# slothfulxtx/Texture-GS

Measured on AMD Instinct MI355X. Metric: fwd+bwd views/sec @800x800, 300k Gaussians + 1024^2 texture; HBM GB/s vs roofline, higher is better.
Workload: dtype f32; 1 GPU; c3: N=300000 Gaussians, cubemap 6x1024x1024x3 f32, 800x800, fwd+bwd, sh_degree 3; parallelism=views sharded dp1, view_pipeline=3 HIP streams, order=accumulate, forwards begun one view per stream ahead, grad_allreduce=none (1 GPU)

## Files before the change

include/texgs.h:

```cpp
#ifndef TEXGS_H
#define TEXGS_H

#include <stddef.h>
#include <stdint.h>

#ifdef __cplusplus
extern "C" {
#endif

#define TEXGS_ABI_VERSION 19
#define TEXGS_TILE 16
#define TEXGS_REC_TEST_FLOATS 8
#define TEXGS_REC_SHADE_FLOATS 20
#define TEXGS_ACC_FLOATS 32

typedef struct TexGSFrame {
    int32_t image_height;
    int32_t image_width;
    float   tanfovx;
    float   tanfovy;
    float   scale_modifier;
    int32_t sh_degree;
    int32_t sh_coeffs;
    int32_t tex_res;
    int32_t num_gaussians;
    int32_t debug;
    const float* bg;
    const float* viewmatrix;
    const float* projmatrix;
    const float* campos;
} TexGSFrame;

typedef struct TexGSInputs {
    const float* means3D;
    const float* shs;
    const float* opacities;
    const float* scales;
    const float* rotations;
    const float* uvs;
    const float* gradient_uvs;
    const float* texture;
    const float* color_offset;
    const float* cov3D_precomp;
} TexGSInputs;

typedef struct TexGSGeom {
    float*    rec_test;
    float*    rec_shade;
    float*    depth;
    int32_t*  radii;
    uint32_t* rect;
    uint32_t* tiles_touched;
    uint32_t* offsets;
    void*     scan_temp;
    size_t    scan_temp_bytes;
} TexGSGeom;

typedef struct TexGSBinning {
    uint32_t  num_rendered;
    uint64_t* keys_unsorted;
    uint64_t* keys_sorted;
    uint32_t* point_list;
    uint32_t* ranges;
    uint32_t* tile_order;
    void*     sort_temp;
    size_t    sort_temp_bytes;
} TexGSBinning;

typedef struct TexGSImage {
    float*    out_color;
    float*    out_depth;
    float*    out_norm;
    float*    out_alpha;
    float*    final_T;
    uint32_t* n_contrib;
    uint32_t* tex_bin_count;
    uint32_t* survivors;
    uint16_t* surv_qmask;
    uint32_t* surv_count;
    uint32_t* tex_bin_resv;
} TexGSImage;
#define TEXGS_RESV_WORDS 192

#define TEXGS_ACC_MEANS3D 1
#define TEXGS_ACC_MEANS2D 2
#define TEXGS_ACC_SHS 4
#define TEXGS_ACC_OPACITIES 8
#define TEXGS_ACC_SCALES 16
#define TEXGS_ACC_ROTATIONS 32
#define TEXGS_ACC_UVS 64
#define TEXGS_ACC_COLOR_OFFSET 128
#define TEXGS_ACC_COV3D 256
#define TEXGS_ACC_ALL 511

#define TEXGS_WANT_TEXTURE   1
#define TEXGS_WANT_GAUSSIANS 2
#define TEXGS_WANT_ALL       3

typedef struct TexGSGrads {
    const float* dL_dcolor;
    const float* dL_ddepth;
    const float* dL_dnorm;
    const float* dL_dalpha;
    float* acc;
    float* dL_dmeans3D;
    float* dL_dmeans2D;
    float* dL_dshs;
    float* dL_dopacities;
    float* dL_dscales;
    float* dL_drotations;
    float* dL_duvs;
    float* dL_dtexture;
    float* dL_dcolor_offset;
    float* dL_dcov3D;
    uint32_t want;
    float*    tex_bins;
    uint32_t* tex_bin_cursor;
    uint32_t* tex_bin_base;
    uint32_t  tex_rec_cap;
    int32_t accumulate;
} TexGSGrads;

int         texgs_abi_version(void);
const char* texgs_build_id(void);
const char* texgs_last_error(void);

size_t texgs_scan_temp_bytes(int32_t num_gaussians);
size_t texgs_sort_temp_bytes(uint32_t num_rendered, uint32_t num_tiles);
size_t texgs_tex_bin_count(int32_t tex_res);
#define TEXGS_TEXBIN_RECORD_FLOATS 4

int texgs_preprocess_forward(const TexGSFrame* frame, const TexGSInputs* in, TexGSGeom* geom, void* stream);

size_t texgs_num_rendered_words(int32_t num_gaussians);
int texgs_num_rendered_begin(const TexGSGeom* geom, int32_t num_gaussians, uint32_t* host_pinned, size_t host_words, int32_t sort_first,
                             void* stream);
int texgs_num_rendered_reduce(const uint32_t* host_pinned, int32_t num_gaussians, uint32_t* host_out, uint64_t* fingerprint_out);
int texgs_depth_sort_scan(TexGSGeom* geom, int32_t num_gaussians, void* stream);

int texgs_bin_sort_render_forward(const TexGSFrame* frame, const TexGSInputs* in, const TexGSGeom* geom,
                                  TexGSBinning* bin, TexGSImage* img, void* stream);

int texgs_render_forward(const TexGSFrame* frame, const TexGSInputs* in, const TexGSGeom* geom,
                         const TexGSBinning* bin, TexGSImage* img, void* stream);

int texgs_backward(const TexGSFrame* frame, const TexGSInputs* in, const TexGSGeom* geom,
                   const TexGSBinning* bin, const TexGSImage* img, TexGSGrads* grads, void* stream);

int texgs_backward_render(const TexGSFrame* frame, const TexGSInputs* in, const TexGSGeom* geom,
                          const TexGSBinning* bin, const TexGSImage* img, TexGSGrads* grads, void* stream);
int texgs_backward_preprocess(const TexGSFrame* frame, const TexGSInputs* in, const TexGSGeom* geom, TexGSGrads* grads,
                              void* stream);

enum {
    TEXGS_K_PREPROCESS_FWD = 0, TEXGS_K_SCAN = 1, TEXGS_K_DUPLICATE = 2, TEXGS_K_SORT = 3, TEXGS_K_RANGES = 4,
    TEXGS_K_RENDER_FWD = 5, TEXGS_K_RENDER_BWD = 6, TEXGS_K_PREPROCESS_BWD = 7, TEXGS_K_TEXGRAD_REDUCE = 8,
    TEXGS_NUM_KERNELS = 9
};
int texgs_profile_enable(int on);
int texgs_profile_select(uint32_t kernel_mask);
int texgs_profile_read(float* ms_sum_host, uint32_t* launches_host);

int texgs_rgb_alpha_loss(const float* image, const float* gt_image, const float* alpha, const float* gt_alpha,
                         int32_t H, int32_t W, float lambda_dssim, float lambda_alpha, float* scratch, float* sums,
                         float* dL_dimage, float* dL_dalpha, void* stream);

int texgs_geom_losses(const float* norm, const float* gt_norm, const float* gt_image, const float* mask, const float* depth,
                      const float* gt_depth, int32_t H, int32_t W, float lambda_norm, float lambda_smooth, float gamma,
                      float lambda_depth, float* sums, float* dL_dnorm, float* dL_ddepth, void* stream);

int texgs_norm_from_depth(const float* depth, const float* viewmatrix, float tanfovx, float tanfovy, int32_t H, int32_t W,
                          float threshold, float* out_norm, float* out_mask, void* stream);

typedef struct TexGSUVNet {
    const float *W1, *b1;
    const float *W2, *b2;
    const float *emb;
    const float *W3, *b3, *W4, *b4;
    const float *W5, *b5;
    const float *xyz_offset, *xyz_scale;
    int32_t hidden;
} TexGSUVNet;
enum { TEXGS_UV_FP32 = 0, TEXGS_UV_BF16X3 = 1, TEXGS_UV_MIXED = 2 };
size_t texgs_uv_packed_bytes(int32_t precision);
int texgs_uv_pack(const TexGSUVNet* net, int32_t precision, void* packed, void* stream);
int texgs_uv_taylor_packed(const TexGSUVNet* net, int32_t precision, const void* packed, const float* xyz, int32_t N, float* uvs,
                           float* grad_uvs, void* stream);

typedef struct TexGSUVNetGrad {
    float *dW1, *db1;
    float *dW2, *db2;
    float *dW3, *db3, *dW4, *db4;
    float *dW5, *db5;
} TexGSUVNetGrad;
size_t texgs_uv_backward_temp_bytes(int32_t N);
int texgs_uv_backward(const TexGSUVNet* net, int32_t precision, const float* xyz, const float* g_uvs, int32_t N, const TexGSUVNetGrad* out,
                      void* temp, void* stream);

#define TEXGS_HASHGRID_MAX_LEVELS 16
#define TEXGS_HASHGRID_FEATURES 4
typedef struct TexGSHashGrid {
    int32_t n_levels;
    int32_t n_features;
    int32_t log2_hashmap_size;
    float   base_resolution;
    float   per_level_scale;
} TexGSHashGrid;
int texgs_hashgrid_levels(const TexGSHashGrid* grid, float* scale, uint32_t* res, uint32_t* size, uint32_t* offset, uint32_t* n_params);
int texgs_hashgrid_forward(const TexGSHashGrid* grid, const float* params, const float* x, int32_t N, float* enc, void* stream);
size_t texgs_hashgrid_backward_temp_bytes(const TexGSHashGrid* grid, int32_t N);
int texgs_hashgrid_backward(const TexGSHashGrid* grid, const float* params, const float* x, const float* d_enc, int32_t N,
                            float* d_params, float* d_x, void* temp, void* stream);
size_t texgs_chamfer_nn_temp_bytes(int32_t P);
int texgs_chamfer_nn(const float* a, int32_t P, const float* b, int32_t Q, float* d2, int32_t* idx, void* temp, void* stream);

size_t texgs_knn3_temp_bytes(int32_t n);
int texgs_knn3_mean_dist2(const float* xyz, int32_t n, float* mean_d2, void* temp, void* stream);
size_t texgs_fps_temp_bytes(int32_t n, int32_t k);
int texgs_farthest_points(const float* xyz, int32_t n, int32_t k, int32_t start, int32_t* idx, void* temp, void* stream);

#define TEXGS_CUBE_LINEAR 0
#define TEXGS_CUBE_NEAREST 1
int texgs_cube_sample(const float* tex, int32_t R, int32_t C, const float* dirs, int32_t N, int32_t filter, int32_t tap_map,
                      float* out, void* stream);
int texgs_cube_latlong(const float* tex, int32_t R, int32_t C, int32_t H, int32_t W, int32_t tap_map, float* out, void* stream);
int texgs_cube_sample_backward(const float* tex, int32_t R, int32_t C, const float* dirs, int32_t N, const float* g_out,
                               float* d_tex, float* d_dirs, void* stream);
int texgs_cube_sample_nearest_backward(int32_t R, int32_t C, const float* dirs, int32_t N, const float* g_out, float* d_tex,
                                       void* stream);

int texgs_density_stats(const float* grad, const int32_t* radii, int32_t n, float* accum, float* denom, float* max_radii, void* stream);

#define TEXGS_DENSITY_KEEP       1
#define TEXGS_DENSITY_CLONE      2
#define TEXGS_DENSITY_CLONE_KEPT 4
#define TEXGS_DENSITY_SPLIT      8
#define TEXGS_DENSITY_CHILD      16
typedef struct {
    const float* accum;
    const float* denom;
    const float* scaling;
    const float* opacity;
    int32_t n;
    float max_grad, min_opacity, dense_scale, big_scale;
    int32_t densify, use_big;
} TexGSDensityPlan;
size_t texgs_density_plan_temp_bytes(int32_t n);
int texgs_density_plan(const TexGSDensityPlan* plan, uint8_t* action, int32_t* rank, uint32_t* totals, void* temp, void* stream);

#define TEXGS_DENSITY_ROW_COPY    0
#define TEXGS_DENSITY_ROW_MOMENT  1
#define TEXGS_DENSITY_ROW_SCALING 2
#define TEXGS_DENSITY_ROW_XYZ     3
#define TEXGS_DENSITY_MAX_ROWS    24
typedef struct {
    const float* src;
    float* dst;
    int32_t width;
    int32_t kind;
} TexGSDensityRow;
typedef struct {
    TexGSDensityRow row[TEXGS_DENSITY_MAX_ROWS];
    int32_t rows;
    int32_t n;
    const uint8_t* action;
    const int32_t* rank;
    int32_t n_kept, n_clone, n_split, n_child;
    const float* scaling;
    const float* rotation;
    const float* noise;
} TexGSDensityMove;
int texgs_density_move(const TexGSDensityMove* move, void* stream);

#define TEXGS_METRICS_ROW     16
#define TEXGS_METRICS_L1      0
#define TEXGS_METRICS_SE      1
#define TEXGS_METRICS_SSIM    4
#define TEXGS_METRICS_MAE_NUM 7
#define TEXGS_METRICS_MAE_DEN 8
#define TEXGS_METRICS_PIXELS  9
#define TEXGS_METRICS_CROPPED 10
size_t texgs_eval_metrics_temp_bytes(int32_t H, int32_t W);
int texgs_eval_metrics(const float* image, const float* gt_image, const float* norm, const float* gt_norm, const float* alpha,
                       int32_t H, int32_t W, int32_t clamp01, void* temp, double* row, void* stream);

int texgs_selftest_waveops(const float* seed128, float* out576, void* stream);

int texgs_mark_visible(const TexGSFrame* frame, const float* means3D, uint8_t* visible, void* stream);

#ifdef __cplusplus
}
#endif
#endif
```

texture-gs_amd/csrc/abi.hip:

```cpp
#include "common.h"
#include <stdio.h>
#include <string.h>
#include <stdlib.h>

#include <mutex>
#include <vector>

namespace {

thread_local char g_err[512] = "";

struct EvRec { int kid; hipEvent_t a, b; };
std::mutex g_prof_mu;
bool g_prof_on = false;
uint32_t g_prof_mask = 0xFFFFFFFFu;
std::vector<EvRec> g_prof_log;
std::vector<hipEvent_t> g_prof_free;

hipEvent_t prof_event() {
    if (!g_prof_free.empty()) { hipEvent_t e = g_prof_free.back(); g_prof_free.pop_back(); return e; }
    hipEvent_t e; (void)hipEventCreate(&e); return e;
}

struct ProfScope {
    int kid; hipStream_t s; hipEvent_t a; bool on;
    ProfScope(int k, hipStream_t st) : kid(k), s(st), a(nullptr), on(false) {
        std::lock_guard<std::mutex> l(g_prof_mu);
        if (g_prof_on && ((g_prof_mask >> k) & 1u)) { on = true; a = prof_event(); (void)hipEventRecord(a, s); }
    }
    ~ProfScope() {
        if (!on) return;
        std::lock_guard<std::mutex> l(g_prof_mu);
        hipEvent_t b = prof_event(); (void)hipEventRecord(b, s);
        g_prof_log.push_back({kid, a, b});
    }
};

int fail(const char* where, hipError_t e) {
    snprintf(g_err, sizeof(g_err), "%s: %s", where, hipGetErrorString(e));
    return (int)e ? (int)e : -1;
}

int fail_msg(const char* msg) {
    snprintf(g_err, sizeof(g_err), "%s", msg);
    return -1;
}

int check(const TexGSFrame* f, hipStream_t s, const char* where) {
    hipError_t e = hipGetLastError();
    if (e != hipSuccess) return fail(where, e);
    if (f->debug) {
        e = hipStreamSynchronize(s);
        if (e != hipSuccess) return fail(where, e);
    }
    return 0;
}

int validate_frame(const TexGSFrame* f) {
    if (!f) return fail_msg("frame is NULL");
    if (f->image_height <= 0 || f->image_width <= 0) return fail_msg("image size must be positive");
    if (f->image_width > 65535 * TEXGS_TILE || f->image_height > 65535 * TEXGS_TILE) return fail_msg("image too large");
    {
        const long long tx = (f->image_width + TEXGS_TILE - 1) / TEXGS_TILE, ty = (f->image_height + TEXGS_TILE - 1) / TEXGS_TILE;
        if (tx * ty > (1ll << 24)) return fail_msg("image too large: more than 2^24 tiles");
    }
    if (f->sh_degree < 0 || f->sh_degree > 3) return fail_msg("sh_degree must be in [0,3]");
    if (f->num_gaussians < 0) return fail_msg("num_gaussians < 0");
    if (f->tex_res <= 0) return fail_msg("tex_res must be positive");
    if (f->tex_res > 7168) return fail_msg("tex_res > 7168: the blend kernels address texels with 32-bit byte offsets (6 R^2 x 12 B < 2^32)");
    if (!f->bg || !f->viewmatrix || !f->projmatrix || !f->campos) return fail_msg("frame device pointers must be non-NULL");
    return 0;
}

}

extern "C" {

int texgs_abi_version(void) { return TEXGS_ABI_VERSION; }

#ifndef TEXGS_BUILD_ID
#define TEXGS_BUILD_ID "unknown"
#endif
const char* texgs_build_id(void) { return TEXGS_BUILD_ID; }

const char* texgs_last_error(void) { return g_err; }

size_t texgs_scan_temp_bytes(int32_t num_gaussians) { return scan_temp_bytes(num_gaussians); }

size_t texgs_sort_temp_bytes(uint32_t num_rendered, uint32_t num_tiles) { return sort_temp_bytes(num_rendered, num_tiles); }

size_t texgs_tex_bin_count(int32_t tex_res) { return tex_bin_count(tex_res); }

int texgs_preprocess_forward(const TexGSFrame* frame, const TexGSInputs* in, TexGSGeom* geom, void* stream) {
    if (int r = validate_frame(frame)) return r;
    if (!in || !geom) return fail_msg("NULL argument");
    if (frame->num_gaussians == 0) return 0;
    if (!in->means3D || !in->opacities) return fail_msg("per-Gaussian input pointer is NULL");
    if (in->texture && (!in->uvs || !in->gradient_uvs)) return fail_msg("uvs / gradient_uvs are required with a texture");
    if (in->cov3D_precomp && in->texture) return fail_msg("cov3D_precomp is an input of the untextured surface only (texture must be NULL)");
    if (!in->cov3D_precomp && (!in->scales || !in->rotations)) return fail_msg("scales and rotations (or cov3D_precomp) are required");
    if (geom->scan_temp_bytes < scan_temp_bytes(frame->num_gaussians)) return fail_msg("scan_temp too small");
    hipStream_t s = (hipStream_t)stream;
    const CamConst c = make_cam(frame);
    { ProfScope p(TEXGS_K_PREPROCESS_FWD, s); launch_preprocess_fwd(c, frame, in, geom, s); }
    if (int r = check(frame, s, "preprocess_fwd")) return r;
    return 0;
}

static int depth_sort_scan(const TexGSFrame* frame, TexGSGeom* geom, hipStream_t s) {
    if (frame->num_gaussians == 0) return 0;
    { ProfScope p(TEXGS_K_SCAN, s);
      if (int r = launch_depth_sort_scan(geom, frame->num_gaussians, s)) return fail("depth sort / scan", (hipError_t)r); }
    return check(frame, s, "depth sort / scan");
}

size_t texgs_num_rendered_words(int32_t num_gaussians) {
    return num_gaussians <= 0 ? 0 : 3 * (((size_t)num_gaussians + TG_BLOCK - 1) / TG_BLOCK);
}
int texgs_num_rendered_begin(const TexGSGeom* geom, int32_t num_gaussians, uint32_t* host_pinned, size_t host_words, int32_t sort_first,
                             void* stream) {
    if (!geom || !host_pinned) return fail_msg("NULL argument");
    if (num_gaussians <= 0) return 0;
    const size_t nw = texgs_num_rendered_words(num_gaussians);
    if (host_words < nw) return fail_msg("host buffer too small (texgs_num_rendered_words)");
    hipStream_t s = (hipStream_t)stream;
    hipError_t e = hipMemcpyAsync(host_pinned, bin_block_sums_ptr(geom, num_gaussians), nw * sizeof(uint32_t), hipMemcpyDeviceToHost, s);
    if (e != hipSuccess) return fail("num_rendered readback", e);
    if (sort_first) {
        TexGSFrame f0; memset(&f0, 0, sizeof(f0)); f0.num_gaussians = num_gaussians;
        if (int r = depth_sort_scan(&f0, const_cast<TexGSGeom*>(geom), s)) return r;
    }
    return 0;
}
int texgs_num_rendered_reduce(const uint32_t* host_pinned, int32_t num_gaussians, uint32_t* host_out, uint64_t* fingerprint_out) {
    if (!host_pinned || !host_out) return fail_msg("NULL argument");
    *host_out = 0;
    if (fingerprint_out) *fingerprint_out = 0;
    if (num_gaussians <= 0) return 0;
    const size_t nblk = ((size_t)num_gaussians + TG_BLOCK - 1) / TG_BLOCK;
    unsigned long long total = 0ull;
    uint32_t fa = 0u, fb = 0u;
    for (size_t k = 0; k < nblk; ++k) { total += host_pinned[k]; fa += host_pinned[nblk + k]; fb += host_pinned[2 * nblk + k]; }
    if (total > 0xFFFFFFFFull) return fail_msg("num_rendered exceeds 2^32 - 1 instances");
    *host_out = (uint32_t)total;
    if (fingerprint_out) *fingerprint_out = ((uint64_t)fb << 32) | (uint64_t)fa;
    return 0;
}

int texgs_depth_sort_scan(TexGSGeom* geom, int32_t num_gaussians, void* stream) {
    if (!geom) return fail_msg("NULL argument");
    TexGSFrame f0; memset(&f0, 0, sizeof(f0)); f0.num_gaussians = num_gaussians;
    return depth_sort_scan(&f0, geom, (hipStream_t)stream);
}

static int render_forward_impl(const TexGSFrame* frame, const TexGSInputs* in, const TexGSGeom* geom,
                               const TexGSBinning* bin, TexGSImage* img, void* stream, bool counters_zeroed) {
    if (int r = validate_frame(frame)) return r;
    if (!in || !geom || !bin || !img) return fail_msg("NULL argument");
    hipStream_t s = (hipStream_t)stream;
    const CamConst c = make_cam(frame);
    if (img->tex_bin_count && in->texture && !counters_zeroed) {
        hipError_t e = hipMemsetAsync(img->tex_bin_count, 0, sizeof(uint32_t) * 2 * tex_bin_count(c.R), s);
        if (e != hipSuccess) return fail("tex_bin_count memset", e);
    }
    { ProfScope p(TEXGS_K_RENDER_FWD, s); launch_render_fwd(c, frame, in, geom, bin, img, s); }
    return check(frame, s, "render_fwd");
}

int texgs_render_forward(const TexGSFrame* frame, const TexGSInputs* in, const TexGSGeom* geom,
                         const TexGSBinning* bin, TexGSImage* img, void* stream) {
    return render_forward_impl(frame, in, geom, bin, img, stream, false);
}

int texgs_bin_sort_render_forward(const TexGSFrame* frame, const TexGSInputs* in, const TexGSGeom* geom,
                                  TexGSBinning* bin, TexGSImage* img, void* stream) {
    if (int r = validate_frame(frame)) return r;
    if (!in || !geom || !bin || !img) return fail_msg("NULL argument");
    hipStream_t s = (hipStream_t)stream;
    const CamConst c = make_cam(frame);
    if (bin->num_rendered > 0) {
        if (bin->sort_temp_bytes < sort_temp_bytes(bin->num_rendered, (uint32_t)(c.tiles_x * c.tiles_y))) return fail_msg("sort_temp too small");
        { ProfScope p(TEXGS_K_DUPLICATE, s); launch_duplicate(c, geom, bin, s); }
        if (int r = check(frame, s, "duplicate_with_keys")) return r;
        { ProfScope p(TEXGS_K_SORT, s);
          if (int r = launch_sort(c, geom, bin, s)) return fail("tile sort", (hipError_t)r); }
        if (int r = check(frame, s, "tile sort")) return r;
    }
    { ProfScope p(TEXGS_K_RANGES, s);
      launch_ranges(c, bin, img->tex_bin_count, img->tex_bin_count ? 2 * (int)tex_bin_count(c.R) : 0, s); }
    if (int r = check(frame, s, "tile_ranges")) return r;
    return render_forward_impl(frame, in, geom, bin, img, stream, true);
}

int texgs_backward_render(const TexGSFrame* frame, const TexGSInputs* in, const TexGSGeom* geom,
                          const TexGSBinning* bin, const TexGSImage* img, TexGSGrads* grads, void* stream) {
    if (int r = validate_frame(frame)) return r;
    if (!in || !geom || !bin || !img || !grads) return fail_msg("NULL argument");
    if (!(grads->want & TEXGS_WANT_ALL)) return fail_msg("TexGSGrads.want is empty: ask for TEXGS_WANT_TEXTURE and / or TEXGS_WANT_GAUSSIANS");
    if ((grads->want & TEXGS_WANT_GAUSSIANS) && !grads->acc) return fail_msg("acc must be allocated (zero-filled) when Gaussian gradients are wanted");
    if ((grads->want & TEXGS_WANT_TEXTURE) && in->texture && !grads->dL_dtexture) return fail_msg("dL_dtexture must be allocated (zero-filled) when the texture gradient is wanted");
    if (!img->survivors || !img->surv_qmask || !img->surv_count)
        return fail_msg("the forward of this call left no survivor lists (TexGSImage.survivors / surv_qmask / surv_count were NULL): "
                        "run the forward with them to be able to run its backward");
    hipStream_t s = (hipStream_t)stream;
    const CamConst c = make_cam(frame);
    if (bin->num_rendered > 0) {
        { ProfScope p(TEXGS_K_RENDER_BWD, s); launch_render_bwd(c, frame, in, geom, bin, img, grads, s); }
        if (int r = check(frame, s, "render_bwd")) return r;
        if (tex_bins_enabled(c, in, img, grads)) {
            { ProfScope p(TEXGS_K_TEXGRAD_REDUCE, s); launch_texgrad_reduce(c, img, grads, s); }
            if (int r = check(frame, s, "texgrad_reduce")) return r;
        }
    }
    return 0;
}

int texgs_backward_preprocess(const TexGSFrame* frame, const TexGSInputs* in, const TexGSGeom* geom, TexGSGrads* grads,
                              void* stream) {
    if (int r = validate_frame(frame)) return r;
    if (!in || !geom || !grads) return fail_msg("NULL argument");
    if (!(grads->want & TEXGS_WANT_GAUSSIANS)) return 0;
    if (!grads->acc) return fail_msg("acc must be allocated");
    if (in->cov3D_precomp && !grads->dL_dcov3D) return fail_msg("dL_dcov3D is required with cov3D_precomp");
    hipStream_t s = (hipStream_t)stream;
    const CamConst c = make_cam(frame);
    { ProfScope p(TEXGS_K_PREPROCESS_BWD, s); launch_preprocess_bwd(c, frame, in, geom, grads, s); }
    return check(frame, s, "preprocess_bwd");
}

int texgs_backward(const TexGSFrame* frame, const TexGSInputs* in, const TexGSGeom* geom,
                   const TexGSBinning* bin, const TexGSImage* img, TexGSGrads* grads, void* stream) {
    if (int r = texgs_backward_render(frame, in, geom, bin, img, grads, stream)) return r;
    return texgs_backward_preprocess(frame, in, geom, grads, stream);
}

int texgs_profile_enable(int on) {
    std::lock_guard<std::mutex> l(g_prof_mu);
    g_prof_on = on != 0;
    if (!g_prof_on) {
        for (auto& r : g_prof_log) { g_prof_free.push_back(r.a); g_prof_free.push_back(r.b); }
        g_prof_log.clear();
    }
    return 0;
}

int texgs_profile_select(uint32_t kernel_mask) {
    std::lock_guard<std::mutex> l(g_prof_mu);
    g_prof_mask = kernel_mask;
    return 0;
}

int texgs_profile_read(float* ms_sum_host, uint32_t* launches_host) {
    if (!ms_sum_host || !launches_host) return fail_msg("NULL argument");
    std::lock_guard<std::mutex> l(g_prof_mu);
    for (auto& r : g_prof_log) {
        hipError_t e = hipEventSynchronize(r.b);
        if (e != hipSuccess) return fail("profile event sync", e);
        float ms = 0.f;
        e = hipEventElapsedTime(&ms, r.a, r.b);
        if (e != hipSuccess) return fail("profile elapsed", e);
        if (r.kid >= 0 && r.kid < TEXGS_NUM_KERNELS) { ms_sum_host[r.kid] += ms; launches_host[r.kid] += 1; }
        g_prof_free.push_back(r.a); g_prof_free.push_back(r.b);
    }
    g_prof_log.clear();
    return 0;
}

int texgs_rgb_alpha_loss(const float* image, const float* gt_image, const float* alpha, const float* gt_alpha,
                         int32_t H, int32_t W, float lambda_dssim, float lambda_alpha, float* scratch, float* sums,
                         float* dL_dimage, float* dL_dalpha, void* stream) {
    if (!image || !gt_image || !scratch || !sums || !dL_dimage) return fail_msg("NULL argument");
    if (H <= 0 || W <= 0) return fail_msg("image size must be positive");
    hipStream_t s = (hipStream_t)stream;
    launch_rgb_alpha_loss(image, gt_image, alpha, gt_alpha, H, W, lambda_dssim, lambda_alpha, scratch, sums, dL_dimage,
                          dL_dalpha, s);
    hipError_t e = hipGetLastError();
    return e == hipSuccess ? 0 : fail("rgb_alpha_loss", e);
}

int texgs_geom_losses(const float* norm, const float* gt_norm, const float* gt_image, const float* mask, const float* depth,
                      const float* gt_depth, int32_t H, int32_t W, float lambda_norm, float lambda_smooth, float gamma,
                      float lambda_depth, float* sums, float* dL_dnorm, float* dL_ddepth, void* stream) {
    if (!sums) return fail_msg("NULL argument");
    if (H <= 0 || W <= 0 || !(gamma > 0.f)) return fail_msg("image size and gamma must be positive");
    if (lambda_norm != 0.f && (!norm || !gt_norm || !dL_dnorm)) return fail_msg("norm term needs norm, gt_norm, dL_dnorm");
    if (lambda_smooth != 0.f && (!norm || !gt_image || !dL_dnorm)) return fail_msg("smoothness term needs norm, gt_image, dL_dnorm");
    if (lambda_depth != 0.f && (!depth || !gt_depth || !dL_ddepth)) return fail_msg("depth term needs depth, gt_depth, dL_ddepth");
    launch_geom_losses(norm, gt_norm, gt_image, mask, depth, gt_depth, H, W, lambda_norm, lambda_smooth, gamma, lambda_depth, sums,
                       dL_dnorm, dL_ddepth, (hipStream_t)stream);
    hipError_t e = hipGetLastError();
    return e == hipSuccess ? 0 : fail("geom_losses", e);
}

int texgs_norm_from_depth(const float* depth, const float* viewmatrix, float tanfovx, float tanfovy, int32_t H, int32_t W,
                          float threshold, float* out_norm, float* out_mask, void* stream) {
    if (!depth || !viewmatrix || !out_norm || !out_mask) return fail_msg("NULL argument");
    if (H <= 0 || W <= 0) return fail_msg("image size must be positive");
    launch_norm_from_depth(depth, viewmatrix, tanfovx, tanfovy, H, W, threshold, out_norm, out_mask, (hipStream_t)stream);
    hipError_t e = hipGetLastError();
    return e == hipSuccess ? 0 : fail("norm_from_depth", e);
}

static int check_uvnet(const TexGSUVNet* net, int32_t precision) {
    if (precision != TEXGS_UV_FP32 && precision != TEXGS_UV_BF16X3 && precision != TEXGS_UV_MIXED)
        return fail_msg("precision must be TEXGS_UV_FP32, TEXGS_UV_BF16X3 or TEXGS_UV_MIXED");
    if (net->hidden != 128) return fail_msg("the UV-map kernels support the shipped UVNet shape only (hidden width 128)");
    if (!net->W1 || !net->W2 || !net->W3 || !net->W4 || !net->W5 || !net->emb) return fail_msg("weight pointer is NULL");
    return 0;
}

size_t texgs_uv_packed_bytes(int32_t precision) { return uv_packed_bytes(precision); }

int texgs_uv_pack(const TexGSUVNet* net, int32_t precision, void* packed, void* stream) {
    if (!net || !packed) return fail_msg("NULL argument");
    if (int r = check_uvnet(net, precision)) return r;
    if (int r = launch_uv_pack(net, precision, packed, (hipStream_t)stream)) return fail("uv_pack", (hipError_t)r);
    return 0;
}

int texgs_uv_taylor_packed(const TexGSUVNet* net, int32_t precision, const void* packed, const float* xyz, int32_t N, float* uvs,
                           float* grad_uvs, void* stream) {
    if (!net || !packed) return fail_msg("NULL argument");
    if (int r = check_uvnet(net, precision)) return r;
    if (N < 0) return fail_msg("N < 0");
    if (N > 0 && (!xyz || !uvs || !grad_uvs)) return fail_msg("NULL argument");
    if (int r = launch_uv_taylor_packed(net, precision, packed, xyz, N, uvs, grad_uvs, (hipStream_t)stream)) return fail("uv_taylor", (hipError_t)r);
    return 0;
}

size_t texgs_uv_backward_temp_bytes(int32_t N) { return uv_backward_temp_bytes(N < 0 ? 0 : N); }

int texgs_uv_backward(const TexGSUVNet* net, int32_t precision, const float* xyz, const float* g_uvs, int32_t N, const TexGSUVNetGrad* out,
                      void* temp, void* stream) {
    if (!net || !out || !temp) return fail_msg("NULL argument");
    if (int r = check_uvnet(net, precision)) return r;
    if (N < 0) return fail_msg("N < 0");
    if (N > 0 && (!xyz || !g_uvs)) return fail_msg("NULL argument");
    if (int r = launch_uv_backward(net, xyz, g_uvs, N, out, temp, precision != TEXGS_UV_FP32, (hipStream_t)stream))
        return fail("uv_backward", (hipError_t)r);
    return 0;
}

static int check_hashgrid(const TexGSHashGrid* g, uint32_t* n_params) {
    if (!g) return fail_msg("grid is NULL");
    float sc[TEXGS_HASHGRID_MAX_LEVELS];
    uint32_t r[TEXGS_HASHGRID_MAX_LEVELS], sz[TEXGS_HASHGRID_MAX_LEVELS], off[TEXGS_HASHGRID_MAX_LEVELS];
    switch (hashgrid_levels(g, sc, r, sz, off, n_params)) {
    case 0: return 0;
    case -1: return fail_msg("hash grid: n_levels must be in [1, 16]");
    case -2: return fail_msg("hash grid: n_features must be 4");
    case -3: return fail_msg("hash grid: log2_hashmap_size must be in [1, 24]");
    case -4: return fail_msg("hash grid: base_resolution must be >= 1 and per_level_scale in [1, 16]");
    case -5: return fail_msg("hash grid: a level's resolution is out of range");
    default: return fail_msg("hash grid: more than 2^31 parameters");
    }
}

int texgs_hashgrid_levels(const TexGSHashGrid* grid, float* scale, uint32_t* res, uint32_t* size, uint32_t* offset, uint32_t* n_params) {
    uint32_t n = 0;
    if (int r = check_hashgrid(grid, &n)) return r;
    float sc[TEXGS_HASHGRID_MAX_LEVELS];
    uint32_t rs[TEXGS_HASHGRID_MAX_LEVELS], sz[TEXGS_HASHGRID_MAX_LEVELS], off[TEXGS_HASHGRID_MAX_LEVELS];
    hashgrid_levels(grid, sc, rs, sz, off, &n);
    for (int l = 0; l < grid->n_levels; ++l) {
        if (scale) scale[l] = sc[l];
        if (res) res[l] = rs[l];
        if (size) size[l] = sz[l];
        if (offset) offset[l] = off[l];
    }
    if (n_params) *n_params = n;
    return 0;
}

int texgs_hashgrid_forward(const TexGSHashGrid* grid, const float* params, const float* x, int32_t N, float* enc, void* stream) {
    uint32_t n = 0;
    if (int r = check_hashgrid(grid, &n)) return r;
    if (N < 0) return fail_msg("N < 0");
    if ((int64_t)N * grid->n_levels * TEXGS_HASHGRID_FEATURES > INT32_MAX) return fail_msg("N * L * F >= 2^31");
    if (N > 0 && (!params || !x || !enc)) return fail_msg("NULL argument");
    if (N > 0 && (((uintptr_t)params | (uintptr_t)enc) & 15)) return fail_msg("params and enc must be 16-byte aligned");
    if (int r = launch_hashgrid_forward(grid, params, x, N, enc, (hipStream_t)stream)) return fail("hashgrid_forward", (hipError_t)r);
    hipError_t e = hipGetLastError();
    return e == hipSuccess ? 0 : fail("hashgrid_forward", e);
}

size_t texgs_hashgrid_backward_temp_bytes(const TexGSHashGrid* grid, int32_t N) {
    uint32_t n = 0;
    if (!grid || check_hashgrid(grid, &n)) return 0;
    return hashgrid_backward_temp_bytes(grid, N);
}

int texgs_hashgrid_backward(const TexGSHashGrid* grid, const float* params, const float* x, const float* d_enc, int32_t N,
                            float* d_params, float* d_x, void* temp, void* stream) {
    uint32_t n = 0;
    if (int r = check_hashgrid(grid, &n)) return r;
    if (N < 0) return fail_msg("N < 0");
    if ((int64_t)N * grid->n_levels * TEXGS_HASHGRID_FEATURES > INT32_MAX) return fail_msg("N * L * F >= 2^31");
    if (N > 0 && (!params || !x || !d_enc)) return fail_msg("NULL argument");
    if (N > 0 && (((uintptr_t)params | (uintptr_t)d_enc | (uintptr_t)d_params) & 15))
        return fail_msg("params, d_enc and d_params must be 16-byte aligned");
    if (N > 0 && d_x && !temp) return fail_msg("temp is NULL (d_x needs texgs_hashgrid_backward_temp_bytes)");
    if (int r = launch_hashgrid_backward(grid, params, x, d_enc, N, d_params, d_x, temp, (hipStream_t)stream))
        return fail("hashgrid_backward", (hipError_t)r);
    hipError_t e = hipGetLastError();
    return e == hipSuccess ? 0 : fail("hashgrid_backward", e);
}

size_t texgs_chamfer_nn_temp_bytes(int32_t P) { return chamfer_nn_temp_bytes(P); }

int texgs_chamfer_nn(const float* a, int32_t P, const float* b, int32_t Q, float* d2, int32_t* idx, void* temp, void* stream) {
    if (P < 0) return fail_msg("P < 0");
    if (Q < 1) return fail_msg("the reference set is empty (Q < 1)");
    if ((int64_t)Q > 65535ll * 512) return fail_msg("Q > 65535 * 512");
    if (P > 0 && (!a || !b || !d2 || !idx || !temp)) return fail_msg("NULL argument");
    if (int r = launch_chamfer_nn(a, P, b, Q, d2, idx, temp, (hipStream_t)stream)) return fail("chamfer_nn", (hipError_t)r);
    hipError_t e = hipGetLastError();
    return e == hipSuccess ? 0 : fail("chamfer_nn", e);
}

size_t texgs_knn3_temp_bytes(int32_t n) { return knn3_temp_bytes(n); }

int texgs_knn3_mean_dist2(const float* xyz, int32_t n, float* mean_d2, void* temp, void* stream) {
    if (n < 4) return fail_msg("n < 4: three nearest other points need at least four points");
    if (!xyz || !mean_d2 || !temp) return fail_msg("NULL argument");
    if (int r = launch_knn3_mean_dist2(xyz, n, mean_d2, temp, (hipStream_t)stream)) return fail("knn3_mean_dist2", (hipError_t)r);
    return 0;
}

size_t texgs_fps_temp_bytes(int32_t n, int32_t k) { return fps_temp_bytes(n, k); }

int texgs_farthest_points(const float* xyz, int32_t n, int32_t k, int32_t start, int32_t* idx, void* temp, void* stream) {
    if (n < 1) return fail_msg("n < 1");
    if (k < 1 || k > n) return fail_msg("k must be in [1, n]");
    if (start < 0 || start >= n) return fail_msg("start must be in [0, n)");
    if (!xyz || !idx || !temp) return fail_msg("NULL argument");
    if (int r = launch_farthest_points(xyz, n, k, start, idx, temp, (hipStream_t)stream)) return fail("farthest_points", (hipError_t)r);
    return 0;
}

static int cube_shape_ok(int32_t R, int32_t C) {
    if (R < 2) return fail_msg("R < 2: a cubemap face needs at least 2 x 2 texels");
    if (C < 1) return fail_msg("C < 1");
    if (6ll * R * R * C >= (1ll << 31)) return fail_msg("6 R R C must be below 2^31");
    return 0;
}

int texgs_cube_sample(const float* tex, int32_t R, int32_t C, const float* dirs, int32_t N, int32_t filter, int32_t tap_map,
                      float* out, void* stream) {
    if (int r = cube_shape_ok(R, C)) return r;
    if (N < 0) return fail_msg("N < 0");
    if (filter != TEXGS_CUBE_LINEAR && filter != TEXGS_CUBE_NEAREST) return fail_msg("filter must be TEXGS_CUBE_LINEAR or TEXGS_CUBE_NEAREST");
    if (!tex || (N > 0 && (!dirs || !out))) return fail_msg("NULL argument");
    if (int r = launch_cube_sample(tex, R, C, dirs, N, filter, tap_map, out, (hipStream_t)stream)) return fail("cube_sample", (hipError_t)r);
    return 0;
}

int texgs_cube_latlong(const float* tex, int32_t R, int32_t C, int32_t H, int32_t W, int32_t tap_map, float* out, void* stream) {
    if (int r = cube_shape_ok(R, C)) return r;
    if (H < 1 || W < 1) return fail_msg("H and W must be positive");
    if ((long long)H * W >= (1ll << 31)) return fail_msg("H W must be below 2^31");
    if (!tex || !out) return fail_msg("NULL argument");
    if (int r = launch_cube_latlong(tex, R, C, H, W, tap_map, out, (hipStream_t)stream)) return fail("cube_latlong", (hipError_t)r);
    return 0;
}

int texgs_cube_sample_backward(const float* tex, int32_t R, int32_t C, const float* dirs, int32_t N, const float* g_out,
                               float* d_tex, float* d_dirs, void* stream) {
    if (int r = cube_shape_ok(R, C)) return r;
    if (N < 0) return fail_msg("N < 0");
    if (!d_tex && !d_dirs) return fail_msg("d_tex and d_dirs are both NULL: nothing to compute");
    if ((d_dirs && !tex) || (N > 0 && (!dirs || !g_out))) return fail_msg("NULL argument");
    if (int r = launch_cube_sample_backward(tex, R, C, dirs, N, g_out, d_tex, d_dirs, (hipStream_t)stream))
        return fail("cube_sample_backward", (hipError_t)r);
    return 0;
}

int texgs_cube_sample_nearest_backward(int32_t R, int32_t C, const float* dirs, int32_t N, const float* g_out, float* d_tex,
                                       void* stream) {
    if (int r = cube_shape_ok(R, C)) return r;
    if (N < 0) return fail_msg("N < 0");
    if (!d_tex || (N > 0 && (!dirs || !g_out))) return fail_msg("NULL argument");
    if (int r = launch_cube_sample_nearest_backward(R, C, dirs, N, g_out, d_tex, (hipStream_t)stream))
        return fail("cube_sample_nearest_backward", (hipError_t)r);
    return 0;
}

int texgs_density_stats(const float* grad, const int32_t* radii, int32_t n, float* accum, float* denom, float* max_radii, void* stream) {
    if (n < 0) return fail_msg("n < 0");
    if (n > 0 && (!grad || !radii || !accum || !denom || !max_radii)) return fail_msg("NULL argument");
    if (int r = launch_density_stats(grad, radii, n, accum, denom, max_radii, (hipStream_t)stream)) return fail("density_stats", (hipError_t)r);
    return 0;
}

size_t texgs_density_plan_temp_bytes(int32_t n) { return density_plan_temp_bytes(n); }

int texgs_density_plan(const TexGSDensityPlan* plan, uint8_t* action, int32_t* rank, uint32_t* totals, void* temp, void* stream) {
    if (!plan || !totals) return fail_msg("NULL argument");
    if (plan->n < 0) return fail_msg("n < 0");
    if (plan->n > 0 && (!plan->scaling || !plan->opacity || !action || !rank || !temp)) return fail_msg("NULL argument");
    if (plan->n > 0 && plan->densify && (!plan->accum || !plan->denom)) return fail_msg("accum and denom are required to densify");
    if (plan->densify && !(plan->max_grad > 0.0f)) return fail_msg("max_grad must be positive (with 0 the reference splits its own clones)");
    if (int r = launch_density_plan(plan, action, rank, totals, temp, (hipStream_t)stream)) return fail("density_plan", (hipError_t)r);
    return 0;
}

int texgs_density_move(const TexGSDensityMove* m, void* stream) {
    if (!m) return fail_msg("NULL argument");
    if (m->n < 0 || m->n_kept < 0 || m->n_clone < 0 || m->n_split < 0 || m->n_child < 0) return fail_msg("negative count");
    if (m->n_kept > m->n || m->n_clone > m->n || m->n_split > m->n || m->n_child > m->n_split) return fail_msg("totals exceed n");
    if ((int64_t)m->n_kept + m->n_clone + 2ll * m->n_child >= (1ll << 31)) return fail_msg("the new row count reaches 2^31");
    if (m->rows < 0 || m->rows > TEXGS_DENSITY_MAX_ROWS) return fail_msg("rows must be in [0, TEXGS_DENSITY_MAX_ROWS]");
    if (m->n == 0 || m->rows == 0) return 0;
    if (!m->action || !m->rank) return fail_msg("NULL argument");
    const bool out_rows = m->n_kept + m->n_clone + m->n_child > 0;
    for (int d = 0; d < m->rows; ++d) {
        const TexGSDensityRow& r = m->row[d];
        if (r.width < 1) return fail_msg("row width < 1");
        if (r.kind < TEXGS_DENSITY_ROW_COPY || r.kind > TEXGS_DENSITY_ROW_XYZ) return fail_msg("unknown row kind");
        if (r.kind == TEXGS_DENSITY_ROW_XYZ && r.width != 3) return fail_msg("an XYZ row has width 3");
        if (!r.src || (out_rows && !r.dst)) return fail_msg("NULL row pointer");
        if (r.kind == TEXGS_DENSITY_ROW_XYZ && m->n_child > 0 && (!m->scaling || !m->rotation || !m->noise))
            return fail_msg("an XYZ row with children needs scaling, rotation and noise");
    }
    if (!out_rows) return 0;
    if (int r = launch_density_move(m, (hipStream_t)stream)) return fail("density_move", (hipError_t)r);
    return 0;
}

size_t texgs_eval_metrics_temp_bytes(int32_t H, int32_t W) { return eval_metrics_temp_bytes(H, W); }

int texgs_eval_metrics(const float* image, const float* gt_image, const float* norm, const float* gt_norm, const float* alpha,
                       int32_t H, int32_t W, int32_t clamp01, void* temp, double* row, void* stream) {
    if (!image || !gt_image || !temp || !row) return fail_msg("NULL argument");
    if (H < 7 || W < 7) return fail_msg("H and W must be at least 7: the 7x7 SSIM window does not fit");
    if ((!norm) != (!gt_norm)) return fail_msg("norm and gt_norm must be both NULL or both set");
    if ((((int64_t)W + 31) / 32) * (((int64_t)H + 31) / 32) >= (1ll << 31)) return fail_msg("image too large: 2^31 tiles or more");
    if (int r = launch_eval_metrics(image, gt_image, norm, gt_norm, alpha, H, W, clamp01 != 0, temp, row, (hipStream_t)stream))
        return fail("eval_metrics", (hipError_t)r);
    return 0;
}

int texgs_selftest_waveops(const float* seed128, float* out576, void* stream) {
    if (!seed128 || !out576) return fail_msg("NULL argument");
    launch_selftest_waveops(seed128, out576, (hipStream_t)stream);
    hipError_t e = hipGetLastError();
    return e == hipSuccess ? 0 : fail("selftest_waveops", e);
}

int texgs_mark_visible(const TexGSFrame* frame, const float* means3D, uint8_t* visible, void* stream) {
    if (int r = validate_frame(frame)) return r;
    if (!means3D || !visible) return fail_msg("NULL argument");
    hipStream_t s = (hipStream_t)stream;
    launch_mark_visible(frame, means3D, visible, s);
    return check(frame, s, "mark_visible");
}

}
```

texture-gs_amd/csrc/common.h:

```cpp
#pragma once
#include <hip/hip_runtime.h>
#include <stdint.h>
#include "texgs.h"

#define TG_NEAR_Z        0.2f
#define TG_LOWPASS       0.3f
#define TG_FRUSTUM_CLAMP 1.3f
#define TG_ALPHA_MAX     0.99f
#define TG_ALPHA_MIN     (1.0f / 255.0f)
#define TG_T_EPS         1e-4f
#define TG_PLANE_EPS     5e-2f
#define TG_DEN_MIN       0.2f
#define TG_MA_MIN        1e-20f
#define TG_SH_C0         0.28209479177387814f

enum {
    R_XY = 0, R_CONIC = 2, R_OP = 5, R_G2 = 6, R_GM = 8, R_PHI = 14, R_VD = 17, R_DEPTH = 20, R_N = 21
};
enum {
    M_P = 0, M_DEN = 6, M_DN = 9, M_PHI = 18, M_VD = 21, M_DEPTH = 24, M_N = 25
};

#define TG_BLOCK 256

struct CamConst {
    int W, H, tiles_x, tiles_y;
    float fx, fy, tanfovx, tanfovy;
    float scale_modifier;
    int sh_degree, sh_coeffs, R, N;
};

static inline CamConst make_cam(const TexGSFrame* f) {
    CamConst c;
    c.W = f->image_width; c.H = f->image_height;
    c.tiles_x = (c.W + TEXGS_TILE - 1) / TEXGS_TILE;
    c.tiles_y = (c.H + TEXGS_TILE - 1) / TEXGS_TILE;
    c.tanfovx = f->tanfovx; c.tanfovy = f->tanfovy;
    c.fx = (float)c.W / (2.0f * f->tanfovx);
    c.fy = (float)c.H / (2.0f * f->tanfovy);
    c.scale_modifier = f->scale_modifier;
    c.sh_degree = f->sh_degree; c.sh_coeffs = f->sh_coeffs; c.R = f->tex_res; c.N = f->num_gaussians;
    return c;
}

void launch_preprocess_fwd(const CamConst& c, const TexGSFrame* f, const TexGSInputs* in, TexGSGeom* g, hipStream_t s);
void launch_preprocess_bwd(const CamConst& c, const TexGSFrame* f, const TexGSInputs* in, const TexGSGeom* g,
                           TexGSGrads* gr, hipStream_t s);
void launch_mark_visible(const TexGSFrame* f, const float* means3D, uint8_t* visible, hipStream_t s);
int  launch_depth_sort_scan(const TexGSGeom* g, int N, hipStream_t s);
uint32_t* bin_block_sums_ptr(const TexGSGeom* g, int N);
uint32_t* bin_header_ptr(const TexGSGeom* g, int N, int* words);
size_t scan_temp_bytes(int N);
size_t sort_temp_bytes(uint32_t D, uint32_t T);
void launch_duplicate(const CamConst& c, const TexGSGeom* g, TexGSBinning* b, hipStream_t s);
int  launch_sort(const CamConst& c, const TexGSGeom* g, TexGSBinning* b, hipStream_t s);
void launch_ranges(const CamConst& c, TexGSBinning* b, uint32_t* zero_words, int num_zero_words, hipStream_t s);
void launch_render_fwd(const CamConst& c, const TexGSFrame* f, const TexGSInputs* in, const TexGSGeom* g,
                       const TexGSBinning* b, TexGSImage* img, hipStream_t s);
size_t tex_bin_count(int R);
bool tex_bins_enabled(const CamConst& c, const TexGSInputs* in, const TexGSImage* img, const TexGSGrads* gr);
void launch_texgrad_reduce(const CamConst& c, const TexGSImage* img, TexGSGrads* gr, hipStream_t s);
void launch_render_bwd(const CamConst& c, const TexGSFrame* f, const TexGSInputs* in, const TexGSGeom* g,
                       const TexGSBinning* b, const TexGSImage* img, TexGSGrads* gr, hipStream_t s);
int launch_rgb_alpha_loss(const float* image, const float* gt_image, const float* alpha, const float* gt_alpha, int H,
                          int W, float lambda_dssim, float lambda_alpha, float* scratch, float* sums, float* d_image,
                          float* d_alpha, hipStream_t s);
void launch_selftest_waveops(const float* seed128, float* out576, hipStream_t s);
int launch_geom_losses(const float* norm, const float* gt_norm, const float* gt_image, const float* mask, const float* depth,
                       const float* gt_depth, int H, int W, float lambda_norm, float lambda_smooth, float gamma,
                       float lambda_depth, float* sums, float* d_norm, float* d_depth, hipStream_t s);
int launch_norm_from_depth(const float* depth, const float* viewmatrix, float tanfovx, float tanfovy, int H, int W, float threshold,
                           float* out_norm, float* out_mask, hipStream_t s);
size_t uv_packed_bytes(int precision);
int launch_uv_pack(const TexGSUVNet* net, int precision, void* packed, hipStream_t s);
int launch_uv_taylor_packed(const TexGSUVNet* net, int precision, const void* packed, const float* xyz, int N, float* uvs, float* grad_uvs,
                            hipStream_t s);
size_t uv_backward_temp_bytes(int N);
int launch_uv_backward(const TexGSUVNet* net, const float* xyz, const float* g, int N, const TexGSUVNetGrad* out, void* temp, int mixed,
                       hipStream_t s);
int hashgrid_levels(const TexGSHashGrid* g, float* scale, uint32_t* res, uint32_t* size, uint32_t* offset, uint32_t* n_params);
int launch_hashgrid_forward(const TexGSHashGrid* g, const float* params, const float* x, int N, float* enc, hipStream_t s);
size_t hashgrid_backward_temp_bytes(const TexGSHashGrid* g, int N);
int launch_hashgrid_backward(const TexGSHashGrid* g, const float* params, const float* x, const float* d_enc, int N, float* d_params,
                             float* d_x, void* temp, hipStream_t s);
size_t chamfer_nn_temp_bytes(int P);
int launch_chamfer_nn(const float* a, int P, const float* b, int Q, float* d2, int32_t* idx, void* temp, hipStream_t s);
size_t sort_pairs32_temp_bytes(uint32_t n);
int launch_sort_pairs32(const uint32_t* keys_in, uint32_t n, int key_bits, uint32_t* keys_out, uint32_t* vals_out, void* temp, hipStream_t s);
size_t knn3_temp_bytes(int n);
int launch_knn3_mean_dist2(const float* xyz, int n, float* mean_d2, void* temp, hipStream_t s);
size_t fps_temp_bytes(int n, int k);
int launch_farthest_points(const float* xyz, int n, int k, int start, int32_t* idx, void* temp, hipStream_t s);
int launch_cube_sample(const float* tex, int R, int C, const float* dirs, int N, int filter, int tap_map, float* out, hipStream_t s);
int launch_cube_latlong(const float* tex, int R, int C, int H, int W, int tap_map, float* out, hipStream_t s);
int launch_cube_sample_backward(const float* tex, int R, int C, const float* dirs, int N, const float* g_out, float* d_tex,
                                float* d_dirs, hipStream_t s);
int launch_cube_sample_nearest_backward(int R, int C, const float* dirs, int N, const float* g_out, float* d_tex, hipStream_t s);
int launch_density_stats(const float* grad, const int32_t* radii, int n, float* accum, float* denom, float* max_radii, hipStream_t s);
size_t density_plan_temp_bytes(int n);
int launch_density_plan(const TexGSDensityPlan* p, uint8_t* action, int32_t* rank, uint32_t* totals, void* temp, hipStream_t s);
int launch_density_move(const TexGSDensityMove* m, hipStream_t s);
size_t eval_metrics_temp_bytes(int H, int W);
int launch_eval_metrics(const float* image, const float* gt_image, const float* norm, const float* gt_norm, const float* alpha, int H,
                        int W, int clamp01, void* temp, double* row, hipStream_t s);
```

texture-gs_amd/csrc/preprocess.hip:

```cpp
#include "common.h"

namespace {

struct Frame {
    float V[16];
    float P[16];
    float cam[3];
};

__device__ __forceinline__ Frame load_frame(const float* vm, const float* pm, const float* cp) {
    Frame f;
#pragma unroll
    for (int i = 0; i < 16; ++i) { f.V[i] = vm[i]; f.P[i] = pm[i]; }
    f.cam[0] = cp[0]; f.cam[1] = cp[1]; f.cam[2] = cp[2];
    return f;
}

struct Geo {
    bool  valid;
    float m[3], t[3];
    float hx, hy, hw, pw, xy[2];
    float q[4], s[3], R[9], M[9], S[6];
    float txc, tyc; bool clx, cly;
    float J00, J02, J11, J12, T0[3], T1[3];
    float a, b, c, det, inv, conic[3];
    int   radius;
    int   kmin; float sign; float n[3];
    float nv[3], sdot; bool degen; float gx, gy, G[6], K[9];
    float dir[3], dlen;
};

#define WR(F, r, c) ((F).V[(c) * 4 + (r)])

__device__ __forceinline__ void smallest_eigvec(const float* S6, float* n) {
    const float tr = S6[0] + S6[3] + S6[5];
    const float sc = (tr > 0.f) ? 1.0f / tr : 1.0f;
    float a00 = S6[0] * sc, a01 = S6[1] * sc, a02 = S6[2] * sc, a11 = S6[3] * sc, a12 = S6[4] * sc, a22 = S6[5] * sc;
    float v00 = 1.f, v01 = 0.f, v02 = 0.f, v10 = 0.f, v11 = 1.f, v12 = 0.f, v20 = 0.f, v21 = 0.f, v22 = 1.f;
    auto rot = [](float& app, float& aqq, float& apq, float& arp, float& arq, float& v0p, float& v0q, float& v1p, float& v1q,
                  float& v2p, float& v2q) {
        if (fabsf(apq) < 1e-30f) return;
        const float theta = (aqq - app) / (2.0f * apq);
        const float t = ((theta >= 0.f) ? 1.0f : -1.0f) / (fabsf(theta) + sqrtf(theta * theta + 1.0f));
        const float c = 1.0f / sqrtf(t * t + 1.0f), sn = t * c;
        app -= t * apq; aqq += t * apq; apq = 0.f;
        const float rp = arp, rq = arq;
        arp = c * rp - sn * rq; arq = sn * rp + c * rq;
        float x;
        x = v0p; v0p = c * x - sn * v0q; v0q = sn * x + c * v0q;
        x = v1p; v1p = c * x - sn * v1q; v1q = sn * x + c * v1q;
        x = v2p; v2p = c * x - sn * v2q; v2q = sn * x + c * v2q;
    };
#pragma unroll 1
    for (int sweep = 0; sweep < 6; ++sweep) {
        rot(a00, a11, a01, a02, a12, v00, v01, v10, v11, v20, v21);
        rot(a00, a22, a02, a01, a12, v00, v02, v10, v12, v20, v22);
        rot(a11, a22, a12, a01, a02, v01, v02, v11, v12, v21, v22);
    }
    int k = 0; float m = a00;
    if (a11 < m) { m = a11; k = 1; }
    if (a22 < m) { m = a22; k = 2; }
    n[0] = (k == 0) ? v00 : ((k == 1) ? v01 : v02);
    n[1] = (k == 0) ? v10 : ((k == 1) ? v11 : v12);
    n[2] = (k == 0) ? v20 : ((k == 1) ? v21 : v22);
}

template <bool COV = false>
__device__ __forceinline__ void geo_forward(Geo& g, const Frame& F, const CamConst& C, int i,
                                            const float* __restrict__ means, const float* __restrict__ scales,
                                            const float* __restrict__ rots, const float* __restrict__ juv,
                                            const float* __restrict__ cov6 = nullptr) {
    g.m[0] = means[3 * i + 0]; g.m[1] = means[3 * i + 1]; g.m[2] = means[3 * i + 2];
    const float mx = g.m[0], my = g.m[1], mz = g.m[2];
    g.t[0] = F.V[0] * mx + F.V[4] * my + F.V[8] * mz + F.V[12];
    g.t[1] = F.V[1] * mx + F.V[5] * my + F.V[9] * mz + F.V[13];
    g.t[2] = F.V[2] * mx + F.V[6] * my + F.V[10] * mz + F.V[14];
    g.valid = g.t[2] > TG_NEAR_Z;
    g.radius = 0;
    if (!g.valid) return;
    const float tx = g.t[0], ty = g.t[1], tz = g.t[2];

    g.hx = F.P[0] * mx + F.P[4] * my + F.P[8] * mz + F.P[12];
    g.hy = F.P[1] * mx + F.P[5] * my + F.P[9] * mz + F.P[13];
    g.hw = F.P[3] * mx + F.P[7] * my + F.P[11] * mz + F.P[15];
    g.pw = 1.0f / (g.hw + 1e-7f);
    const float ndcx = g.hx * g.pw, ndcy = g.hy * g.pw;
    g.xy[0] = ((ndcx + 1.0f) * (float)C.W - 1.0f) * 0.5f;
    g.xy[1] = ((ndcy + 1.0f) * (float)C.H - 1.0f) * 0.5f;

    float s0 = 0.f, s1 = 0.f, s2 = 0.f;
    if constexpr (COV) {
#pragma unroll
        for (int k = 0; k < 6; ++k) g.S[k] = cov6[6 * i + k];
#pragma unroll
        for (int k = 0; k < 9; ++k) { g.R[k] = 0.f; g.M[k] = 0.f; }
        g.q[0] = g.q[1] = g.q[2] = g.q[3] = 0.f; g.s[0] = g.s[1] = g.s[2] = 0.f;
    } else {
    g.q[0] = rots[4 * i + 0]; g.q[1] = rots[4 * i + 1]; g.q[2] = rots[4 * i + 2]; g.q[3] = rots[4 * i + 3];
    const float r = g.q[0], x = g.q[1], y = g.q[2], z = g.q[3];
    g.R[0] = 1.0f - 2.0f * (y * y + z * z); g.R[1] = 2.0f * (x * y - r * z); g.R[2] = 2.0f * (x * z + r * y);
    g.R[3] = 2.0f * (x * y + r * z); g.R[4] = 1.0f - 2.0f * (x * x + z * z); g.R[5] = 2.0f * (y * z - r * x);
    g.R[6] = 2.0f * (x * z - r * y); g.R[7] = 2.0f * (y * z + r * x); g.R[8] = 1.0f - 2.0f * (x * x + y * y);
    s0 = scales[3 * i + 0]; s1 = scales[3 * i + 1]; s2 = scales[3 * i + 2];
    g.s[0] = C.scale_modifier * s0; g.s[1] = C.scale_modifier * s1; g.s[2] = C.scale_modifier * s2;
#pragma unroll
    for (int rr = 0; rr < 3; ++rr)
#pragma unroll
        for (int cc = 0; cc < 3; ++cc) g.M[rr * 3 + cc] = g.R[rr * 3 + cc] * g.s[cc];
    const float* M = g.M;
    g.S[0] = M[0] * M[0] + M[1] * M[1] + M[2] * M[2];
    g.S[1] = M[0] * M[3] + M[1] * M[4] + M[2] * M[5];
    g.S[2] = M[0] * M[6] + M[1] * M[7] + M[2] * M[8];
    g.S[3] = M[3] * M[3] + M[4] * M[4] + M[5] * M[5];
    g.S[4] = M[3] * M[6] + M[4] * M[7] + M[5] * M[8];
    g.S[5] = M[6] * M[6] + M[7] * M[7] + M[8] * M[8];
    }

    const float limx = TG_FRUSTUM_CLAMP * C.tanfovx, limy = TG_FRUSTUM_CLAMP * C.tanfovy;
    const float txtz = tx / tz, tytz = ty / tz;
    g.clx = (txtz < -limx) || (txtz > limx);
    g.cly = (tytz < -limy) || (tytz > limy);
    g.txc = fminf(limx, fmaxf(-limx, txtz)) * tz;
    g.tyc = fminf(limy, fmaxf(-limy, tytz)) * tz;
    if (!g.clx) g.txc = tx;
    if (!g.cly) g.tyc = ty;
    const float tz2 = tz * tz;
    g.J00 = C.fx / tz; g.J02 = -(C.fx * g.txc) / tz2;
    g.J11 = C.fy / tz; g.J12 = -(C.fy * g.tyc) / tz2;
#pragma unroll
    for (int k = 0; k < 3; ++k) {
        g.T0[k] = g.J00 * WR(F, 0, k) + g.J02 * WR(F, 2, k);
        g.T1[k] = g.J11 * WR(F, 1, k) + g.J12 * WR(F, 2, k);
    }
    const float* S = g.S;
    const float v00 = S[0] * g.T0[0] + S[1] * g.T0[1] + S[2] * g.T0[2];
    const float v01 = S[1] * g.T0[0] + S[3] * g.T0[1] + S[4] * g.T0[2];
    const float v02 = S[2] * g.T0[0] + S[4] * g.T0[1] + S[5] * g.T0[2];
    const float v10 = S[0] * g.T1[0] + S[1] * g.T1[1] + S[2] * g.T1[2];
    const float v11 = S[1] * g.T1[0] + S[3] * g.T1[1] + S[4] * g.T1[2];
    const float v12 = S[2] * g.T1[0] + S[4] * g.T1[1] + S[5] * g.T1[2];
    g.a = (g.T0[0] * v00 + g.T0[1] * v01 + g.T0[2] * v02) + TG_LOWPASS;
    g.b = g.T1[0] * v00 + g.T1[1] * v01 + g.T1[2] * v02;
    g.c = (g.T1[0] * v10 + g.T1[1] * v11 + g.T1[2] * v12) + TG_LOWPASS;
    g.det = g.a * g.c - g.b * g.b;
    if (g.det == 0.0f) { g.valid = false; return; }
    g.inv = 1.0f / g.det;
    g.conic[0] = g.c * g.inv; g.conic[1] = -g.b * g.inv; g.conic[2] = g.a * g.inv;
    const float mid = 0.5f * (g.a + g.c);
    const float lam = mid + sqrtf(fmaxf(0.1f, mid * mid - g.det));
    g.radius = (int)ceilf(3.0f * sqrtf(lam));

    g.dir[0] = mx - F.cam[0]; g.dir[1] = my - F.cam[1]; g.dir[2] = mz - F.cam[2];
    float n0, n1, n2;
    if constexpr (COV) {
        float ev[3];
        smallest_eigvec(g.S, ev);
        n0 = ev[0]; n1 = ev[1]; n2 = ev[2];
        g.kmin = -1;
    } else {
        g.kmin = 0; float smin = s0;
        if (s1 < smin) { smin = s1; g.kmin = 1; }
        if (s2 < smin) { smin = s2; g.kmin = 2; }
        n0 = (g.kmin == 0) ? g.R[0] : ((g.kmin == 1) ? g.R[1] : g.R[2]);
        n1 = (g.kmin == 0) ? g.R[3] : ((g.kmin == 1) ? g.R[4] : g.R[5]);
        n2 = (g.kmin == 0) ? g.R[6] : ((g.kmin == 1) ? g.R[7] : g.R[8]);
    }
    g.sign = ((n0 * g.dir[0] + n1 * g.dir[1] + n2 * g.dir[2]) > 0.0f) ? -1.0f : 1.0f;
    g.n[0] = g.sign * n0; g.n[1] = g.sign * n1; g.n[2] = g.sign * n2;
    g.dlen = sqrtf(g.dir[0] * g.dir[0] + g.dir[1] * g.dir[1] + g.dir[2] * g.dir[2]);
    g.dir[0] /= g.dlen; g.dir[1] /= g.dlen; g.dir[2] /= g.dlen;

#pragma unroll
    for (int k = 0; k < 3; ++k)
        g.nv[k] = WR(F, k, 0) * g.n[0] + WR(F, k, 1) * g.n[1] + WR(F, k, 2) * g.n[2];
    g.sdot = g.nv[0] * tx + g.nv[1] * ty + g.nv[2] * tz;
    const float tn = sqrtf(tx * tx + ty * ty + tz * tz);
    g.degen = (juv == nullptr) || fabsf(g.sdot) <= TG_PLANE_EPS * tn;
#pragma unroll
    for (int rr = 0; rr < 3; ++rr)
#pragma unroll
        for (int cc = 0; cc < 3; ++cc)
            g.K[rr * 3 + cc] = (juv == nullptr) ? 0.0f
                             : juv[9 * i + rr * 3 + 0] * WR(F, cc, 0) + juv[9 * i + rr * 3 + 1] * WR(F, cc, 1)
                             + juv[9 * i + rr * 3 + 2] * WR(F, cc, 2);
    if (g.degen) {
        g.gx = 0.0f; g.gy = 0.0f;
#pragma unroll
        for (int k = 0; k < 6; ++k) g.G[k] = 0.0f;
    } else {
        const float ax = tz * g.nv[0] / g.sdot, ay = tz * g.nv[1] / g.sdot;
        g.gx = ax / C.fx; g.gy = ay / C.fy;
        const float B00 = tz / C.fx - tx * g.gx, B01 = -tx * g.gy;
        const float B10 = -ty * g.gx,            B11 = tz / C.fy - ty * g.gy;
        const float B20 = -tz * g.gx,            B21 = -tz * g.gy;
#pragma unroll
        for (int rr = 0; rr < 3; ++rr) {
            g.G[rr * 2 + 0] = g.K[rr * 3 + 0] * B00 + g.K[rr * 3 + 1] * B10 + g.K[rr * 3 + 2] * B20;
            g.G[rr * 2 + 1] = g.K[rr * 3 + 0] * B01 + g.K[rr * 3 + 1] * B11 + g.K[rr * 3 + 2] * B21;
        }
    }
}

__device__ __forceinline__ void tile_rect(const Geo& g, const CamConst& C, int& x0, int& y0, int& x1, int& y1) {
    const float rf = (float)g.radius;
    x0 = min(C.tiles_x, max(0, (int)((g.xy[0] - rf) / (float)TEXGS_TILE)));
    y0 = min(C.tiles_y, max(0, (int)((g.xy[1] - rf) / (float)TEXGS_TILE)));
    x1 = min(C.tiles_x, max(0, (int)((g.xy[0] + rf + (float)(TEXGS_TILE - 1)) / (float)TEXGS_TILE)));
    y1 = min(C.tiles_y, max(0, (int)((g.xy[1] + rf + (float)(TEXGS_TILE - 1)) / (float)TEXGS_TILE)));
}

__device__ __forceinline__ void sh_basis(int deg, float x, float y, float z, float* b) {
    const float C1 = 0.4886025119029199f;
    b[0] = -C1 * y; b[1] = C1 * z; b[2] = -C1 * x;
    if (deg > 1) {
        const float xx = x * x, yy = y * y, zz = z * z, xy = x * y, yz = y * z, xz = x * z;
        b[3] = 1.0925484305920792f * xy;
        b[4] = -1.0925484305920792f * yz;
        b[5] = 0.31539156525252005f * (2.0f * zz - xx - yy);
        b[6] = -1.0925484305920792f * xz;
        b[7] = 0.5462742152960396f * (xx - yy);
        if (deg > 2) {
            b[8]  = -0.5900435899266435f * y * (3.0f * xx - yy);
            b[9]  = 2.890611442640554f * xy * z;
            b[10] = -0.4570457994644658f * y * (4.0f * zz - xx - yy);
            b[11] = 0.3731763325901154f * z * (2.0f * zz - 3.0f * xx - 3.0f * yy);
            b[12] = -0.4570457994644658f * x * (4.0f * zz - xx - yy);
            b[13] = 1.445305721320277f * z * (xx - yy);
            b[14] = -0.5900435899266435f * x * (xx - 3.0f * yy);
        }
    }
}

__device__ __forceinline__ void sh_basis_grad(int deg, float x, float y, float z, float* bx, float* by, float* bz) {
    const float C1 = 0.4886025119029199f;
    bx[0] = 0.f; by[0] = -C1; bz[0] = 0.f;
    bx[1] = 0.f; by[1] = 0.f; bz[1] = C1;
    bx[2] = -C1; by[2] = 0.f; bz[2] = 0.f;
    if (deg > 1) {
        const float c20 = 1.0925484305920792f, c22 = 0.31539156525252005f, c24 = 0.5462742152960396f;
        bx[3] = c20 * y;   by[3] = c20 * x;   bz[3] = 0.f;
        bx[4] = 0.f;       by[4] = -c20 * z;  bz[4] = -c20 * y;
        bx[5] = c22 * (-2.0f * x); by[5] = c22 * (-2.0f * y); bz[5] = c22 * 4.0f * z;
        bx[6] = -c20 * z;  by[6] = 0.f;       bz[6] = -c20 * x;
        bx[7] = c24 * 2.0f * x; by[7] = -c24 * 2.0f * y; bz[7] = 0.f;
        if (deg > 2) {
            const float xx = x * x, yy = y * y, zz = z * z;
            const float c30 = -0.5900435899266435f, c31 = 2.890611442640554f, c32 = -0.4570457994644658f,
                        c33 = 0.3731763325901154f, c35 = 1.445305721320277f;
            bx[8]  = c30 * 6.0f * x * y;            by[8]  = c30 * (3.0f * xx - 3.0f * yy);        bz[8]  = 0.f;
            bx[9]  = c31 * y * z;                   by[9]  = c31 * x * z;                          bz[9]  = c31 * x * y;
            bx[10] = c32 * (-2.0f * x * y);         by[10] = c32 * (4.0f * zz - xx - 3.0f * yy);   bz[10] = c32 * 8.0f * y * z;
            bx[11] = c33 * (-6.0f * x * z);         by[11] = c33 * (-6.0f * y * z);                bz[11] = c33 * (6.0f * zz - 3.0f * xx - 3.0f * yy);
            bx[12] = c32 * (4.0f * zz - 3.0f * xx - yy); by[12] = c32 * (-2.0f * x * y);           bz[12] = c32 * 8.0f * x * z;
            bx[13] = c35 * 2.0f * x * z;            by[13] = -c35 * 2.0f * y * z;                  bz[13] = c35 * (xx - yy);
            bx[14] = c30 * (3.0f * xx - 3.0f * yy); by[14] = c30 * (-6.0f * x * y);                bz[14] = 0.f;
        }
    }
}

__device__ __forceinline__ int sh_active(int deg, int K) {
    const int want = (deg + 1) * (deg + 1) - 1;
    return want < K ? want : K;
}

template <int BLOCK, bool ADD>
__device__ __forceinline__ void sh_rows_out(float* __restrict__ g, const float* __restrict__ s, int count, bool vec) {
    const int tid = (int)threadIdx.x;
    int done = 0;
    if (vec) {
        const int n4 = count >> 2;
        float4* __restrict__ g4 = reinterpret_cast<float4*>(g);
        const float4* s4 = reinterpret_cast<const float4*>(s);
        for (int k = tid; k < n4; k += 4 * BLOCK) {
            float4 v[4], o[4];
            bool nz[4];
#pragma unroll
            for (int u = 0; u < 4; ++u) {
                const bool in = k + u * BLOCK < n4;
                v[u] = in ? s4[k + u * BLOCK] : make_float4(0.f, 0.f, 0.f, 0.f);
                nz[u] = in && (!ADD || v[u].x != 0.f || v[u].y != 0.f || v[u].z != 0.f || v[u].w != 0.f);
            }
            if (ADD) {
#pragma unroll
                for (int u = 0; u < 4; ++u) if (nz[u]) o[u] = g4[k + u * BLOCK];
#pragma unroll
                for (int u = 0; u < 4; ++u) if (nz[u]) g4[k + u * BLOCK] = make_float4(o[u].x + v[u].x, o[u].y + v[u].y, o[u].z + v[u].z, o[u].w + v[u].w);
            } else {
#pragma unroll
                for (int u = 0; u < 4; ++u) if (nz[u]) g4[k + u * BLOCK] = v[u];
            }
        }
        done = n4 << 2;
    }
    for (int k = done + tid; k < count; k += BLOCK) {
        const float v = s[k];
        if (ADD) { if (v != 0.f) g[k] += v; } else g[k] = v;
    }
}

template <bool COV>
__global__ void __launch_bounds__(TG_BLOCK)
k_preprocess_fwd(CamConst C, const float* __restrict__ vm, const float* __restrict__ pm, const float* __restrict__ cp,
                 const float* __restrict__ means, const float* __restrict__ shs, const float* __restrict__ opac,
                 const float* __restrict__ scales, const float* __restrict__ rots, const float* __restrict__ uvs,
                 const float* __restrict__ juv, const float* __restrict__ coff, const float* __restrict__ cov6,
                 float4* __restrict__ rec_test, float4* __restrict__ rec_shade, float* __restrict__ depth, int32_t* __restrict__ radii,
                 uint2* __restrict__ rect, uint32_t* __restrict__ tiles_touched, uint32_t* __restrict__ block_D,
                 uint32_t* __restrict__ zero_words, int num_zero_words) {
    extern __shared__ __attribute__((aligned(16))) float s_sh[];
    __shared__ uint32_t s_tt[5 * (TG_BLOCK / 64)];
    const int i = blockIdx.x * TG_BLOCK + threadIdx.x;
    const bool live = i < C.N;
    for (int k = i; k < num_zero_words; k += (int)gridDim.x * TG_BLOCK) zero_words[k] = 0u;
    const Frame F = load_frame(vm, pm, cp);
    Geo g;
    g.valid = false;
    if (live) geo_forward<COV>(g, F, C, i, means, scales, rots, juv, cov6);
    int x0 = 0, y0 = 0, x1 = 0, y1 = 0;
    if (g.valid) {
        tile_rect(g, C, x0, y0, x1, y1);
        if ((x1 - x0) * (y1 - y0) == 0) g.valid = false;
    }
    const int na = (shs != nullptr && C.sh_degree > 0) ? sh_active(C.sh_degree, C.sh_coeffs) : 0;
    const int row = 3 * C.sh_coeffs;
    if (na > 0) {
        const size_t first = (size_t)blockIdx.x * TG_BLOCK * row;
        const size_t total = (size_t)C.N * row;
        const int count = (int)min((size_t)TG_BLOCK * row, total - first);
        for (int k = threadIdx.x; k < count; k += TG_BLOCK) s_sh[k] = shs[first + k];
        __syncthreads();
    }
    uint32_t tt = 0u, ha = 0u, hb = 0u;
    if (live) {
        ha = (uint32_t)i * 0x9E3779B1u + 0x85EBCA77u;
        hb = ((uint32_t)i * 0xC2B2AE3Du) ^ 0x27D4EB2Fu;
    }
    auto mix = [&](uint32_t w) {
        ha = (ha ^ w) * 0x01000193u;
        hb = __builtin_rotateleft32(hb ^ w, 13) * 5u + 0xE6546B64u;
    };
    if (live && !g.valid) {
        radii[i] = 0; tiles_touched[i] = 0; rect[i] = make_uint2(0u, 0u);
        depth[i] = __uint_as_float(0xFFFFFFFFu);
        mix(0xFFFFFFFFu);
    }
    if (live && g.valid) {
    float vd[3] = {0.f, 0.f, 0.f};
    if (na > 0) {
        float b[15];
#pragma unroll
        for (int k = 0; k < 15; ++k) b[k] = 0.f;
        sh_basis(C.sh_degree, g.dir[0], g.dir[1], g.dir[2], b);
        const float* sp = s_sh + threadIdx.x * row;
#pragma unroll
        for (int k = 0; k < 15; ++k) {
            if (k < na) { vd[0] += b[k] * sp[3 * k + 0]; vd[1] += b[k] * sp[3 * k + 1]; vd[2] += b[k] * sp[3 * k + 2]; }
        }
    }
    if (coff) { vd[0] += coff[3 * i + 0]; vd[1] += coff[3 * i + 1]; vd[2] += coff[3 * i + 2]; }
    radii[i] = g.radius;
    tt = (uint32_t)((x1 - x0) * (y1 - y0));
    tiles_touched[i] = tt;
    depth[i] = g.t[2];
    const uint2 rc = make_uint2((uint32_t)x0 | ((uint32_t)y0 << 16), (uint32_t)x1 | ((uint32_t)y1 << 16));
    rect[i] = rc;
    const float op = opac[i];
    const float thr = (op > 0.0f) ? (-logf(255.0f * op) - 1e-3f) : 1.0f;
    const float cmid = 0.5f * (g.a + g.c);
    const float clam = cmid + sqrtf(fmaxf(0.1f, cmid * cmid - g.det));
    const float rcull = (thr < 0.0f) ? (sqrtf(-2.0f * thr * clam) * 1.001f + 0.01f) : -1.0f;
    const float4 t0 = make_float4(g.xy[0], g.xy[1], -0.5f * g.conic[0], -g.conic[1]);
    const float4 t1 = make_float4(-0.5f * g.conic[2], op, rcull, thr);
    const float4 s0 = make_float4(g.gx, g.gy, g.G[0], g.G[1]);
    const float4 s1 = make_float4(g.G[2], g.G[3], g.G[4], g.G[5]);
    const float4 s2 = uvs ? make_float4(uvs[3 * i + 0], uvs[3 * i + 1], uvs[3 * i + 2], vd[0]) : make_float4(0.f, 0.f, 1.f, vd[0]);
    float4* rt = rec_test + (size_t)i * (TEXGS_REC_TEST_FLOATS / 4);
    rt[0] = t0; rt[1] = t1;
    float4* rs = rec_shade + (size_t)i * (TEXGS_REC_SHADE_FLOATS / 4);
    rs[0] = s0; rs[1] = s1; rs[2] = s2;
    rs[3] = make_float4(vd[1], vd[2], g.t[2], g.n[0]);
    rs[4] = make_float4(g.n[1], g.n[2], g.xy[0], g.xy[1]);
    mix(__float_as_uint(g.t[2])); mix(rc.x); mix(rc.y);
    mix(__float_as_uint(t0.x)); mix(__float_as_uint(t0.y)); mix(__float_as_uint(t0.z)); mix(__float_as_uint(t0.w));
    mix(__float_as_uint(t1.x)); mix(__float_as_uint(t1.y)); mix(__float_as_uint(t1.z)); mix(__float_as_uint(t1.w));
    mix(__float_as_uint(s0.x)); mix(__float_as_uint(s0.y)); mix(__float_as_uint(s0.z)); mix(__float_as_uint(s0.w));
    mix(__float_as_uint(s1.x)); mix(__float_as_uint(s1.y)); mix(__float_as_uint(s1.z)); mix(__float_as_uint(s1.w));
    mix(__float_as_uint(s2.x)); mix(__float_as_uint(s2.y)); mix(__float_as_uint(s2.z));
    }
    ha ^= ha >> 15; ha *= 0x2C1B3C6Du; ha ^= ha >> 12;
    hb ^= hb >> 16; hb *= 0x85EBCA6Bu; hb ^= hb >> 13;
    if (!live) { ha = 0u; hb = 0u; }
    uint32_t kmin = (live && g.valid) ? __float_as_uint(g.t[2]) : 0xFFFFFFFFu, kmax = (live && g.valid) ? __float_as_uint(g.t[2]) : 0u;
    for (int d = 32; d >= 1; d >>= 1) {
        tt += __shfl_xor(tt, d, 64); ha += __shfl_xor(ha, d, 64); hb += __shfl_xor(hb, d, 64);
        kmin = min(kmin, (uint32_t)__shfl_xor((int)kmin, d, 64)); kmax = max(kmax, (uint32_t)__shfl_xor((int)kmax, d, 64));
    }
    constexpr int NW = TG_BLOCK / 64;
    if ((threadIdx.x & 63) == 0) {
        const int w = threadIdx.x >> 6;
        s_tt[w] = tt; s_tt[NW + w] = ha; s_tt[2 * NW + w] = hb; s_tt[3 * NW + w] = kmin; s_tt[4 * NW + w] = kmax;
    }
    __syncthreads();
    if (threadIdx.x < 5) {
        uint32_t r = s_tt[threadIdx.x * NW];
        for (int w = 1; w < NW; ++w) {
            const uint32_t v = s_tt[threadIdx.x * NW + w];
            r = (threadIdx.x < 3) ? r + v : ((threadIdx.x == 3) ? min(r, v) : max(r, v));
        }
        block_D[threadIdx.x * gridDim.x + blockIdx.x] = r;
    }
}

#ifndef K8_BLOCK
#define K8_BLOCK 256
#endif
template <bool COV>
__global__ void __launch_bounds__(K8_BLOCK)
k_preprocess_bwd(CamConst C, const float* __restrict__ vm, const float* __restrict__ pm, const float* __restrict__ cp,
                 const float* __restrict__ means, const float* __restrict__ shs, const float* __restrict__ opac,
                 const float* __restrict__ scales,
                 const float* __restrict__ rots, const float* __restrict__ juv, const float* __restrict__ cov6,
                 const int32_t* __restrict__ radii, float* __restrict__ acc,
                 float* __restrict__ d_means, float* __restrict__ d_means2D, float* __restrict__ d_shs,
                 float* __restrict__ d_op, float* __restrict__ d_scales, float* __restrict__ d_rots,
                 float* __restrict__ d_uvs, float* __restrict__ d_coff, float* __restrict__ d_cov6, int accumulate) {
    extern __shared__ __attribute__((aligned(16))) float s_sh[];
    const int i = blockIdx.x * K8_BLOCK + threadIdx.x;
    const int K = C.sh_coeffs;
    const bool live = i < C.N;
    const int row = 3 * K;
    const int na = (shs != nullptr && C.sh_degree > 0) ? sh_active(C.sh_degree, K) : 0;
    const size_t first = (size_t)blockIdx.x * K8_BLOCK * row;
    const int count = d_shs ? (int)min((size_t)K8_BLOCK * row, (size_t)C.N * row - first) : 0;
    const bool vec = d_shs && (((size_t)d_shs) & 15) == 0;
    if (na > 0 && d_shs) {
        for (int k = threadIdx.x; k < count; k += K8_BLOCK) s_sh[k] = shs[first + k];
        __syncthreads();
    }
    const bool visible = live && radii[i] > 0;
    if (live && !visible) {
        if (!(accumulate & TEXGS_ACC_MEANS3D)) d_means[3 * i] = d_means[3 * i + 1] = d_means[3 * i + 2] = 0.f;
        if (!(accumulate & TEXGS_ACC_MEANS2D)) d_means2D[3 * i] = d_means2D[3 * i + 1] = d_means2D[3 * i + 2] = 0.f;
        if (!(accumulate & TEXGS_ACC_OPACITIES)) d_op[i] = 0.f;
        if constexpr (COV) {
            if (!(accumulate & TEXGS_ACC_COV3D)) { for (int k = 0; k < 6; ++k) d_cov6[6 * i + k] = 0.f; }
        } else {
            if (!(accumulate & TEXGS_ACC_SCALES)) d_scales[3 * i] = d_scales[3 * i + 1] = d_scales[3 * i + 2] = 0.f;
            if (!(accumulate & TEXGS_ACC_ROTATIONS)) d_rots[4 * i] = d_rots[4 * i + 1] = d_rots[4 * i + 2] = d_rots[4 * i + 3] = 0.f;
        }
        if (d_uvs && !(accumulate & TEXGS_ACC_UVS)) d_uvs[3 * i] = d_uvs[3 * i + 1] = d_uvs[3 * i + 2] = 0.f;
        if (d_coff && !(accumulate & TEXGS_ACC_COLOR_OFFSET)) d_coff[3 * i] = d_coff[3 * i + 1] = d_coff[3 * i + 2] = 0.f;
    }
    if (visible) {
#define OUT(BIT, P, V) do { if (accumulate & (BIT)) (P) += (V); else (P) = (V); } while (0)
    const Frame F = load_frame(vm, pm, cp);
    Geo g;
    geo_forward<COV>(g, F, C, i, means, scales, rots, juv, cov6);
    float A[24];
    {
        float Mo[TEXGS_ACC_FLOATS];
        float4* ap = reinterpret_cast<float4*>(acc + (size_t)i * TEXGS_ACC_FLOATS);
#pragma unroll
        for (int k = 0; k < TEXGS_ACC_FLOATS / 4; ++k) {
            const float4 v = ap[k];
            Mo[4 * k] = v.x; Mo[4 * k + 1] = v.y; Mo[4 * k + 2] = v.z; Mo[4 * k + 3] = v.w;
            ap[k] = make_float4(0.f, 0.f, 0.f, 0.f);
        }
        const float ca = g.conic[0], cb = g.conic[1], cc = g.conic[2];
        const float m00 = Mo[M_P], m10 = Mo[M_P + 1], m01 = Mo[M_P + 2];
        const float N00 = Mo[M_DN], N10 = Mo[M_DN + 3], N20 = Mo[M_DN + 6], D0 = Mo[M_DEN];
        A[R_XY]     = -(ca * m10 + cb * m01) - ((g.G[0] * N00 + g.G[2] * N10 + g.G[4] * N20) + g.gx * D0);
        A[R_XY + 1] = -(cc * m01 + cb * m10) - ((g.G[1] * N00 + g.G[3] * N10 + g.G[5] * N20) + g.gy * D0);
        A[R_CONIC] = -0.5f * Mo[M_P + 3]; A[R_CONIC + 1] = -Mo[M_P + 4]; A[R_CONIC + 2] = -0.5f * Mo[M_P + 5];
        const float op = opac[i];
        A[R_OP] = (op > 0.0f) ? m00 / op : 0.0f;
        A[R_G2] = Mo[M_DEN + 1]; A[R_G2 + 1] = Mo[M_DEN + 2];
#pragma unroll
        for (int cidx = 0; cidx < 3; ++cidx) {
            A[R_GM + 2 * cidx] = Mo[M_DN + 3 * cidx + 1]; A[R_GM + 2 * cidx + 1] = Mo[M_DN + 3 * cidx + 2];
            A[R_PHI + cidx] = Mo[M_PHI + cidx]; A[R_VD + cidx] = Mo[M_VD + cidx]; A[R_N + cidx] = Mo[M_N + cidx];
        }
        A[R_DEPTH] = Mo[M_DEPTH];
    }
    const float tx = g.t[0], ty = g.t[1], tz = g.t[2];
    float dt[3] = {0.f, 0.f, 0.f};
    float dm[3] = {0.f, 0.f, 0.f};
    float dR[9];
#pragma unroll
    for (int k = 0; k < 9; ++k) dR[k] = 0.f;

    OUT(TEXGS_ACC_OPACITIES, d_op[i], A[R_OP]);
    if (d_uvs) { OUT(TEXGS_ACC_UVS, d_uvs[3 * i + 0], A[R_PHI]); OUT(TEXGS_ACC_UVS, d_uvs[3 * i + 1], A[R_PHI + 1]); OUT(TEXGS_ACC_UVS, d_uvs[3 * i + 2], A[R_PHI + 2]); }
    if (d_coff) { OUT(TEXGS_ACC_COLOR_OFFSET, d_coff[3 * i + 0], A[R_VD]); OUT(TEXGS_ACC_COLOR_OFFSET, d_coff[3 * i + 1], A[R_VD + 1]); OUT(TEXGS_ACC_COLOR_OFFSET, d_coff[3 * i + 2], A[R_VD + 2]); }

    const float dA = A[R_CONIC], dB = A[R_CONIC + 1], dC = A[R_CONIC + 2];
    const float inv = g.inv, inv2 = inv * inv;
    const float da = dA * (-g.c * g.c * inv2) + dB * (g.b * g.c * inv2) + dC * (inv - g.a * g.c * inv2);
    const float db = dA * (2.0f * g.b * g.c * inv2) + dB * (-inv - 2.0f * g.b * g.b * inv2) + dC * (2.0f * g.a * g.b * inv2);
    const float dc = dA * (inv - g.a * g.c * inv2) + dB * (g.a * g.b * inv2) + dC * (-g.a * g.a * inv2);
    const float hb = 0.5f * db;
    const float* S = g.S;
    float TS0[3], TS1[3];
    TS0[0] = g.T0[0] * S[0] + g.T0[1] * S[1] + g.T0[2] * S[2];
    TS0[1] = g.T0[0] * S[1] + g.T0[1] * S[3] + g.T0[2] * S[4];
    TS0[2] = g.T0[0] * S[2] + g.T0[1] * S[4] + g.T0[2] * S[5];
    TS1[0] = g.T1[0] * S[0] + g.T1[1] * S[1] + g.T1[2] * S[2];
    TS1[1] = g.T1[0] * S[1] + g.T1[1] * S[3] + g.T1[2] * S[4];
    TS1[2] = g.T1[0] * S[2] + g.T1[1] * S[4] + g.T1[2] * S[5];
    float dT0[3], dT1[3];
#pragma unroll
    for (int k = 0; k < 3; ++k) {
        dT0[k] = 2.0f * (da * TS0[k] + hb * TS1[k]);
        dT1[k] = 2.0f * (hb * TS0[k] + dc * TS1[k]);
    }
    float dS[9];
#pragma unroll
    for (int k = 0; k < 3; ++k)
#pragma unroll
        for (int l = 0; l < 3; ++l)
            dS[k * 3 + l] = g.T0[k] * g.T0[l] * da + (g.T0[k] * g.T1[l] + g.T1[k] * g.T0[l]) * hb + g.T1[k] * g.T1[l] * dc;
    float dM[9];
#pragma unroll
    for (int rr = 0; rr < 3; ++rr)
#pragma unroll
        for (int cc = 0; cc < 3; ++cc)
            dM[rr * 3 + cc] = 2.0f * (dS[rr * 3 + 0] * g.M[0 * 3 + cc] + dS[rr * 3 + 1] * g.M[1 * 3 + cc] + dS[rr * 3 + 2] * g.M[2 * 3 + cc]);
    float dscale[3];
#pragma unroll
    for (int cc = 0; cc < 3; ++cc) {
        dscale[cc] = (dM[0 + cc] * g.R[0 + cc] + dM[3 + cc] * g.R[3 + cc] + dM[6 + cc] * g.R[6 + cc]) * C.scale_modifier;
#pragma unroll
        for (int rr = 0; rr < 3; ++rr) dR[rr * 3 + cc] += dM[rr * 3 + cc] * g.s[cc];
    }
    const float dJ00 = dT0[0] * WR(F, 0, 0) + dT0[1] * WR(F, 0, 1) + dT0[2] * WR(F, 0, 2);
    const float dJ02 = dT0[0] * WR(F, 2, 0) + dT0[1] * WR(F, 2, 1) + dT0[2] * WR(F, 2, 2);
    const float dJ11 = dT1[0] * WR(F, 1, 0) + dT1[1] * WR(F, 1, 1) + dT1[2] * WR(F, 1, 2);
    const float dJ12 = dT1[0] * WR(F, 2, 0) + dT1[1] * WR(F, 2, 1) + dT1[2] * WR(F, 2, 2);
    const float tz2 = tz * tz, tz3 = tz2 * tz;
    dt[2] += -dJ00 * C.fx / tz2 - dJ11 * C.fy / tz2 + 2.0f * dJ02 * C.fx * g.txc / tz3 + 2.0f * dJ12 * C.fy * g.tyc / tz3;
    if (!g.clx) dt[0] += -dJ02 * C.fx / tz2;
    if (!g.cly) dt[1] += -dJ12 * C.fy / tz2;

    const float dndx = A[R_XY] * 0.5f * (float)C.W, dndy = A[R_XY + 1] * 0.5f * (float)C.H;
    OUT(TEXGS_ACC_MEANS2D, d_means2D[3 * i + 0], dndx); OUT(TEXGS_ACC_MEANS2D, d_means2D[3 * i + 1], dndy); if (!(accumulate & TEXGS_ACC_MEANS2D)) d_means2D[3 * i + 2] = 0.f;
    {
        const float dhx = dndx * g.pw, dhy = dndy * g.pw;
        const float dhw = -(dndx * g.hx + dndy * g.hy) * g.pw * g.pw;
#pragma unroll
        for (int k = 0; k < 3; ++k) dm[k] += dhx * F.P[k * 4 + 0] + dhy * F.P[k * 4 + 1] + dhw * F.P[k * 4 + 3];
    }
    dt[2] += A[R_DEPTH];
    float dn[3] = {A[R_N], A[R_N + 1], A[R_N + 2]};

    if (!g.degen) {
        const float* dG = &A[R_GM];
        float dBm[6];
#pragma unroll
        for (int k = 0; k < 3; ++k)
#pragma unroll
            for (int cc = 0; cc < 2; ++cc)
                dBm[k * 2 + cc] = g.K[0 * 3 + k] * dG[0 * 2 + cc] + g.K[1 * 3 + k] * dG[1 * 2 + cc] + g.K[2 * 3 + k] * dG[2 * 2 + cc];
        float dtz = dBm[0] / C.fx + dBm[3] / C.fy;
        float dgt[2];
#pragma unroll
        for (int cc = 0; cc < 2; ++cc)
            dgt[cc] = A[R_G2 + cc] - (dBm[0 * 2 + cc] * tx + dBm[1 * 2 + cc] * ty + dBm[2 * 2 + cc] * tz);
#pragma unroll
        for (int k = 0; k < 3; ++k) dt[k] -= dBm[k * 2 + 0] * g.gx + dBm[k * 2 + 1] * g.gy;
        const float dax = dgt[0] / C.fx, day = dgt[1] / C.fy;
        const float dot_a_nv = dax * g.nv[0] + day * g.nv[1];
        dtz += dot_a_nv / g.sdot;
        float dnv[3] = {tz * dax / g.sdot, tz * day / g.sdot, 0.f};
        const float ds = -tz * dot_a_nv / (g.sdot * g.sdot);
        dnv[0] += ds * tx; dnv[1] += ds * ty; dnv[2] += ds * tz;
        dt[0] += ds * g.nv[0]; dt[1] += ds * g.nv[1]; dt[2] += ds * g.nv[2] + dtz;
#pragma unroll
        for (int k = 0; k < 3; ++k)
            dn[k] += dnv[0] * WR(F, 0, k) + dnv[1] * WR(F, 1, k) + dnv[2] * WR(F, 2, k);
    }
#pragma unroll
    for (int k = 0; k < 3; ++k) {
        const float on = (g.kmin == k) ? g.sign : 0.0f;
        dR[0 + k] += on * dn[0]; dR[3 + k] += on * dn[1]; dR[6 + k] += on * dn[2];
    }

    if (d_shs && na > 0) {
        float b[15], bx[15], by[15], bz[15];
#pragma unroll
        for (int k = 0; k < 15; ++k) { b[k] = 0.f; bx[k] = 0.f; by[k] = 0.f; bz[k] = 0.f; }
        sh_basis(C.sh_degree, g.dir[0], g.dir[1], g.dir[2], b);
        sh_basis_grad(C.sh_degree, g.dir[0], g.dir[1], g.dir[2], bx, by, bz);
        float* sp = s_sh + threadIdx.x * row;
        const float v0 = A[R_VD], v1 = A[R_VD + 1], v2 = A[R_VD + 2];
        float ddx = 0.f, ddy = 0.f, ddz = 0.f;
#pragma unroll
        for (int k = 0; k < 15; ++k) {
            if (k < na) {
                const float w = sp[3 * k + 0] * v0 + sp[3 * k + 1] * v1 + sp[3 * k + 2] * v2;
                ddx += bx[k] * w; ddy += by[k] * w; ddz += bz[k] * w;
                sp[3 * k + 0] = b[k] * v0; sp[3 * k + 1] = b[k] * v1; sp[3 * k + 2] = b[k] * v2;
            }
        }
        for (int k = 3 * na; k < row; ++k) sp[k] = 0.f;
        const float dd = g.dir[0] * ddx + g.dir[1] * ddy + g.dir[2] * ddz;
        dm[0] += (ddx - g.dir[0] * dd) / g.dlen;
        dm[1] += (ddy - g.dir[1] * dd) / g.dlen;
        dm[2] += (ddz - g.dir[2] * dd) / g.dlen;
    }

#pragma unroll
    for (int k = 0; k < 3; ++k) dm[k] += dt[0] * F.V[k * 4 + 0] + dt[1] * F.V[k * 4 + 1] + dt[2] * F.V[k * 4 + 2];
    OUT(TEXGS_ACC_MEANS3D, d_means[3 * i + 0], dm[0]); OUT(TEXGS_ACC_MEANS3D, d_means[3 * i + 1], dm[1]); OUT(TEXGS_ACC_MEANS3D, d_means[3 * i + 2], dm[2]);
    if constexpr (COV) {
        OUT(TEXGS_ACC_COV3D, d_cov6[6 * i + 0], dS[0]); OUT(TEXGS_ACC_COV3D, d_cov6[6 * i + 1], dS[1] + dS[3]);
        OUT(TEXGS_ACC_COV3D, d_cov6[6 * i + 2], dS[2] + dS[6]); OUT(TEXGS_ACC_COV3D, d_cov6[6 * i + 3], dS[4]);
        OUT(TEXGS_ACC_COV3D, d_cov6[6 * i + 4], dS[5] + dS[7]); OUT(TEXGS_ACC_COV3D, d_cov6[6 * i + 5], dS[8]);
    }
    if constexpr (!COV) { OUT(TEXGS_ACC_SCALES, d_scales[3 * i + 0], dscale[0]); OUT(TEXGS_ACC_SCALES, d_scales[3 * i + 1], dscale[1]); OUT(TEXGS_ACC_SCALES, d_scales[3 * i + 2], dscale[2]); }

    if constexpr (!COV) {
    const float r = g.q[0], x = g.q[1], y = g.q[2], z = g.q[3];
    OUT(TEXGS_ACC_ROTATIONS, d_rots[4 * i + 0], 2.0f * (-z * dR[1] + y * dR[2] + z * dR[3] - x * dR[5] - y * dR[6] + x * dR[7]));
    OUT(TEXGS_ACC_ROTATIONS, d_rots[4 * i + 1], 2.0f * (y * dR[1] + z * dR[2] + y * dR[3] - 2.0f * x * dR[4] - r * dR[5] + z * dR[6] + r * dR[7] - 2.0f * x * dR[8]));
    OUT(TEXGS_ACC_ROTATIONS, d_rots[4 * i + 2], 2.0f * (-2.0f * y * dR[0] + x * dR[1] + r * dR[2] + x * dR[3] + z * dR[5] - r * dR[6] + z * dR[7] - 2.0f * y * dR[8]));
    OUT(TEXGS_ACC_ROTATIONS, d_rots[4 * i + 3], 2.0f * (-2.0f * z * dR[0] - r * dR[1] + x * dR[2] + r * dR[3] - 2.0f * z * dR[4] + y * dR[5] + x * dR[6] + y * dR[7]));
    }
#undef OUT
    }
    if (d_shs) {
        if (na == 0 || (live && !visible)) {
            if (live) for (int k = 0; k < row; ++k) s_sh[threadIdx.x * row + k] = 0.f;
        }
        __syncthreads();
        if (accumulate & TEXGS_ACC_SHS) sh_rows_out<K8_BLOCK, true>(d_shs + first, s_sh, count, vec);
        else sh_rows_out<K8_BLOCK, false>(d_shs + first, s_sh, count, vec);
    }
}

__global__ void __launch_bounds__(TG_BLOCK)
k_mark_visible(int N, const float* __restrict__ vm, const float* __restrict__ means, uint8_t* __restrict__ visible) {
    const int i = blockIdx.x * TG_BLOCK + threadIdx.x;
    if (i >= N) return;
    const float tz = vm[2] * means[3 * i] + vm[6] * means[3 * i + 1] + vm[10] * means[3 * i + 2] + vm[14];
    visible[i] = tz > TG_NEAR_Z ? 1 : 0;
}

}

void launch_preprocess_fwd(const CamConst& c, const TexGSFrame* f, const TexGSInputs* in, TexGSGeom* g, hipStream_t s) {
    if (c.N <= 0) return;
    const int blocks = (c.N + TG_BLOCK - 1) / TG_BLOCK;
    const size_t lds = (in->shs && c.sh_degree > 0) ? (size_t)TG_BLOCK * 3 * c.sh_coeffs * sizeof(float) : 0;
    int hdr_words = 0;
    uint32_t* hdr = bin_header_ptr(g, c.N, &hdr_words);
#define K1_LAUNCH(COV) hipLaunchKernelGGL(k_preprocess_fwd<COV>, dim3(blocks), dim3(TG_BLOCK), lds, s, c, f->viewmatrix, f->projmatrix, f->campos, \
                       in->means3D, in->shs, in->opacities, in->scales, in->rotations, in->uvs, in->gradient_uvs, in->color_offset, \
                       in->cov3D_precomp, reinterpret_cast<float4*>(g->rec_test), reinterpret_cast<float4*>(g->rec_shade), g->depth, g->radii, \
                       reinterpret_cast<uint2*>(g->rect), g->tiles_touched, bin_block_sums_ptr(g, c.N), hdr, hdr_words)
    if (in->cov3D_precomp) K1_LAUNCH(true); else K1_LAUNCH(false);
#undef K1_LAUNCH
}

void launch_preprocess_bwd(const CamConst& c, const TexGSFrame* f, const TexGSInputs* in, const TexGSGeom* g,
                           TexGSGrads* gr, hipStream_t s) {
    if (c.N <= 0) return;
    const int blocks = (c.N + K8_BLOCK - 1) / K8_BLOCK;
    const size_t lds = gr->dL_dshs ? (size_t)K8_BLOCK * 3 * c.sh_coeffs * sizeof(float) : 0;
#define K8_LAUNCH(COV) hipLaunchKernelGGL(k_preprocess_bwd<COV>, dim3(blocks), dim3(K8_BLOCK), lds, s, c, f->viewmatrix, f->projmatrix, f->campos, \
                       in->means3D, in->shs, in->opacities, in->scales, in->rotations, in->gradient_uvs, in->cov3D_precomp, \
                       g->radii, gr->acc, gr->dL_dmeans3D, gr->dL_dmeans2D, gr->dL_dshs, gr->dL_dopacities, gr->dL_dscales, \
                       gr->dL_drotations, gr->dL_duvs, gr->dL_dcolor_offset, gr->dL_dcov3D, gr->accumulate)
    if (in->cov3D_precomp) K8_LAUNCH(true); else K8_LAUNCH(false);
#undef K8_LAUNCH
}

void launch_mark_visible(const TexGSFrame* f, const float* means3D, uint8_t* visible, hipStream_t s) {
    if (f->num_gaussians <= 0) return;
    const int blocks = (f->num_gaussians + TG_BLOCK - 1) / TG_BLOCK;
    hipLaunchKernelGGL(k_mark_visible, dim3(blocks), dim3(TG_BLOCK), 0, s, f->num_gaussians, f->viewmatrix, means3D, visible);
}
```

texture-gs_amd/texgs/_lib.py:

```python
import ctypes as C
import os

_HERE = os.path.dirname(os.path.abspath(__file__))
LIB_PATH = os.environ.get("TEXGS_LIB") or os.path.join(os.path.dirname(_HERE), "libtexgs.so")

ABI_VERSION = 19
TILE = 16
REC_TEST_FLOATS = 8
REC_SHADE_FLOATS = 20
TEXBIN_RECORD_FLOATS = 4
RESV_WORDS = 192
ACC_FLOATS = 32
WANT_TEXTURE, WANT_GAUSSIANS, WANT_ALL = 1, 2, 3

_fp = C.c_void_p


class Frame(C.Structure):
    _fields_ = [("image_height", C.c_int32), ("image_width", C.c_int32), ("tanfovx", C.c_float),
                ("tanfovy", C.c_float), ("scale_modifier", C.c_float), ("sh_degree", C.c_int32),
                ("sh_coeffs", C.c_int32), ("tex_res", C.c_int32), ("num_gaussians", C.c_int32),
                ("debug", C.c_int32), ("bg", _fp), ("viewmatrix", _fp), ("projmatrix", _fp), ("campos", _fp)]


class Inputs(C.Structure):
    _fields_ = [("means3D", _fp), ("shs", _fp), ("opacities", _fp), ("scales", _fp), ("rotations", _fp),
                ("uvs", _fp), ("gradient_uvs", _fp), ("texture", _fp), ("color_offset", _fp), ("cov3D_precomp", _fp)]


class Geom(C.Structure):
    _fields_ = [("rec_test", _fp), ("rec_shade", _fp), ("depth", _fp), ("radii", _fp), ("rect", _fp), ("tiles_touched", _fp),
                ("offsets", _fp), ("scan_temp", _fp), ("scan_temp_bytes", C.c_size_t)]


class Binning(C.Structure):
    _fields_ = [("num_rendered", C.c_uint32), ("keys_unsorted", _fp), ("keys_sorted", _fp), ("point_list", _fp),
                ("ranges", _fp), ("tile_order", _fp), ("sort_temp", _fp), ("sort_temp_bytes", C.c_size_t)]


class Image(C.Structure):
    _fields_ = [("out_color", _fp), ("out_depth", _fp), ("out_norm", _fp), ("out_alpha", _fp),
                ("final_T", _fp), ("n_contrib", _fp), ("tex_bin_count", _fp),
                ("survivors", _fp), ("surv_qmask", _fp), ("surv_count", _fp), ("tex_bin_resv", _fp)]


class Grads(C.Structure):
    _fields_ = [("dL_dcolor", _fp), ("dL_ddepth", _fp), ("dL_dnorm", _fp), ("dL_dalpha", _fp), ("acc", _fp),
                ("dL_dmeans3D", _fp), ("dL_dmeans2D", _fp), ("dL_dshs", _fp), ("dL_dopacities", _fp),
                ("dL_dscales", _fp), ("dL_drotations", _fp), ("dL_duvs", _fp), ("dL_dtexture", _fp),
                ("dL_dcolor_offset", _fp), ("dL_dcov3D", _fp), ("want", C.c_uint32), ("tex_bins", _fp), ("tex_bin_cursor", _fp), ("tex_bin_base", _fp),
                ("tex_rec_cap", C.c_uint32),
                ("accumulate", C.c_int32)]


class UVNetStruct(C.Structure):
    _fields_ = [(n, _fp) for n in ("W1", "b1", "W2", "b2", "emb", "W3", "b3", "W4", "b4", "W5", "b5", "xyz_offset", "xyz_scale")] \
        + [("hidden", C.c_int32)]


class HashGridStruct(C.Structure):
    _fields_ = [("n_levels", C.c_int32), ("n_features", C.c_int32), ("log2_hashmap_size", C.c_int32), ("base_resolution", C.c_float),
                ("per_level_scale", C.c_float)]


HASHGRID_MAX_LEVELS = 16
HASHGRID_FEATURES = 4


class UVNetGradStruct(C.Structure):
    _fields_ = [(n, _fp) for n in ("dW1", "db1", "dW2", "db2", "dW3", "db3", "dW4", "db4", "dW5", "db5")]


DENSITY_KEEP, DENSITY_CLONE, DENSITY_CLONE_KEPT, DENSITY_SPLIT, DENSITY_CHILD = 1, 2, 4, 8, 16
DENSITY_ROW = {"copy": 0, "moment": 1, "scaling": 2, "xyz": 3}
DENSITY_MAX_ROWS = 24
METRICS_ROW = 16


class DensityPlanStruct(C.Structure):
    _fields_ = [("accum", _fp), ("denom", _fp), ("scaling", _fp), ("opacity", _fp), ("n", C.c_int32), ("max_grad", C.c_float),
                ("min_opacity", C.c_float), ("dense_scale", C.c_float), ("big_scale", C.c_float), ("densify", C.c_int32),
                ("use_big", C.c_int32)]


class DensityRowStruct(C.Structure):
    _fields_ = [("src", _fp), ("dst", _fp), ("width", C.c_int32), ("kind", C.c_int32)]


class DensityMoveStruct(C.Structure):
    _fields_ = [("row", DensityRowStruct * DENSITY_MAX_ROWS), ("rows", C.c_int32), ("n", C.c_int32), ("action", _fp), ("rank", _fp),
                ("n_kept", C.c_int32), ("n_clone", C.c_int32), ("n_split", C.c_int32), ("n_child", C.c_int32), ("scaling", _fp),
                ("rotation", _fp), ("noise", _fp)]


UV_PRECISION = {"fp32": 0, "bf16x3": 1, "mixed": 2}


EXPORTS = ["texgs_abi_version", "texgs_build_id", "texgs_last_error", "texgs_scan_temp_bytes", "texgs_sort_temp_bytes",
           "texgs_preprocess_forward", "texgs_num_rendered_words", "texgs_num_rendered_begin", "texgs_num_rendered_reduce", "texgs_depth_sort_scan", "texgs_bin_sort_render_forward",
           "texgs_render_forward", "texgs_backward", "texgs_backward_render", "texgs_backward_preprocess",
           "texgs_rgb_alpha_loss", "texgs_mark_visible", "texgs_profile_enable", "texgs_tex_bin_count",
           "texgs_profile_read", "texgs_profile_select", "texgs_selftest_waveops", "texgs_geom_losses", "texgs_norm_from_depth",
           "texgs_uv_packed_bytes", "texgs_uv_pack", "texgs_uv_taylor_packed", "texgs_uv_backward", "texgs_uv_backward_temp_bytes",
           "texgs_hashgrid_levels", "texgs_hashgrid_forward", "texgs_hashgrid_backward_temp_bytes", "texgs_hashgrid_backward",
           "texgs_chamfer_nn_temp_bytes", "texgs_chamfer_nn",
           "texgs_knn3_temp_bytes", "texgs_knn3_mean_dist2", "texgs_fps_temp_bytes", "texgs_farthest_points",
           "texgs_cube_sample", "texgs_cube_latlong", "texgs_cube_sample_backward", "texgs_cube_sample_nearest_backward",
           "texgs_density_stats", "texgs_density_plan_temp_bytes", "texgs_density_plan", "texgs_density_move",
           "texgs_eval_metrics_temp_bytes", "texgs_eval_metrics"]
KERNEL_NAMES = ["preprocess_fwd", "scan", "duplicate", "sort", "ranges", "render_fwd", "render_bwd", "preprocess_bwd",
                "texgrad_reduce"]

_lib = None


def load():
    global _lib
    if _lib is not None:
        return _lib
    if not os.path.exists(LIB_PATH):
        raise RuntimeError(
            f"libtexgs.so not found at {LIB_PATH}: build it with `python texture-gs_amd/build.py` "
            "(hipcc --offload-arch=gfx950). There is no CPU fallback for the rasterizer.")
    lib = C.CDLL(LIB_PATH)
    missing = [n for n in EXPORTS if not hasattr(lib, n)]
    if missing:
        raise RuntimeError(f"libtexgs.so at {LIB_PATH} does not export {', '.join(missing)}; rebuild it with "
                           "`python texture-gs_amd/build.py`")
    P = C.POINTER
    lib.texgs_abi_version.restype = C.c_int
    lib.texgs_last_error.restype = C.c_char_p
    lib.texgs_scan_temp_bytes.restype = C.c_size_t
    lib.texgs_scan_temp_bytes.argtypes = [C.c_int32]
    lib.texgs_sort_temp_bytes.restype = C.c_size_t
    lib.texgs_sort_temp_bytes.argtypes = [C.c_uint32, C.c_uint32]
    lib.texgs_tex_bin_count.restype = C.c_size_t
    lib.texgs_tex_bin_count.argtypes = [C.c_int32]
    lib.texgs_preprocess_forward.argtypes = [P(Frame), P(Inputs), P(Geom), C.c_void_p]
    lib.texgs_num_rendered_words.argtypes = [C.c_int32]
    lib.texgs_num_rendered_words.restype = C.c_size_t
    lib.texgs_num_rendered_begin.argtypes = [P(Geom), C.c_int32, C.c_void_p, C.c_size_t, C.c_int32, C.c_void_p]
    lib.texgs_num_rendered_begin.restype = C.c_int
    lib.texgs_num_rendered_reduce.argtypes = [C.c_void_p, C.c_int32, P(C.c_uint32), P(C.c_uint64)]
    lib.texgs_num_rendered_reduce.restype = C.c_int
    lib.texgs_depth_sort_scan.argtypes = [P(Geom), C.c_int32, C.c_void_p]
    lib.texgs_depth_sort_scan.restype = C.c_int
    lib.texgs_bin_sort_render_forward.argtypes = [P(Frame), P(Inputs), P(Geom), P(Binning), P(Image), C.c_void_p]
    lib.texgs_render_forward.argtypes = [P(Frame), P(Inputs), P(Geom), P(Binning), P(Image), C.c_void_p]
    lib.texgs_backward.argtypes = [P(Frame), P(Inputs), P(Geom), P(Binning), P(Image), P(Grads), C.c_void_p]
    lib.texgs_backward_render.argtypes = [P(Frame), P(Inputs), P(Geom), P(Binning), P(Image), P(Grads), C.c_void_p]
    lib.texgs_backward_preprocess.argtypes = [P(Frame), P(Inputs), P(Geom), P(Grads), C.c_void_p]
    lib.texgs_mark_visible.argtypes = [P(Frame), C.c_void_p, C.c_void_p, C.c_void_p]
    lib.texgs_rgb_alpha_loss.argtypes = [C.c_void_p, C.c_void_p, C.c_void_p, C.c_void_p, C.c_int32, C.c_int32, C.c_float,
                                         C.c_float, C.c_void_p, C.c_void_p, C.c_void_p, C.c_void_p, C.c_void_p]
    lib.texgs_rgb_alpha_loss.restype = C.c_int
    lib.texgs_geom_losses.argtypes = [C.c_void_p] * 6 + [C.c_int32, C.c_int32, C.c_float, C.c_float, C.c_float, C.c_float,
                                      C.c_void_p, C.c_void_p, C.c_void_p, C.c_void_p]
    lib.texgs_geom_losses.restype = C.c_int
    lib.texgs_norm_from_depth.argtypes = [C.c_void_p, C.c_void_p, C.c_float, C.c_float, C.c_int32, C.c_int32, C.c_float,
                                          C.c_void_p, C.c_void_p, C.c_void_p]
    lib.texgs_norm_from_depth.restype = C.c_int
    lib.texgs_uv_packed_bytes.argtypes = [C.c_int32]
    lib.texgs_uv_packed_bytes.restype = C.c_size_t
    lib.texgs_uv_pack.argtypes = [P(UVNetStruct), C.c_int32, C.c_void_p, C.c_void_p]
    lib.texgs_uv_pack.restype = C.c_int
    lib.texgs_uv_taylor_packed.argtypes = [P(UVNetStruct), C.c_int32, C.c_void_p, C.c_void_p, C.c_int32, C.c_void_p, C.c_void_p, C.c_void_p]
    lib.texgs_uv_taylor_packed.restype = C.c_int
    lib.texgs_uv_backward_temp_bytes.argtypes = [C.c_int32]
    lib.texgs_uv_backward_temp_bytes.restype = C.c_size_t
    lib.texgs_uv_backward.argtypes = [P(UVNetStruct), C.c_int32, C.c_void_p, C.c_void_p, C.c_int32, P(UVNetGradStruct), C.c_void_p, C.c_void_p]
    lib.texgs_uv_backward.restype = C.c_int
    lib.texgs_hashgrid_levels.argtypes = [P(HashGridStruct), C.c_void_p, C.c_void_p, C.c_void_p, C.c_void_p, P(C.c_uint32)]
    lib.texgs_hashgrid_levels.restype = C.c_int
    lib.texgs_hashgrid_forward.argtypes = [P(HashGridStruct), C.c_void_p, C.c_void_p, C.c_int32, C.c_void_p, C.c_void_p]
    lib.texgs_hashgrid_forward.restype = C.c_int
    lib.texgs_hashgrid_backward_temp_bytes.argtypes = [P(HashGridStruct), C.c_int32]
    lib.texgs_hashgrid_backward_temp_bytes.restype = C.c_size_t
    lib.texgs_hashgrid_backward.argtypes = [P(HashGridStruct), C.c_void_p, C.c_void_p, C.c_void_p, C.c_int32, C.c_void_p, C.c_void_p,
                                            C.c_void_p, C.c_void_p]
    lib.texgs_hashgrid_backward.restype = C.c_int
    lib.texgs_chamfer_nn_temp_bytes.argtypes = [C.c_int32]
    lib.texgs_chamfer_nn_temp_bytes.restype = C.c_size_t
    lib.texgs_chamfer_nn.argtypes = [C.c_void_p, C.c_int32, C.c_void_p, C.c_int32, C.c_void_p, C.c_void_p, C.c_void_p, C.c_void_p]
    lib.texgs_chamfer_nn.restype = C.c_int
    lib.texgs_knn3_temp_bytes.argtypes = [C.c_int32]
    lib.texgs_knn3_temp_bytes.restype = C.c_size_t
    lib.texgs_knn3_mean_dist2.argtypes = [C.c_void_p, C.c_int32, C.c_void_p, C.c_void_p, C.c_void_p]
    lib.texgs_knn3_mean_dist2.restype = C.c_int
    lib.texgs_fps_temp_bytes.argtypes = [C.c_int32, C.c_int32]
    lib.texgs_fps_temp_bytes.restype = C.c_size_t
    lib.texgs_farthest_points.argtypes = [C.c_void_p, C.c_int32, C.c_int32, C.c_int32, C.c_void_p, C.c_void_p, C.c_void_p]
    lib.texgs_farthest_points.restype = C.c_int
    lib.texgs_cube_sample.argtypes = [C.c_void_p, C.c_int32, C.c_int32, C.c_void_p, C.c_int32, C.c_int32, C.c_int32, C.c_void_p, C.c_void_p]
    lib.texgs_cube_sample.restype = C.c_int
    lib.texgs_cube_latlong.argtypes = [C.c_void_p, C.c_int32, C.c_int32, C.c_int32, C.c_int32, C.c_int32, C.c_void_p, C.c_void_p]
    lib.texgs_cube_latlong.restype = C.c_int
    lib.texgs_cube_sample_backward.argtypes = [C.c_void_p, C.c_int32, C.c_int32, C.c_void_p, C.c_int32, C.c_void_p, C.c_void_p, C.c_void_p,
                                               C.c_void_p]
    lib.texgs_cube_sample_backward.restype = C.c_int
    lib.texgs_cube_sample_nearest_backward.argtypes = [C.c_int32, C.c_int32, C.c_void_p, C.c_int32, C.c_void_p, C.c_void_p, C.c_void_p]
    lib.texgs_cube_sample_nearest_backward.restype = C.c_int
    lib.texgs_density_stats.argtypes = [C.c_void_p, C.c_void_p, C.c_int32, C.c_void_p, C.c_void_p, C.c_void_p, C.c_void_p]
    lib.texgs_density_stats.restype = C.c_int
    lib.texgs_density_plan_temp_bytes.argtypes = [C.c_int32]
    lib.texgs_density_plan_temp_bytes.restype = C.c_size_t
    lib.texgs_density_plan.argtypes = [P(DensityPlanStruct), C.c_void_p, C.c_void_p, C.c_void_p, C.c_void_p, C.c_void_p]
    lib.texgs_density_plan.restype = C.c_int
    lib.texgs_density_move.argtypes = [P(DensityMoveStruct), C.c_void_p]
    lib.texgs_density_move.restype = C.c_int
    lib.texgs_eval_metrics_temp_bytes.argtypes = [C.c_int32, C.c_int32]
    lib.texgs_eval_metrics_temp_bytes.restype = C.c_size_t
    lib.texgs_eval_metrics.argtypes = [C.c_void_p] * 5 + [C.c_int32, C.c_int32, C.c_int32, C.c_void_p, C.c_void_p, C.c_void_p]
    lib.texgs_eval_metrics.restype = C.c_int
    lib.texgs_selftest_waveops.argtypes = [C.c_void_p, C.c_void_p, C.c_void_p]
    lib.texgs_selftest_waveops.restype = C.c_int
    lib.texgs_profile_enable.argtypes = [C.c_int]
    lib.texgs_profile_enable.restype = C.c_int
    lib.texgs_profile_select.argtypes = [C.c_uint32]
    lib.texgs_profile_select.restype = C.c_int
    lib.texgs_profile_read.argtypes = [P(C.c_float), P(C.c_uint32)]
    lib.texgs_profile_read.restype = C.c_int
    for name in ("texgs_preprocess_forward", "texgs_bin_sort_render_forward",
                 "texgs_render_forward", "texgs_backward", "texgs_backward_render",
                 "texgs_backward_preprocess", "texgs_rgb_alpha_loss", "texgs_mark_visible"):
        getattr(lib, name).restype = C.c_int
    v = lib.texgs_abi_version()
    if v != ABI_VERSION:
        raise RuntimeError(f"libtexgs.so ABI version {v} != expected {ABI_VERSION}; rebuild it")
    lib.texgs_build_id.restype = C.c_char_p
    global BUILD_ID
    BUILD_ID = lib.texgs_build_id().decode()
    if not os.environ.get("TEXGS_LIB"):
        want = tree_build_id()
        if want is not None and BUILD_ID != want:
            raise RuntimeError(f"libtexgs.so was built from other sources (build id {BUILD_ID}, this tree is {want}); "
                               "rebuild it with `python texture-gs_amd/build.py`")
    _lib = lib
    return lib


BUILD_ID = None


def tree_build_id():
    import importlib.util
    path = os.path.join(os.path.dirname(_HERE), "build.py")
    if not os.path.exists(path):
        return None
    spec = importlib.util.spec_from_file_location("texgs_build_script", path)
    mod = importlib.util.module_from_spec(spec)
    spec.loader.exec_module(mod)
    return mod.build_id()


def check(rc, what):
    if rc != 0:
        msg = load().texgs_last_error().decode("utf-8", "replace")
        raise RuntimeError(f"{what} failed (code {rc}): {msg}")


def profile_enable(on: bool, only=None):
    mask = 0xFFFFFFFF if only is None else sum(1 << KERNEL_NAMES.index(n) for n in only)
    check(load().texgs_profile_select(mask), "texgs_profile_select")
    check(load().texgs_profile_enable(1 if on else 0), "texgs_profile_enable")


def profile_read():
    n = len(KERNEL_NAMES)
    ms = (C.c_float * n)()
    cnt = (C.c_uint32 * n)()
    check(load().texgs_profile_read(ms, cnt), "texgs_profile_read")
    return {KERNEL_NAMES[i]: (float(ms[i]), int(cnt[i])) for i in range(n)}
```

texture-gs_amd/texgs/multiview.py:

```python
from typing import List, Sequence

import torch


def shard_views(num_views: int, rank: int, world: int) -> List[int]:
    if not (0 <= rank < world):
        raise ValueError(f"rank {rank} outside world {world}")
    views = list(range(rank, num_views, world))
    if not views:
        raise ValueError(f"rank {rank} gets no view: {num_views} views over {world} ranks")
    return views


def lpt_shard_views(costs: Sequence[float], rank: int, world: int) -> List[int]:
    if not (0 <= rank < world):
        raise ValueError(f"rank {rank} outside world {world}")
    n = len(costs)
    if n < world:
        raise ValueError(f"{n} views over {world} ranks")
    order = sorted(range(n), key=lambda v: (-float(costs[v]), v))
    quota = [n // world + (1 if r < n % world else 0) for r in range(world)]
    load = [0.0] * world
    mine = [[] for _ in range(world)]
    for v in order:
        r = min((r for r in range(world) if len(mine[r]) < quota[r]), key=lambda r: (load[r], r))
        mine[r].append(v)
        load[r] += float(costs[v])
    return sorted(mine[rank])


class GradBucket:

    def __init__(self, params: Sequence[torch.Tensor]):
        self.params = [p for p in params if p is not None and p.requires_grad]
        if not self.params:
            raise ValueError("no parameter requires grad")
        dev = self.params[0].device
        total = sum(p.numel() for p in self.params)
        self.flat = torch.zeros(total, dtype=torch.float32, device=dev)
        off = 0
        self.slices = []
        for p in self.params:
            if p.dtype != torch.float32 or p.device != dev:
                raise ValueError("GradBucket needs float32 parameters on one device")
            n = p.numel()
            p.grad = self.flat[off:off + n].view_as(p)
            self.slices.append((off, n))
            off += n
        self.replicas = []
        self.active = 0
        self.before_accumulate = None

    def select(self, k: int):
        while len(self.replicas) < k:
            self.replicas.append(torch.zeros_like(self.flat))
        self.active = k

    def fold(self):
        self.active = 0
        for r in self.replicas:
            self.flat.add_(r)
            r.zero_()

    def sink_for(self, tensor):
        for p, (off, n) in zip(self.params, self.slices):
            if p is tensor:
                sl = self.flat[off:off + n]
                if p.grad is None:
                    sl.zero_()
                    p.grad = sl.view_as(p)
                elif p.grad.data_ptr() != self.flat.data_ptr() + 4 * off or not p.grad.is_contiguous():
                    return None
                return sl if self.active == 0 else self.replicas[self.active - 1][off:off + n]
        return None

    def zero(self):
        self.flat.zero_()
        for p, (off, n) in zip(self.params, self.slices):
            if p.grad is None or p.grad.data_ptr() != self.flat.data_ptr() + 4 * off:
                p.grad = self.flat[off:off + n].view_as(p)

    def segment_of(self, tensors) -> tuple:
        idx = sorted(i for i, p in enumerate(self.params) if any(p is t for t in tensors))
        if not idx or idx != list(range(idx[0], idx[-1] + 1)):
            raise ValueError("the tensors of a segment must be registered parameters that are adjacent in the bucket")
        off = self.slices[idx[0]][0]
        return off, self.slices[idx[-1]][0] + self.slices[idx[-1]][1] - off

    def all_reduce_async(self, dist, segment=None, after=(), timing=False, wire_dtype=None):
        off, n = segment if segment is not None else (0, self.flat.numel())
        buf = self.flat[off:off + n]
        if dist.get_backend() != "nccl" or not self.flat.is_cuda:
            for ev in after:
                ev.synchronize()
            self._reduce_now(dist, buf, wire_dtype)
            return self
        cur = torch.cuda.current_stream(self.flat.device)
        if getattr(self, "_comm", None) is None:
            self._comm = torch.cuda.Stream(self.flat.device)
            self._comm_events = []
        self._comm.wait_stream(cur)
        for ev in after:
            self._comm.wait_event(ev)
        with torch.cuda.stream(self._comm):
            e0 = e1 = None
            if timing:
                e0, e1 = torch.cuda.Event(enable_timing=True), torch.cuda.Event(enable_timing=True)
                e0.record(self._comm)
            if wire_dtype is None or wire_dtype == torch.float32:
                dist.all_reduce(buf, op=dist.ReduceOp.SUM)
                wire_bytes = n * 4
            else:
                stage = buf.to(wire_dtype)
                dist.all_reduce(stage, op=dist.ReduceOp.SUM)
                buf.copy_(stage)
                wire_bytes = n * stage.element_size()
            if timing:
                e1.record(self._comm)
                self._comm_events.append((wire_bytes, e0, e1))
        self._pending = True
        return self

    def wait(self):
        if getattr(self, "_pending", False):
            torch.cuda.current_stream(self.flat.device).wait_stream(self._comm)
            self._pending = False
        return self.flat

    def comm_timings(self):
        out = []
        for nbytes, e0, e1 in getattr(self, "_comm_events", []):
            e1.synchronize()
            out.append((nbytes, e0.elapsed_time(e1)))
        if getattr(self, "_comm_events", None):
            self._comm_events.clear()
        return out

    def _reduce_now(self, dist, buf, wire_dtype=None):
        wd = torch.float32 if wire_dtype is None else wire_dtype
        if buf.is_cuda:
            host = torch.empty(buf.shape, dtype=wd).pin_memory()
            host.copy_(buf, non_blocking=True)
            torch.cuda.current_stream(buf.device).synchronize()
            dist.all_reduce(host, op=dist.ReduceOp.SUM)
            buf.copy_(host, non_blocking=True)
        elif wd != torch.float32:
            stage = buf.to(wd)
            dist.all_reduce(stage, op=dist.ReduceOp.SUM)
            buf.copy_(stage)
        else:
            dist.all_reduce(buf, op=dist.ReduceOp.SUM)

    def all_reduce(self, dist, average_over: int = 0):
        if dist.get_backend() == "nccl":
            dist.all_reduce(self.flat, op=dist.ReduceOp.SUM)
        else:
            if self.flat.is_cuda:
                if getattr(self, "_host", None) is None:
                    self._host = torch.empty(self.flat.shape, dtype=torch.float32).pin_memory()
                self._host.copy_(self.flat, non_blocking=True)
                torch.cuda.current_stream(self.flat.device).synchronize()
                dist.all_reduce(self._host, op=dist.ReduceOp.SUM)
                self.flat.copy_(self._host, non_blocking=True)
            else:
                dist.all_reduce(self.flat, op=dist.ReduceOp.SUM)
        if average_over:
            self.flat.div_(float(average_over))
        return self.flat


class ViewPipeline:

    def __init__(self, device, depth: int = 2):
        if depth < 1:
            raise ValueError("depth must be >= 1")
        self.device = torch.device(device)
        self.streams = [torch.cuda.Stream(self.device) for _ in range(depth)] if depth > 1 else []

    def close(self):
        from . import rasterizer
        for s in self.streams:
            s.synchronize()
            rasterizer.release_scratch(self.device, s.cuda_stream)
        self.streams = []

    def __del__(self):
        try:
            self.close()
        except Exception:
            pass

    def run(self, views, forward_fn, backward_fn=None, sink=None, order="accumulate", texture_ready=None, prefetch_fn=None,
            prefetch_ahead=1):
        results = []
        views = list(views)
        if not self.streams:
            for i, v in enumerate(views):
                obj = forward_fn(v)
                if prefetch_fn is not None and i + 1 < len(views):
                    prefetch_fn(views[i + 1])
                if backward_fn is not None:
                    if texture_ready is not None and sink is not None and i == len(views) - 1:
                        sink.before_accumulate = lambda: texture_ready([])
                    try:
                        backward_fn(obj)
                    finally:
                        if sink is not None:
                            sink.before_accumulate = None
                results.append(obj)
            return results
        if order not in ("backward", "accumulate", "none"):
            raise ValueError(order)
        if sink is None and order != "backward":
            order = "backward"
        cur = torch.cuda.current_stream(self.device)
        for s in self.streams:
            s.wait_stream(cur)
        prev_bwd = None
        render_done = {}
        depth = len(self.streams)
        try:
            ahead = depth * max(1, int(prefetch_ahead))
            if prefetch_fn is not None:
                for i, v in enumerate(views[:ahead]):
                    with torch.cuda.stream(self.streams[i % depth]):
                        prefetch_fn(v)
            for i, v in enumerate(views):
                k = i % depth
                s = self.streams[k]
                with torch.cuda.stream(s):
                    if order == "none":
                        sink.select(k)
                    obj = forward_fn(v)
                    if prefetch_fn is not None and i + ahead < len(views):
                        prefetch_fn(views[i + ahead])
                    if backward_fn is not None:
                        if order == "backward" and prev_bwd is not None:
                            s.wait_event(prev_bwd)
                        if order == "accumulate":
                            last = i == len(views) - 1

                            def hook(ev=prev_bwd, s=s, k=k, last=last):
                                if texture_ready is not None:
                                    e = torch.cuda.Event()
                                    e.record(s)
                                    render_done[k] = e
                                    if last:
                                        texture_ready([render_done[j] for j in sorted(render_done)])
                                if ev is not None:
                                    s.wait_event(ev)
                            sink.before_accumulate = hook
                        backward_fn(obj)
                        prev_bwd = torch.cuda.Event()
                        prev_bwd.record(s)
                results.append(obj)
        finally:
            if sink is not None:
                sink.before_accumulate = None
            for s in self.streams:
                cur.wait_stream(s)
            if sink is not None and order == "none":
                sink.fold()
        return results
```

texture-gs_amd/texgs/rasterizer.py:

```python
import ctypes as C
import math
import os as _os
import threading as _threading
from collections import namedtuple
from types import SimpleNamespace
from typing import NamedTuple, Optional

import torch
from torch import nn

from . import _lib

USE_TEX_BINS = _os.environ.get("TEXGS_TEX_BINS", "1") != "0"
TEX_REC_CAP = int(_os.environ.get("TEXGS_REC_CAP", "0"))
DIRECT_LEAF_GRADS = _os.environ.get("TEXGS_DIRECT_LEAF_GRADS", "0") != "0"
TEX_REC_BYTES_MAX = int(float(_os.environ.get("TEXGS_BIN_GB_MAX", "4")) * (1 << 30))
_ACC_BITS = dict(means3D=1, means2D=2, shs=4, opacities=8, scales=16, rotations=32, uvs=64, color_offset=128, cov3D=256)


class GaussianRasterizationSettings(NamedTuple):
    image_height: int
    image_width: int
    tanfovx: float
    tanfovy: float
    bg: torch.Tensor
    scale_modifier: float
    viewmatrix: torch.Tensor
    projmatrix: torch.Tensor
    sh_degree: int
    campos: torch.Tensor
    prefiltered: bool
    debug: bool


def _ptr(t: Optional[torch.Tensor]):
    return None if t is None else t.data_ptr()


def _f32c(t: torch.Tensor, name: str, device) -> torch.Tensor:
    if not isinstance(t, torch.Tensor):
        raise TypeError(f"{name} must be a torch.Tensor")
    if t.device != device:
        raise ValueError(f"{name} is on {t.device}, expected {device}")
    if t.dtype != torch.float32:
        raise TypeError(f"{name} must be float32, got {t.dtype}")
    return t.contiguous()


class _Arena:

    def __init__(self, device):
        self.device, self.specs, self.size, self.buf = device, {}, 0, None

    def add(self, name, shape, dtype):
        off = (self.size + 255) & ~255
        self.specs[name] = (off, tuple(shape), dtype)
        self.size = off + math.prod(shape) * dtype.itemsize

    def commit(self):
        self.buf = torch.empty(max(self.size, 1), dtype=torch.uint8, device=self.device)

    def ptr(self, name):
        return self.buf.data_ptr() + self.specs[name][0] if name in self.specs else None

    def view(self, name):
        off, shape, dtype = self.specs[name]
        return self.buf[off:off + math.prod(shape) * dtype.itemsize].view(dtype).view(shape)


class _Tensors(dict):

    def __init__(self, arenas, **real):
        super().__init__(**real)
        self._arenas = arenas

    def __missing__(self, name):
        for ar in self._arenas:
            if name in ar.specs:
                self[name] = v = ar.view(name)
                return v
        self[name] = None
        return None

    def get(self, name, default=None):
        v = self[name]
        return default if v is None else v


GEOM_CACHE = _os.environ.get("TEXGS_GEOM_CACHE", "1") != "0"
_CAPACITY_HINT = {}
_GEOM = {}
_GeomEntry = namedtuple("_GeomEntry", "ints cam_key fingerprint D cap bin arenas handoff counts")
_GEOM_STATS = {"hits": 0, "misses": 0, "late_handoffs": 0}
_SERIAL = [0]
_LAST_DIFFERENTIATED = {}
_DROPPED = {}
_PRED_LOCK = _threading.RLock()


def unused_streak(dev_index):
    with _PRED_LOCK:
        last = _LAST_DIFFERENTIATED.get(dev_index, -1)
        return sum(1 for n in _DROPPED.get(dev_index, ()) if n > last)


def reset_handoff_predictor():
    with _PRED_LOCK:
        _LAST_DIFFERENTIATED.clear()
        _DROPPED.clear()


def geometry_cache_stats():
    return dict(_GEOM_STATS)


_SCRATCH = {}


def release_scratch(device=None, stream=None):
    for cache in (_SCRATCH, _GEOM, _PREFETCH):
        for key in list(cache):
            if (device is None or key[0] == torch.device(device).index) and (stream is None or key[1] == int(stream)):
                for _, fwd in (cache[key] if cache is _PREFETCH else ()):
                    fwd.abandon()
                del cache[key]


def scratch_bytes():
    total = 0
    for sc in _SCRATCH.values():
        if sc.acc is not None:
            total += sc.acc.numel() * 4
        if sc.bins is not None:
            total += sc.bins.nbytes()
    for e in _GEOM.values():
        total += sum(ar.buf.numel() for ar in e.arenas if ar is not None and ar.buf is not None)
    return total


class _TexBins:

    def __init__(self, lib, device, R):
        self.device, self.R = device, R
        self.nbins = int(lib.texgs_tex_bin_count(R))
        self.cursor = torch.zeros(self.nbins + 2, dtype=torch.int32, device=device)
        self.base = torch.empty(2 * self.nbins + 1, dtype=torch.int32, device=device)
        self.cap = 0
        self.rec = None
        self.host_stat = torch.zeros(1, dtype=torch.int32).pin_memory()
        self.event = None
        self.calls = 0

    def nbytes(self):
        return ((0 if self.rec is None else self.rec.numel()) + self.cursor.numel() + self.base.numel()) * 4

    def _resize(self, cap):
        cap = max(1024, min(int(cap), TEX_REC_BYTES_MAX // (4 * _lib.TEXBIN_RECORD_FLOATS)))
        if cap != self.cap:
            self.rec = None
            self.rec = torch.empty(cap * _lib.TEXBIN_RECORD_FLOATS, dtype=torch.float32, device=self.device)
            self.cap = cap

    def before_call(self, D, counts=None):
        if TEX_REC_CAP:
            self._resize(TEX_REC_CAP)
            return
        if self.rec is None and counts is not None and not torch.cuda.is_current_stream_capturing():
            self._resize(int(counts.sum().item() * 1.25) + 4096)
        if self.event is not None and self.event.query():
            self.event = None
            wanted = int(self.host_stat[0])
            if wanted > self.cap:
                self._resize(int(wanted * 1.25) + 4096)
        if self.rec is None:
            self._resize(24 * max(int(D), 1024))

    def after_call(self):
        self.calls += 1
        if self.event is None and not TEX_REC_CAP and (self.calls <= 4 or self.calls % 16 == 0):
            self.host_stat.copy_(self.cursor[self.nbins:self.nbins + 1], non_blocking=True)
            self.event = torch.cuda.Event()
            self.event.record(torch.cuda.current_stream(self.device))


class _State:
    __slots__ = ("frame", "inputs", "geom", "bin", "img", "tensors", "args", "N", "K", "R", "H", "W", "D", "cap", "tiles",
                 "want_counts", "lazy", "backward_ran", "shared_geometry", "serial", "__weakref__")

    def __init__(self, frame, inputs, geom, bin, img, tensors, args, D, cap, tiles, want_counts, lazy, shared_geometry):
        self.frame, self.inputs, self.geom, self.bin, self.img, self.tensors, self.args = frame, inputs, geom, bin, img, tensors, args
        self.N, self.K, self.R, self.H, self.W = args.N, args.K, args.R, frame.image_height, frame.image_width
        self.D, self.cap, self.tiles = D, cap, tiles
        self.want_counts, self.lazy, self.backward_ran, self.shared_geometry = want_counts, lazy, False, shared_geometry
        with _PRED_LOCK:
            _SERIAL[0] += 1
            self.serial = _SERIAL[0]

    def __del__(self):
        try:
            if getattr(self, "lazy", False) and not self.backward_ran:
                dev = self.args.means3D.device.index
                with _PRED_LOCK:
                    last = _LAST_DIFFERENTIATED.get(dev, -1)
                    _DROPPED[dev] = [n for n in _DROPPED.get(dev, []) if n > last][-8:] + [self.serial]
        except Exception:
            pass


def _make_frame(st: GaussianRasterizationSettings, N, K, R, device, keep):
    bg = _f32c(st.bg, "bg", device).reshape(-1)
    vm = _f32c(st.viewmatrix, "viewmatrix", device).reshape(-1)
    pm = _f32c(st.projmatrix, "projmatrix", device).reshape(-1)
    cp = _f32c(st.campos, "campos", device).reshape(-1)
    if bg.numel() != 3 or vm.numel() != 16 or pm.numel() != 16 or cp.numel() != 3:
        raise ValueError("bg/campos must have 3 elements and viewmatrix/projmatrix 16")
    keep.extend([bg, vm, pm, cp])
    return _lib.Frame(int(st.image_height), int(st.image_width), float(st.tanfovx), float(st.tanfovy), float(st.scale_modifier),
                      int(st.sh_degree), int(K), int(R), int(N), 1 if st.debug else 0, _ptr(bg), _ptr(vm), _ptr(pm), _ptr(cp))


_PREFETCH = {}
_PIN_POOL = {}


def _pin_take(words):
    pool = _PIN_POOL.setdefault(words, [])
    return pool.pop() if pool else torch.empty(max(words, 1), dtype=torch.int32).pin_memory()


def _pin_give(t):
    pool = _PIN_POOL.setdefault(t.numel(), [])
    if len(pool) < 16:
        pool.append(t)


def _prefetch_take(device, key):
    skey = (device.index, int(torch.cuda.current_stream(device).cuda_stream))
    lst = _PREFETCH.get(skey, ())
    for k, (key_k, fwd) in enumerate(lst):
        if key_k == key:
            del lst[k]
            if not lst:
                del _PREFETCH[skey]
            return fwd


_Args = namedtuple("_Args", "means3D shs opacities scales rotations uvs gradient_uvs texture color_offset cov3D_precomp N K R")
_HANDOFF = tuple(n for n, _ in _lib.Image._fields_[6:])


def _check_inputs(st, means3D, shs, opacities, scales, rotations, uvs, gradient_uvs, texture, color_offset=None, cov3D_precomp=None):
    device = means3D.device
    N = means3D.shape[0]
    means3D = _f32c(means3D, "means3D", device)
    if means3D.dim() != 2 or means3D.shape[1] != 3:
        raise ValueError("means3D must be [N,3]")
    opacities = _f32c(opacities, "opacities", device)
    if opacities.numel() != N:
        raise ValueError(f"per-Gaussian inputs must have exactly N rows (N={N}; opacities {tuple(opacities.shape)})")
    if cov3D_precomp is not None:
        if texture is not None:
            raise ValueError("cov3D_precomp is an input of the untextured surface only")
        cov3D_precomp = _f32c(cov3D_precomp, "cov3D_precomp", device)
        if cov3D_precomp.shape != (N, 6):
            raise ValueError(f"cov3D_precomp must be [N,6], got {tuple(cov3D_precomp.shape)}")
        scales = rotations = None
    else:
        scales = _f32c(scales, "scales", device)
        rotations = _f32c(rotations, "rotations", device)
        if scales.shape != (N, 3) or rotations.shape != (N, 4):
            raise ValueError("per-Gaussian inputs must have exactly N rows "
                             f"(N={N}; scales {tuple(scales.shape)}, rotations {tuple(rotations.shape)})")
    if texture is not None:
        uvs = _f32c(uvs, "uvs", device)
        gradient_uvs = _f32c(gradient_uvs, "gradient_uvs", device)
        texture = _f32c(texture, "texture", device)
        if uvs.shape != (N, 3) or gradient_uvs.numel() != 9 * N:
            raise ValueError("per-Gaussian inputs must have exactly N rows "
                             f"(N={N}; uvs {tuple(uvs.shape)}, gradient_uvs {tuple(gradient_uvs.shape)})")
        if texture.dim() != 4 or texture.shape[0] != 6 or texture.shape[1] != texture.shape[2] or texture.shape[3] != 3:
            raise ValueError(f"texture must be [6,R,R,3], got {tuple(texture.shape)}")
        R = texture.shape[1]
    else:
        uvs = gradient_uvs = None
        R = 1
    K = 0
    if shs is not None:
        shs = _f32c(shs, "shs", device)
        if shs.dim() != 3 or shs.shape[0] != N or shs.shape[2] != 3:
            raise ValueError(f"shs must be [N,K,3], got {tuple(shs.shape)}")
        K = shs.shape[1]
        if K > 15:
            raise ValueError("shs holds at most 15 view-dependent coefficients (degree 3)")
    if color_offset is not None:
        color_offset = _f32c(color_offset, "color_offset", device)
        if color_offset.shape != (N, 3):
            raise ValueError(f"color_offset must be [N,3], got {tuple(color_offset.shape)}")
    if int(st.sh_degree) < 0 or int(st.sh_degree) > 3:
        raise ValueError("sh_degree must be in [0,3]")
    return _Args(means3D, shs, opacities, scales, rotations, uvs, gradient_uvs, texture, color_offset, cov3D_precomp, N, K, R)


def _add_handoff(ar, cap, tiles, R, want_counts):
    if cap is not None:
        ar.add("survivors", (4 * max(cap, 1), 2), torch.int32)
        ar.add("surv_qmask", (4 * max(cap, 1),), torch.int16)
    if tiles is not None:
        ar.add("surv_count", (4 * tiles,), torch.int32)
        if want_counts:
            ar.add("tex_bin_count", (2 * int(_lib.load().texgs_tex_bin_count(R)),), torch.int32)
            ar.add("tex_bin_resv", (4 * tiles, _lib.RESV_WORDS), torch.int32)


class _Forward:

    def __init__(self, st, tensors, for_backward, count_bins, lazy):
        self.st, self.raw, self.flags = st, tensors, (for_backward, count_bins, lazy)

    def key(self):
        t = lambda x: None if x is None else (x.data_ptr(), x._version, tuple(x.shape), x.requires_grad)
        st = self.st
        return (int(st.image_height), int(st.image_width), float(st.tanfovx), float(st.tanfovy), float(st.scale_modifier), int(st.sh_degree),
                bool(st.debug), t(st.bg), t(st.viewmatrix), t(st.projmatrix), t(st.campos)) + tuple(t(x) for x in self.raw) + self.flags

    def begin(self):
        lib, st = _lib.load(), self.st
        a = self.args = _check_inputs(st, *self.raw)
        for_backward, count_bins, lazy = self.flags
        device, N = a.means3D.device, a.N
        if count_bins is None:
            count_bins = for_backward
        self.handoff = bool(for_backward) and not (lazy and unused_streak(device.index) >= 2)
        self.want_counts = bool(count_bins and for_backward and a.texture is not None and USE_TEX_BINS)
        H, W = int(st.image_height), int(st.image_width)
        self.tiles = ((W + _lib.TILE - 1) // _lib.TILE) * ((H + _lib.TILE - 1) // _lib.TILE)
        cur_stream = torch.cuda.current_stream(device)
        stream = self.stream = cur_stream.cuda_stream
        self.keep = list(a[:10])
        with torch.cuda.device(device):
            self.frame = _make_frame(st, N, a.K, a.R, device, self.keep)
            self.inputs = _lib.Inputs(*map(_ptr, a[:10]))
            i32, f32, u8, n1 = torch.int32, torch.float32, torch.uint8, max(N, 1)
            self.gints = (N, H, W, a.R if a.texture is not None else 0, float(st.tanfovx), float(st.tanfovy), float(st.scale_modifier),
                          a.cov3D_precomp is not None)
            self.cam_key = tuple((t.data_ptr(), t._version) for t in (st.viewmatrix, st.projmatrix, st.campos))
            gkey = self.gkey = (device.index, int(stream))
            entry = _GEOM.get(gkey) if GEOM_CACHE else None
            if entry is not None and not (entry.ints == self.gints and entry.cam_key == self.cam_key):
                del _GEOM[gkey]
                entry = None
            self.entry = entry
            scan_bytes = lib.texgs_scan_temp_bytes(N)
            fix = self.fix = _Arena(device)
            fix.add("rec", (n1, _lib.REC_TEST_FLOATS), f32)
            fix.add("rec_shade", (n1, _lib.REC_SHADE_FLOATS), f32)
            fix.add("depth", (n1,), f32)
            fix.add("rect", (n1, 2), i32)
            fix.add("tiles_touched", (n1,), i32)
            fix.add("offsets", (n1,), i32)
            fix.add("scan_temp", (scan_bytes,), u8)
            fix.add("final_T", (H, W), f32)
            fix.add("n_contrib", (H, W), i32)
            if entry is None:
                self._add_lists(fix)
            fix.commit()
            radii = torch.empty(N, dtype=i32, device=device)
            self.geom = _lib.Geom(fix.ptr("rec"), fix.ptr("rec_shade"), fix.ptr("depth"), _ptr(radii), fix.ptr("rect"),
                                  fix.ptr("tiles_touched"), fix.ptr("offsets"), fix.ptr("scan_temp"), scan_bytes)
            self.outs = (torch.empty(3, H, W, dtype=f32, device=device), torch.empty(1, H, W, dtype=f32, device=device),
                         torch.empty(3, H, W, dtype=f32, device=device), torch.empty(1, H, W, dtype=f32, device=device), radii)
            self.img = _lib.Image(*map(_ptr, self.outs[:4]), fix.ptr("final_T"), fix.ptr("n_contrib"), None, None, None, None, None)
            self.hint_key = (device.index, N, H, W)
            self.cap = _CAPACITY_HINT.get(self.hint_key, max(4 * N, 1024))
            self.binning = self.bin_ar = None
            if entry is None:
                self._alloc_bin(self.cap, fix)
            refs = self.refs = [C.byref(x) for x in (self.frame, self.inputs, self.geom)]
            _lib.check(lib.texgs_preprocess_forward(*refs, stream), "texgs_preprocess_forward")
            pin = self.pin = _pin_take(int(lib.texgs_num_rendered_words(N)))
            _lib.check(lib.texgs_num_rendered_begin(refs[2], N, pin.data_ptr(), pin.numel(), 0, stream), "texgs_num_rendered_begin")
            self.d_ev = torch.cuda.Event()
            self.d_ev.record(cur_stream)
            if entry is None:
                _lib.check(lib.texgs_depth_sort_scan(refs[2], N, stream), "texgs_depth_sort_scan")
        return self

    def _add_lists(self, ar):
        ar.add("ranges", (self.tiles, 2), torch.int32)
        ar.add("tile_order", (self.tiles,), torch.int32)
        if self.handoff:
            _add_handoff(ar, None, self.tiles, self.args.R, self.want_counts)

    def _alloc_bin(self, cap, lists_ar):
        c1, tiles = max(cap, 1), self.tiles
        sort_bytes = _lib.load().texgs_sort_temp_bytes(cap, tiles)
        ar = self.bin_ar = _Arena(self.fix.device)
        ar.add("keys_unsorted", (c1,), torch.int64)
        ar.add("keys_sorted", (c1,), torch.int64)
        ar.add("point_list", (c1,), torch.int32)
        ar.add("sort_temp", (sort_bytes,), torch.uint8)
        if lists_ar is None:
            self._add_lists(ar)
        if self.handoff:
            _add_handoff(ar, cap, None, self.args.R, self.want_counts)
        ar.commit()
        la = lists_ar if lists_ar is not None else ar
        self.binning = _lib.Binning(0, ar.ptr("keys_unsorted"), ar.ptr("keys_sorted"), ar.ptr("point_list"), la.ptr("ranges"),
                                    la.ptr("tile_order"), ar.ptr("sort_temp"), sort_bytes)
        for n in _HANDOFF:
            setattr(self.img, n, (ar if n in ar.specs else la).ptr(n))

    def finish(self):
        lib, a, img, entry, refs = _lib.load(), self.args, self.img, self.entry, self.refs
        for_backward, _, lazy = self.flags
        stream, cap, pin = self.stream, self.cap, self.pin
        with torch.cuda.device(a.means3D.device):
            self.d_ev.synchronize()
            d_host, fp_host = C.c_uint32(0), C.c_uint64(0)
            _lib.check(lib.texgs_num_rendered_reduce(pin.data_ptr(), a.N, C.byref(d_host), C.byref(fp_host)), "texgs_num_rendered_reduce")
            _pin_give(pin)
            D, fp = int(d_host.value), int(fp_host.value)
            shared = entry is not None and fp == entry.fingerprint and D == entry.D
            if shared:
                _GEOM_STATS["hits"] += 1
                binning, cap = _lib.Binning(D, *entry.bin), entry.cap
                _lib.check(lib.texgs_render_forward(*refs, C.byref(binning), C.byref(img), stream), "texgs_render_forward")
                if for_backward and entry.handoff and (entry.counts or not self.want_counts):
                    img.survivors, img.surv_qmask, img.surv_count = entry.handoff
                    img.tex_bin_count, img.tex_bin_resv = entry.counts if self.want_counts else (None, None)
            else:
                _GEOM_STATS["misses"] += 1
                grown = int(D * 1.25) + 1024
                if entry is not None:
                    cap = max(cap, grown)
                    self._alloc_bin(cap, None)
                    _lib.check(lib.texgs_depth_sort_scan(refs[2], a.N, stream), "texgs_depth_sort_scan")
                elif D > cap:
                    cap = grown
                    self._alloc_bin(cap, self.fix)
                binning = self.binning
                binning.num_rendered = D
                _lib.check(lib.texgs_bin_sort_render_forward(*refs, C.byref(binning), C.byref(img), stream), "texgs_bin_sort_render_forward")
                _CAPACITY_HINT[self.hint_key] = max(_CAPACITY_HINT.get(self.hint_key, 0), grown)
                if GEOM_CACHE:
                    _GEOM[self.gkey] = _GeomEntry(
                        self.gints, self.cam_key, fp, D, cap, tuple(getattr(binning, n) for n, _ in _lib.Binning._fields_[1:]),
                        (self.fix, self.bin_ar), (img.survivors, img.surv_qmask, img.surv_count) if self.handoff else None,
                        (img.tex_bin_count, img.tex_bin_resv) if (self.handoff and img.tex_bin_count) else None)
        arenas = (self.fix,) + ((self.bin_ar,) if self.bin_ar is not None else ()) + (tuple(entry.arenas) if shared else ())
        tensors = _Tensors(arenas, keep=self.keep, radii=self.outs[4], for_backward=bool(for_backward))
        for n in _HANDOFF:
            if getattr(img, n) is None:
                tensors[n] = None
        return self.outs, _State(self.frame, self.inputs, self.geom, binning, img, tensors, a, D, cap, self.tiles, self.want_counts,
                                 bool(lazy and for_backward), shared)

    def abandon(self):
        self.d_ev.synchronize()
        _pin_give(self.pin)


def _gpu_only(device):
    _lib.load()
    if device.type != "cuda":
        raise RuntimeError("the textured rasterizer runs on an AMD GPU (torch device 'cuda' = HIP); "
                           f"got tensors on {device}. There is no CPU fallback.")


def prefetch_forward(st, means3D, shs, opacities, scales, rotations, uvs, gradient_uvs, texture, color_offset=None,
                     for_backward=True, cov3D_precomp=None, count_bins=None, lazy=False):
    device = means3D.device
    _gpu_only(device)
    fwd = _Forward(st, (means3D, shs, opacities, scales, rotations, uvs, gradient_uvs, texture, color_offset, cov3D_precomp),
                   for_backward, count_bins, lazy).begin()
    lst = _PREFETCH.setdefault((device.index, int(torch.cuda.current_stream(device).cuda_stream)), [])
    lst.append((fwd.key(), fwd))
    for _, old in lst[:-4]:
        old.abandon()
    del lst[:-4]


def forward_raw(st, means3D, shs, opacities, scales, rotations, uvs, gradient_uvs, texture, color_offset=None,
                for_backward=True, cov3D_precomp=None, count_bins=None, lazy=False):
    _gpu_only(means3D.device)
    fwd = _Forward(st, (means3D, shs, opacities, scales, rotations, uvs, gradient_uvs, texture, color_offset, cov3D_precomp),
                   for_backward, count_bins, lazy)
    pend = _prefetch_take(means3D.device, fwd.key()) if _PREFETCH else None
    return (pend or fwd.begin()).finish()


def _late_handoff(s: _State):
    lib = _lib.load()
    device = s.args.means3D.device
    stream = torch.cuda.current_stream(device).cuda_stream
    ar = _Arena(device)
    _add_handoff(ar, s.cap, s.tiles, s.R, s.want_counts)
    ar.add("scratch_out", (8, s.H, s.W), torch.float32)
    ar.add("final_T", (s.H, s.W), torch.float32)
    ar.add("n_contrib", (s.H, s.W), torch.int32)
    ar.commit()
    so = ar.ptr("scratch_out")
    hw = 4 * s.H * s.W
    img = _lib.Image(so, so + 3 * hw, so + 4 * hw, so + 7 * hw, ar.ptr("final_T"), ar.ptr("n_contrib"), *(ar.ptr(n) for n in _HANDOFF))
    _lib.check(lib.texgs_render_forward(C.byref(s.frame), C.byref(s.inputs), C.byref(s.geom), C.byref(s.bin), C.byref(img), stream),
               "texgs_render_forward (late hand-off)")
    s.tensors._arenas = tuple(s.tensors._arenas) + (ar,)
    for n in _HANDOFF:
        setattr(s.img, n, ar.ptr(n))
        s.tensors.pop(n, None)
        if n not in ar.specs:
            s.tensors[n] = None
    _GEOM_STATS["late_handoffs"] += 1


def _plan_outputs(N, K, textured, has_cov, has_coff, want, sinks, device):
    shapes = {}
    if want & _lib.WANT_GAUSSIANS:
        shapes = dict(means3D=(N, 3), means2D=(N, 3), opacities=(N, 1))
        if has_cov:
            shapes["cov3D"] = (N, 6)
        else:
            shapes.update(scales=(N, 3), rotations=(N, 4))
        if textured:
            shapes["uvs"] = (N, 3)
        if K > 0:
            shapes["shs"] = (N, K, 3)
        if has_coff:
            shapes["color_offset"] = (N, 3)
    fresh = [n for n in shapes if n not in sinks]
    sizes = [math.prod(shapes[n]) for n in fresh]
    flat = torch.empty(sum(sizes), dtype=torch.float32, device=device).split(sizes) if fresh else ()
    outs, mask = {n: v.view(shapes[n]) for n, v in zip(fresh, flat)}, 0
    for n in shapes.keys() - set(fresh):
        t = outs[n] = sinks[n]
        assert t.dtype == torch.float32 and t.is_contiguous() and t.numel() == math.prod(shapes[n]), n
        mask |= _ACC_BITS[n]
    return outs, mask, {n: (None if n in sinks else outs[n]) for n in shapes}


def backward_raw(s: _State, dL_dcolor, dL_ddepth, dL_dnorm, dL_dalpha, sinks=None, before_accumulate=None,
                 want=_lib.WANT_ALL):
    lib = _lib.load()
    if not s.tensors["for_backward"]:
        raise RuntimeError("this forward ran with for_backward=False (no survivor lists were kept): its backward cannot run")
    a = s.args
    device = a.means3D.device
    f32 = dict(dtype=torch.float32, device=device)
    N, R = s.N, s.R
    stream = torch.cuda.current_stream(device).cuda_stream
    textured = a.texture is not None
    want &= _lib.WANT_ALL if textured else _lib.WANT_GAUSSIANS
    want_g, want_t = bool(want & _lib.WANT_GAUSSIANS), bool(want & _lib.WANT_TEXTURE)
    if not want:
        return (None,) * 8

    def g(t, shape):
        if t is None:
            return None
        t = t.to(torch.float32).contiguous()
        assert tuple(t.shape) == shape, (tuple(t.shape), shape)
        return t
    dc, dd, dn, da = g(dL_dcolor, (3, s.H, s.W)), g(dL_ddepth, (1, s.H, s.W)), g(dL_dnorm, (3, s.H, s.W)), g(dL_dalpha, (1, s.H, s.W))
    with torch.cuda.device(device):
        if s.img.survivors is None:
            _late_handoff(s)
        s.backward_ran = True
        if s.lazy:
            with _PRED_LOCK:
                _LAST_DIFFERENTIATED[device.index] = max(_LAST_DIFFERENTIATED.get(device.index, -1), s.serial)
        skey = (device.index, int(stream))
        sc = _SCRATCH.pop(skey, None) or SimpleNamespace(acc=None, bins=None)
        if want_g and (sc.acc is None or sc.acc.shape[0] < max(N, 1)):
            sc.acc = torch.zeros(max(N, 1), _lib.ACC_FLOATS, **f32)
        acc = sc.acc if want_g else None
        sinks = sinks or {}
        outs, mask, res = _plan_outputs(N, s.K, textured, a.cov3D_precomp is not None, a.color_offset is not None, want, sinks, device)
        tex_sink = sinks.get("texture") if want_t else None
        d_tex = (tex_sink if tex_sink is not None else torch.zeros(6, R, R, 3, **f32)) if want_t else None
        bins = None
        if want_t and USE_TEX_BINS and s.tensors.get("tex_bin_count") is not None:
            bins = sc.bins if (sc.bins is not None and sc.bins.R == R) else _TexBins(lib, device, R)
            sc.bins = None
            bins.before_call(s.D, s.tensors.get("tex_bin_count"))
        grads = _lib.Grads(_ptr(dc), _ptr(dd), _ptr(dn), _ptr(da), _ptr(acc), _ptr(outs.get("means3D")), _ptr(outs.get("means2D")),
                           _ptr(outs.get("shs")), _ptr(outs.get("opacities")), _ptr(outs.get("scales")), _ptr(outs.get("rotations")),
                           _ptr(outs.get("uvs")), _ptr(d_tex), _ptr(outs.get("color_offset")), _ptr(outs.get("cov3D")), want,
                           _ptr(bins.rec) if bins else None, _ptr(bins.cursor) if bins else None,
                           _ptr(bins.base) if bins else None, bins.cap if bins else 0, mask)
        refs = [C.byref(x) for x in (s.frame, s.inputs, s.geom, s.bin, s.img, grads)]
        if before_accumulate is None:
            _lib.check(lib.texgs_backward(*refs, stream), "texgs_backward")
        else:
            _lib.check(lib.texgs_backward_render(*refs, stream), "texgs_backward_render")
            before_accumulate()
            _lib.check(lib.texgs_backward_preprocess(*refs[:3], refs[5], stream), "texgs_backward_preprocess")
    if bins is not None:
        bins.after_call()
        sc.bins = bins
    _SCRATCH[skey] = sc
    s.tensors["d_color_offset"] = res.get("color_offset")
    s.tensors["d_cov3D"] = res.get("cov3D")
    return tuple(res.get(n) for n in ("means3D", "means2D", "shs", "opacities", "scales", "rotations", "uvs")) \
        + (None if tex_sink is not None else d_tex,)


def _leaf_grad_sink(t):
    if t is None or not (t.is_leaf and t.requires_grad):
        return None
    if getattr(t, "_backward_hooks", None) or getattr(t, "_post_accumulate_grad_hooks", None):
        return None
    gr = t.grad
    if gr is None or gr.dtype != torch.float32 or not gr.is_contiguous() or gr.shape != t.shape or gr.device != t.device:
        return None
    return gr


_ARG = dict(means3D=0, means2D=1, shs=2, opacities=3, scales=4, rotations=5, uvs=6, gradient_uvs=7, texture=8, st=9,
            color_offset=10, grad_sink=11, cov3D_precomp=12)
_GAUSSIAN_ARGS = ("means3D", "means2D", "shs", "opacities", "scales", "rotations", "uvs", "color_offset", "cov3D_precomp")


class _RasterizeGaussians(torch.autograd.Function):
    @staticmethod
    def forward(ctx, means3D, means2D, shs, opacities, scales, rotations, uvs, gradient_uvs, texture, st, color_offset=None,
                grad_sink=None, cov3D_precomp=None):
        ctx.grad_sink = grad_sink
        ctx.set_materialize_grads(False)
        ctx.named = dict(means3D=means3D, means2D=means2D, shs=shs, opacities=opacities, scales=scales,
                         rotations=rotations, uvs=uvs, texture=texture, color_offset=color_offset, cov3D=cov3D_precomp)
        nig = tuple(ctx.needs_input_grad) + (False,) * len(_ARG)
        want = (_lib.WANT_TEXTURE if (texture is not None and nig[_ARG["texture"]]) else 0) \
            | (_lib.WANT_GAUSSIANS if any(nig[_ARG[n]] for n in _GAUSSIAN_ARGS) else 0)
        ctx.want = want
        ctx.nargs = len(ctx.needs_input_grad)
        outs, state = forward_raw(st, means3D, shs, opacities, scales, rotations, uvs, gradient_uvs, texture, color_offset,
                                  for_backward=bool(want), cov3D_precomp=cov3D_precomp,
                                  count_bins=bool(want & _lib.WANT_TEXTURE), lazy=True)
        color, depth, norm, alpha, radii = outs
        ctx.state = state
        ctx.versions = [(t, t._version) for t in state.tensors["keep"] if t is not None]
        ctx.op_shape = opacities.shape
        ctx.mark_non_differentiable(radii)
        return color, depth, norm, alpha, radii

    @staticmethod
    def backward(ctx, dL_dcolor, dL_ddepth, dL_dnorm, dL_dalpha, _dradii):
        s = ctx.state
        if s is None:
            raise RuntimeError("the rasterizer's backward ran a second time: its per-call state was released after the "
                               "first backward (retain_graph=True is not supported); run the forward again")
        for t, v in ctx.versions:
            if t._version != v:
                raise RuntimeError("an input of the rasterizer was modified in place between its forward and backward "
                                   "(the backward re-reads inputs through saved pointers); clone it before modifying")
        sinks, bucket = {}, False
        if ctx.grad_sink is not None:
            sinks = {k: g for k, g in ((k, ctx.grad_sink.sink_for(v)) for k, v in ctx.named.items() if v is not None)
                     if g is not None}
            bucket = bool(sinks)
        if not bucket and DIRECT_LEAF_GRADS:
            sinks = {k: g for k, g in ((k, _leaf_grad_sink(v)) for k, v in ctx.named.items()) if g is not None}
        d_means3D, d_means2D, d_shs, d_op, d_scales, d_rot, d_uvs, d_tex = backward_raw(
            s, dL_dcolor, dL_ddepth, dL_dnorm, dL_dalpha, sinks=sinks or None,
            before_accumulate=getattr(ctx.grad_sink, "before_accumulate", None) if bucket else None, want=ctx.want)
        d_coff = s.tensors.get("d_color_offset")
        d_cov = s.tensors.get("d_cov3D")
        ctx.state = None
        ctx.versions = None
        ctx.named = None
        if d_op is not None:
            d_op = d_op.reshape(ctx.op_shape)
        return (d_means3D, d_means2D, d_shs, d_op, d_scales, d_rot, d_uvs, None, d_tex, None, d_coff, None, d_cov)[:ctx.nargs]


EXTRA_ATTRS_MAX = 32


def blend_extra_attrs(st, means3D, means2D, opacities, scales, rotations, extra_attrs, grad_sink=None, cov3D_precomp=None):
    N = means3D.shape[0]
    if not isinstance(extra_attrs, torch.Tensor) or extra_attrs.dim() != 2 or extra_attrs.shape[0] != N:
        raise ValueError(f"extra_attrs must be a [N, C] tensor with N = {N} rows")
    C_ = int(extra_attrs.shape[1])
    if C_ > EXTRA_ATTRS_MAX:
        raise ValueError(f"extra_attrs has {C_} channels; at most {EXTRA_ATTRS_MAX} are blended")
    H, W = int(st.image_height), int(st.image_width)
    ea = extra_attrs.to(torch.float32)
    if C_ == 0 or N == 0:
        return torch.zeros(C_, H, W, dtype=torch.float32, device=means3D.device) + 0.0 * ea.sum()
    m = ea.detach().amin() - 1.0
    st0 = st._replace(bg=torch.zeros_like(st.bg), sh_degree=0)
    if means2D is None:
        means2D = torch.zeros_like(means3D)
    outs = []
    for c0 in range(0, C_, 3):
        grp = ea[:, c0:c0 + 3]
        if grp.shape[1] < 3:
            grp = torch.cat([grp, (m + 1.0).expand(N, 3 - grp.shape[1])], dim=1)
        color, _, _, alpha, _ = _RasterizeGaussians.apply(means3D, means2D, None, opacities, scales, rotations, None, None, None, st0,
                                                          ((grp - m) - 0.5).contiguous(), grad_sink, cov3D_precomp)
        outs.append(color + m * alpha)
    return torch.cat(outs, dim=0)[:C_]


class GaussianRasterizer(nn.Module):

    def __init__(self, raster_settings: GaussianRasterizationSettings, grad_sink=None):
        super().__init__()
        self.raster_settings = raster_settings
        self.grad_sink = grad_sink

    def markVisible(self, positions):
        lib = _lib.load()
        st = self.raster_settings
        positions = _f32c(positions, "positions", positions.device)
        N = positions.shape[0]
        keep = []
        frame = _make_frame(st, N, 0, 1, positions.device, keep)
        vis = torch.zeros(N, dtype=torch.uint8, device=positions.device)
        stream = torch.cuda.current_stream(positions.device).cuda_stream
        with torch.cuda.device(positions.device):
            _lib.check(lib.texgs_mark_visible(C.byref(frame), positions.data_ptr(), vis.data_ptr(), stream),
                       "texgs_mark_visible")
        return vis.bool()

    def prefetch(self, means3D, means2D, opacities, shs=None, scales=None, rotations=None, uvs=None,
                 gradient_uvs=None, texture=None, extra_attrs=None):
        grad = torch.is_grad_enabled()
        rg = lambda t: bool(grad and t is not None and t.requires_grad)
        want_tex = rg(texture)
        want_g = any(rg(t) for t in (means3D, means2D, shs, opacities, scales, rotations, uvs))
        prefetch_forward(self.raster_settings, means3D, shs, opacities, scales, rotations, uvs, gradient_uvs, texture, None,
                         for_backward=want_tex or want_g, cov3D_precomp=None, count_bins=want_tex, lazy=True)

    def forward(self, means3D, means2D, opacities, shs=None, scales=None, rotations=None, uvs=None,
                gradient_uvs=None, texture=None, extra_attrs=None):
        st = self.raster_settings
        if scales is None or rotations is None:
            raise ValueError("scales and rotations are required (the textured operator has no cov3D_precomp path)")
        if uvs is None or gradient_uvs is None or texture is None:
            raise ValueError("uvs, gradient_uvs and texture are required")
        if means2D is None:
            means2D = torch.zeros_like(means3D)
        color, depth, norm, alpha, radii = _RasterizeGaussians.apply(
            means3D, means2D, shs, opacities, scales, rotations, uvs, gradient_uvs, texture, st, None, self.grad_sink)
        extra = None
        if extra_attrs is not None:
            extra = blend_extra_attrs(st, means3D, means2D, opacities, scales, rotations, extra_attrs, self.grad_sink)
        return color, depth, norm, alpha, radii, extra
```

Before: 1014 views/s.

## Batch per-view preprocess backward into one grouped kernel over several views

Adds a grouped preprocess-backward entry point that processes up to 8 views' per-Gaussian accumulators in one kernel launch. Each thread reads the shared Gaussian inputs once and sums the per-view gradients before writing the outputs once, instead of one read-modify-write pass over all N Gaussians per view. On the Python side, backward passes in accumulate mode are deferred into a group with a separate accumulator buffer per view, and the group is flushed at the end. This cuts repeated HBM traffic on the gradient outputs. The cost is per-view accumulator buffers, extra cross-stream event ordering, and a single flush that serializes the views at the end.

```diff
diff --git a/include/texgs.h b/include/texgs.h
--- a/include/texgs.h
+++ b/include/texgs.h
@@ -152,6 +152,15 @@
 int texgs_backward_preprocess(const TexGSFrame* frame, const TexGSInputs* in, const TexGSGeom* geom, TexGSGrads* grads,
                               void* stream);
 
+#define TEXGS_K8_GROUP_MAX 8
+typedef struct TexGSGroupView {
+    const TexGSFrame* frame;
+    const TexGSGeom*  geom;
+    float*            acc;
+} TexGSGroupView;
+int texgs_backward_preprocess_group(const TexGSInputs* in, TexGSGrads* grads, const TexGSGroupView* views, int32_t num_views,
+                                    void* stream);
+
 enum {
     TEXGS_K_PREPROCESS_FWD = 0, TEXGS_K_SCAN = 1, TEXGS_K_DUPLICATE = 2, TEXGS_K_SORT = 3, TEXGS_K_RANGES = 4,
     TEXGS_K_RENDER_FWD = 5, TEXGS_K_RENDER_BWD = 6, TEXGS_K_PREPROCESS_BWD = 7, TEXGS_K_TEXGRAD_REDUCE = 8,
diff --git a/texture-gs_amd/csrc/abi.hip b/texture-gs_amd/csrc/abi.hip
--- a/texture-gs_amd/csrc/abi.hip
+++ b/texture-gs_amd/csrc/abi.hip
@@ -226,6 +226,45 @@
     const CamConst c = make_cam(frame);
     { ProfScope p(TEXGS_K_PREPROCESS_BWD, s); launch_preprocess_bwd(c, frame, in, geom, grads, s); }
     return check(frame, s, "preprocess_bwd");
+}
+
+int texgs_backward_preprocess_group(const TexGSInputs* in, TexGSGrads* grads, const TexGSGroupView* views, int32_t num_views,
+                                    void* stream) {
+    if (!in || !grads || !views) return fail_msg("NULL argument");
+    if (num_views < 1) return fail_msg("texgs_backward_preprocess_group: num_views must be >= 1");
+    int debug = 0;
+    for (int v = 0; v < num_views; ++v) {
+        if (!views[v].frame || !views[v].geom) return fail_msg("texgs_backward_preprocess_group: a view's frame or geom is NULL");
+        if (int r = validate_frame(views[v].frame)) return r;
+        if (views[v].frame->num_gaussians != views[0].frame->num_gaussians)
+            return fail_msg("texgs_backward_preprocess_group: num_gaussians differs between the views");
+        if (views[v].frame->sh_coeffs != views[0].frame->sh_coeffs)
+            return fail_msg("texgs_backward_preprocess_group: sh_coeffs differs between the views");
+        debug |= views[v].frame->debug;
+    }
+    if (!(grads->want & TEXGS_WANT_GAUSSIANS)) return 0;
+    if (in->cov3D_precomp || in->color_offset || grads->dL_dcov3D || grads->dL_dcolor_offset)
+        return fail_msg("texgs_backward_preprocess_group: cov3D_precomp / color_offset are not supported (call texgs_backward_preprocess per view)");
+    if (views[0].frame->sh_coeffs < 0 || views[0].frame->sh_coeffs > 15)
+        return fail_msg("texgs_backward_preprocess_group: sh_coeffs must be in [0, 15]");
+    if (views[0].frame->num_gaussians == 0) return 0;
+    if (!in->means3D || !in->opacities || !in->scales || !in->rotations) return fail_msg("per-Gaussian input pointer is NULL");
+    if (grads->dL_dshs && !in->shs) return fail_msg("texgs_backward_preprocess_group: dL_dshs without shs");
+    if (!grads->dL_dmeans3D || !grads->dL_dmeans2D || !grads->dL_dopacities || !grads->dL_dscales || !grads->dL_drotations)
+        return fail_msg("texgs_backward_preprocess_group: dL_dmeans3D, dL_dmeans2D, dL_dopacities, dL_dscales and dL_drotations are required");
+    const int planned = TEXGS_ACC_MEANS3D | TEXGS_ACC_MEANS2D | TEXGS_ACC_OPACITIES | TEXGS_ACC_SCALES | TEXGS_ACC_ROTATIONS
+                      | (grads->dL_duvs ? TEXGS_ACC_UVS : 0) | (grads->dL_dshs ? TEXGS_ACC_SHS : 0);
+    if ((grads->accumulate & planned) != planned)
+        return fail_msg("texgs_backward_preprocess_group: the accumulate bit of every output must be set (the views are added into the outputs)");
+    for (int v = 0; v < num_views; ++v) {
+        if (!views[v].acc || !views[v].geom->radii) return fail_msg("texgs_backward_preprocess_group: a view's acc or radii is NULL");
+        for (int u = 0; u < v; ++u)
+            if (views[u].acc == views[v].acc) return fail_msg("texgs_backward_preprocess_group: two views share an accumulator buffer");
+    }
+    hipStream_t s = (hipStream_t)stream;
+    { ProfScope p(TEXGS_K_PREPROCESS_BWD, s); launch_preprocess_bwd_group(in, grads, views, num_views, s); }
+    TexGSFrame f0; memset(&f0, 0, sizeof(f0)); f0.debug = debug;
+    return check(&f0, s, "preprocess_bwd_group");
 }
 
 int texgs_backward(const TexGSFrame* frame, const TexGSInputs* in, const TexGSGeom* geom,
diff --git a/texture-gs_amd/csrc/common.h b/texture-gs_amd/csrc/common.h
--- a/texture-gs_amd/csrc/common.h
+++ b/texture-gs_amd/csrc/common.h
@@ -46,6 +46,8 @@
 void launch_preprocess_fwd(const CamConst& c, const TexGSFrame* f, const TexGSInputs* in, TexGSGeom* g, hipStream_t s);
 void launch_preprocess_bwd(const CamConst& c, const TexGSFrame* f, const TexGSInputs* in, const TexGSGeom* g,
                            TexGSGrads* gr, hipStream_t s);
+void launch_preprocess_bwd_group(const TexGSInputs* in, const TexGSGrads* gr, const TexGSGroupView* views, int num_views,
+                                 hipStream_t s);
 void launch_mark_visible(const TexGSFrame* f, const float* means3D, uint8_t* visible, hipStream_t s);
 int  launch_depth_sort_scan(const TexGSGeom* g, int N, hipStream_t s);
 uint32_t* bin_block_sums_ptr(const TexGSGeom* g, int N);
diff --git a/texture-gs_amd/csrc/preprocess.hip b/texture-gs_amd/csrc/preprocess.hip
--- a/texture-gs_amd/csrc/preprocess.hip
+++ b/texture-gs_amd/csrc/preprocess.hip
@@ -1,4 +1,5 @@
 #include "common.h"
+#include <string.h>
 
 namespace {
 
@@ -414,6 +415,184 @@
 #ifndef K8_BLOCK
 #define K8_BLOCK 256
 #endif
+
+struct K8Part {
+    float op, phi[3], vd[3];
+    float m2[2];
+    float dm[3], dscale[3], dq[4];
+    float dS[9];
+};
+
+template <bool COV, class SHOut>
+__device__ __forceinline__ void k8_view(K8Part& o, const CamConst& C, const Frame& F, int gi,
+                                        const float* __restrict__ means, const float* __restrict__ scales,
+                                        const float* __restrict__ rots, const float* __restrict__ juv,
+                                        const float* __restrict__ cov6, float op, float* __restrict__ acc_row,
+                                        const float* sp, int na, SHOut&& sh_out) {
+    Geo g;
+    geo_forward<COV>(g, F, C, gi, means, scales, rots, juv, cov6);
+    float A[24];
+    {
+        float Mo[TEXGS_ACC_FLOATS];
+        float4* ap = reinterpret_cast<float4*>(acc_row);
+#pragma unroll
+        for (int k = 0; k < TEXGS_ACC_FLOATS / 4; ++k) {
+            const float4 v = ap[k];
+            Mo[4 * k] = v.x; Mo[4 * k + 1] = v.y; Mo[4 * k + 2] = v.z; Mo[4 * k + 3] = v.w;
+            ap[k] = make_float4(0.f, 0.f, 0.f, 0.f);
+        }
+        const float ca = g.conic[0], cb = g.conic[1], cc = g.conic[2];
+        const float m00 = Mo[M_P], m10 = Mo[M_P + 1], m01 = Mo[M_P + 2];
+        const float N00 = Mo[M_DN], N10 = Mo[M_DN + 3], N20 = Mo[M_DN + 6], D0 = Mo[M_DEN];
+        A[R_XY]     = -(ca * m10 + cb * m01) - ((g.G[0] * N00 + g.G[2] * N10 + g.G[4] * N20) + g.gx * D0);
+        A[R_XY + 1] = -(cc * m01 + cb * m10) - ((g.G[1] * N00 + g.G[3] * N10 + g.G[5] * N20) + g.gy * D0);
+        A[R_CONIC] = -0.5f * Mo[M_P + 3]; A[R_CONIC + 1] = -Mo[M_P + 4]; A[R_CONIC + 2] = -0.5f * Mo[M_P + 5];
+        A[R_OP] = (op > 0.0f) ? m00 / op : 0.0f;
+        A[R_G2] = Mo[M_DEN + 1]; A[R_G2 + 1] = Mo[M_DEN + 2];
+#pragma unroll
+        for (int cidx = 0; cidx < 3; ++cidx) {
+            A[R_GM + 2 * cidx] = Mo[M_DN + 3 * cidx + 1]; A[R_GM + 2 * cidx + 1] = Mo[M_DN + 3 * cidx + 2];
+            A[R_PHI + cidx] = Mo[M_PHI + cidx]; A[R_VD + cidx] = Mo[M_VD + cidx]; A[R_N + cidx] = Mo[M_N + cidx];
+        }
+        A[R_DEPTH] = Mo[M_DEPTH];
+    }
+    const float tx = g.t[0], ty = g.t[1], tz = g.t[2];
+    float dt[3] = {0.f, 0.f, 0.f};
+    float dm[3] = {0.f, 0.f, 0.f};
+    float dR[9];
+#pragma unroll
+    for (int k = 0; k < 9; ++k) dR[k] = 0.f;
+
+    o.op = A[R_OP];
+#pragma unroll
+    for (int k = 0; k < 3; ++k) { o.phi[k] = A[R_PHI + k]; o.vd[k] = A[R_VD + k]; }
+
+    const float dA = A[R_CONIC], dB = A[R_CONIC + 1], dC = A[R_CONIC + 2];
+    const float inv = g.inv, inv2 = inv * inv;
+    const float da = dA * (-g.c * g.c * inv2) + dB * (g.b * g.c * inv2) + dC * (inv - g.a * g.c * inv2);
+    const float db = dA * (2.0f * g.b * g.c * inv2) + dB * (-inv - 2.0f * g.b * g.b * inv2) + dC * (2.0f * g.a * g.b * inv2);
+    const float dc = dA * (inv - g.a * g.c * inv2) + dB * (g.a * g.b * inv2) + dC * (-g.a * g.a * inv2);
+    const float hb = 0.5f * db;
+    const float* S = g.S;
+    float TS0[3], TS1[3];
+    TS0[0] = g.T0[0] * S[0] + g.T0[1] * S[1] + g.T0[2] * S[2];
+    TS0[1] = g.T0[0] * S[1] + g.T0[1] * S[3] + g.T0[2] * S[4];
+    TS0[2] = g.T0[0] * S[2] + g.T0[1] * S[4] + g.T0[2] * S[5];
+    TS1[0] = g.T1[0] * S[0] + g.T1[1] * S[1] + g.T1[2] * S[2];
+    TS1[1] = g.T1[0] * S[1] + g.T1[1] * S[3] + g.T1[2] * S[4];
+    TS1[2] = g.T1[0] * S[2] + g.T1[1] * S[4] + g.T1[2] * S[5];
+    float dT0[3], dT1[3];
+#pragma unroll
+    for (int k = 0; k < 3; ++k) {
+        dT0[k] = 2.0f * (da * TS0[k] + hb * TS1[k]);
+        dT1[k] = 2.0f * (hb * TS0[k] + dc * TS1[k]);
+    }
+    float* dS = o.dS;
+#pragma unroll
+    for (int k = 0; k < 3; ++k)
+#pragma unroll
+        for (int l = 0; l < 3; ++l)
+            dS[k * 3 + l] = g.T0[k] * g.T0[l] * da + (g.T0[k] * g.T1[l] + g.T1[k] * g.T0[l]) * hb + g.T1[k] * g.T1[l] * dc;
+    float dM[9];
+#pragma unroll
+    for (int rr = 0; rr < 3; ++rr)
+#pragma unroll
+        for (int cc = 0; cc < 3; ++cc)
+            dM[rr * 3 + cc] = 2.0f * (dS[rr * 3 + 0] * g.M[0 * 3 + cc] + dS[rr * 3 + 1] * g.M[1 * 3 + cc] + dS[rr * 3 + 2] * g.M[2 * 3 + cc]);
+#pragma unroll
+    for (int cc = 0; cc < 3; ++cc) {
+        o.dscale[cc] = (dM[0 + cc] * g.R[0 + cc] + dM[3 + cc] * g.R[3 + cc] + dM[6 + cc] * g.R[6 + cc]) * C.scale_modifier;
+#pragma unroll
+        for (int rr = 0; rr < 3; ++rr) dR[rr * 3 + cc] += dM[rr * 3 + cc] * g.s[cc];
+    }
+    const float dJ00 = dT0[0] * WR(F, 0, 0) + dT0[1] * WR(F, 0, 1) + dT0[2] * WR(F, 0, 2);
+    const float dJ02 = dT0[0] * WR(F, 2, 0) + dT0[1] * WR(F, 2, 1) + dT0[2] * WR(F, 2, 2);
+    const float dJ11 = dT1[0] * WR(F, 1, 0) + dT1[1] * WR(F, 1, 1) + dT1[2] * WR(F, 1, 2);
+    const float dJ12 = dT1[0] * WR(F, 2, 0) + dT1[1] * WR(F, 2, 1) + dT1[2] * WR(F, 2, 2);
+    const float tz2 = tz * tz, tz3 = tz2 * tz;
+    dt[2] += -dJ00 * C.fx / tz2 - dJ11 * C.fy / tz2 + 2.0f * dJ02 * C.fx * g.txc / tz3 + 2.0f * dJ12 * C.fy * g.tyc / tz3;
+    if (!g.clx) dt[0] += -dJ02 * C.fx / tz2;
+    if (!g.cly) dt[1] += -dJ12 * C.fy / tz2;
+
+    const float dndx = A[R_XY] * 0.5f * (float)C.W, dndy = A[R_XY + 1] * 0.5f * (float)C.H;
+    o.m2[0] = dndx; o.m2[1] = dndy;
+    {
+        const float dhx = dndx * g.pw, dhy = dndy * g.pw;
+        const float dhw = -(dndx * g.hx + dndy * g.hy) * g.pw * g.pw;
+#pragma unroll
+        for (int k = 0; k < 3; ++k) dm[k] += dhx * F.P[k * 4 + 0] + dhy * F.P[k * 4 + 1] + dhw * F.P[k * 4 + 3];
+    }
+    dt[2] += A[R_DEPTH];
+    float dn[3] = {A[R_N], A[R_N + 1], A[R_N + 2]};
+
+    if (!g.degen) {
+        const float* dG = &A[R_GM];
+        float dBm[6];
+#pragma unroll
+        for (int k = 0; k < 3; ++k)
+#pragma unroll
+            for (int cc = 0; cc < 2; ++cc)
+                dBm[k * 2 + cc] = g.K[0 * 3 + k] * dG[0 * 2 + cc] + g.K[1 * 3 + k] * dG[1 * 2 + cc] + g.K[2 * 3 + k] * dG[2 * 2 + cc];
+        float dtz = dBm[0] / C.fx + dBm[3] / C.fy;
+        float dgt[2];
+#pragma unroll
+        for (int cc = 0; cc < 2; ++cc)
+            dgt[cc] = A[R_G2 + cc] - (dBm[0 * 2 + cc] * tx + dBm[1 * 2 + cc] * ty + dBm[2 * 2 + cc] * tz);
+#pragma unroll
+        for (int k = 0; k < 3; ++k) dt[k] -= dBm[k * 2 + 0] * g.gx + dBm[k * 2 + 1] * g.gy;
+        const float dax = dgt[0] / C.fx, day = dgt[1] / C.fy;
+        const float dot_a_nv = dax * g.nv[0] + day * g.nv[1];
+        dtz += dot_a_nv / g.sdot;
+        float dnv[3] = {tz * dax / g.sdot, tz * day / g.sdot, 0.f};
+        const float ds = -tz * dot_a_nv / (g.sdot * g.sdot);
+        dnv[0] += ds * tx; dnv[1] += ds * ty; dnv[2] += ds * tz;
+        dt[0] += ds * g.nv[0]; dt[1] += ds * g.nv[1]; dt[2] += ds * g.nv[2] + dtz;
+#pragma unroll
+        for (int k = 0; k < 3; ++k)
+            dn[k] += dnv[0] * WR(F, 0, k) + dnv[1] * WR(F, 1, k) + dnv[2] * WR(F, 2, k);
+    }
+#pragma unroll
+    for (int k = 0; k < 3; ++k) {
+        const float on = (g.kmin == k) ? g.sign : 0.0f;
+        dR[0 + k] += on * dn[0]; dR[3 + k] += on * dn[1]; dR[6 + k] += on * dn[2];
+    }
+
+    if (na > 0) {
+        float b[15], bx[15], by[15], bz[15];
+#pragma unroll
+        for (int k = 0; k < 15; ++k) { b[k] = 0.f; bx[k] = 0.f; by[k] = 0.f; bz[k] = 0.f; }
+        sh_basis(C.sh_degree, g.dir[0], g.dir[1], g.dir[2], b);
+        sh_basis_grad(C.sh_degree, g.dir[0], g.dir[1], g.dir[2], bx, by, bz);
+        const float v0 = A[R_VD], v1 = A[R_VD + 1], v2 = A[R_VD + 2];
+        float ddx = 0.f, ddy = 0.f, ddz = 0.f;
+#pragma unroll
+        for (int k = 0; k < 15; ++k) {
+            if (k < na) {
+                const float w = sp[3 * k + 0] * v0 + sp[3 * k + 1] * v1 + sp[3 * k + 2] * v2;
+                ddx += bx[k] * w; ddy += by[k] * w; ddz += bz[k] * w;
+                sh_out(k, b[k] * v0, b[k] * v1, b[k] * v2);
+            }
+        }
+        const float dd = g.dir[0] * ddx + g.dir[1] * ddy + g.dir[2] * ddz;
+        dm[0] += (ddx - g.dir[0] * dd) / g.dlen;
+        dm[1] += (ddy - g.dir[1] * dd) / g.dlen;
+        dm[2] += (ddz - g.dir[2] * dd) / g.dlen;
+    }
+
+#pragma unroll
+    for (int k = 0; k < 3; ++k) o.dm[k] = dm[k] + (dt[0] * F.V[k * 4 + 0] + dt[1] * F.V[k * 4 + 1] + dt[2] * F.V[k * 4 + 2]);
+
+    if constexpr (!COV) {
+    const float r = g.q[0], x = g.q[1], y = g.q[2], z = g.q[3];
+    o.dq[0] = 2.0f * (-z * dR[1] + y * dR[2] + z * dR[3] - x * dR[5] - y * dR[6] + x * dR[7]);
+    o.dq[1] = 2.0f * (y * dR[1] + z * dR[2] + y * dR[3] - 2.0f * x * dR[4] - r * dR[5] + z * dR[6] + r * dR[7] - 2.0f * x * dR[8]);
+    o.dq[2] = 2.0f * (-2.0f * y * dR[0] + x * dR[1] + r * dR[2] + x * dR[3] + z * dR[5] - r * dR[6] + z * dR[7] - 2.0f * y * dR[8]);
+    o.dq[3] = 2.0f * (-2.0f * z * dR[0] - r * dR[1] + x * dR[2] + r * dR[3] - 2.0f * z * dR[4] + y * dR[5] + x * dR[6] + y * dR[7]);
+    } else {
+        o.dq[0] = o.dq[1] = o.dq[2] = o.dq[3] = 0.f;
+    }
+}
+
 template <bool COV>
 __global__ void __launch_bounds__(K8_BLOCK)
 k_preprocess_bwd(CamConst C, const float* __restrict__ vm, const float* __restrict__ pm, const float* __restrict__ cp,
@@ -454,176 +633,26 @@
     if (visible) {
 #define OUT(BIT, P, V) do { if (accumulate & (BIT)) (P) += (V); else (P) = (V); } while (0)
     const Frame F = load_frame(vm, pm, cp);
-    Geo g;
-    geo_forward<COV>(g, F, C, i, means, scales, rots, juv, cov6);
-    float A[24];
-    {
-        float Mo[TEXGS_ACC_FLOATS];
-        float4* ap = reinterpret_cast<float4*>(acc + (size_t)i * TEXGS_ACC_FLOATS);
-#pragma unroll
-        for (int k = 0; k < TEXGS_ACC_FLOATS / 4; ++k) {
-            const float4 v = ap[k];
-            Mo[4 * k] = v.x; Mo[4 * k + 1] = v.y; Mo[4 * k + 2] = v.z; Mo[4 * k + 3] = v.w;
-            ap[k] = make_float4(0.f, 0.f, 0.f, 0.f);
-        }
-        const float ca = g.conic[0], cb = g.conic[1], cc = g.conic[2];
-        const float m00 = Mo[M_P], m10 = Mo[M_P + 1], m01 = Mo[M_P + 2];
-        const float N00 = Mo[M_DN], N10 = Mo[M_DN + 3], N20 = Mo[M_DN + 6], D0 = Mo[M_DEN];
-        A[R_XY]     = -(ca * m10 + cb * m01) - ((g.G[0] * N00 + g.G[2] * N10 + g.G[4] * N20) + g.gx * D0);
-        A[R_XY + 1] = -(cc * m01 + cb * m10) - ((g.G[1] * N00 + g.G[3] * N10 + g.G[5] * N20) + g.gy * D0);
-        A[R_CONIC] = -0.5f * Mo[M_P + 3]; A[R_CONIC + 1] = -Mo[M_P + 4]; A[R_CONIC + 2] = -0.5f * Mo[M_P + 5];
-        const float op = opac[i];
-        A[R_OP] = (op > 0.0f) ? m00 / op : 0.0f;
-        A[R_G2] = Mo[M_DEN + 1]; A[R_G2 + 1] = Mo[M_DEN + 2];
-#pragma unroll
-        for (int cidx = 0; cidx < 3; ++cidx) {
-            A[R_GM + 2 * cidx] = Mo[M_DN + 3 * cidx + 1]; A[R_GM + 2 * cidx + 1] = Mo[M_DN + 3 * cidx + 2];
-            A[R_PHI + cidx] = Mo[M_PHI + cidx]; A[R_VD + cidx] = Mo[M_VD + cidx]; A[R_N + cidx] = Mo[M_N + cidx];
-        }
-        A[R_DEPTH] = Mo[M_DEPTH];
-    }
-    const float tx = g.t[0], ty = g.t[1], tz = g.t[2];
-    float dt[3] = {0.f, 0.f, 0.f};
-    float dm[3] = {0.f, 0.f, 0.f};
-    float dR[9];
-#pragma unroll
-    for (int k = 0; k < 9; ++k) dR[k] = 0.f;
-
-    OUT(TEXGS_ACC_OPACITIES, d_op[i], A[R_OP]);
-    if (d_uvs) { OUT(TEXGS_ACC_UVS, d_uvs[3 * i + 0], A[R_PHI]); OUT(TEXGS_ACC_UVS, d_uvs[3 * i + 1], A[R_PHI + 1]); OUT(TEXGS_ACC_UVS, d_uvs[3 * i + 2], A[R_PHI + 2]); }
-    if (d_coff) { OUT(TEXGS_ACC_COLOR_OFFSET, d_coff[3 * i + 0], A[R_VD]); OUT(TEXGS_ACC_COLOR_OFFSET, d_coff[3 * i + 1], A[R_VD + 1]); OUT(TEXGS_ACC_COLOR_OFFSET, d_coff[3 * i + 2], A[R_VD + 2]); }
-
-    const float dA = A[R_CONIC], dB = A[R_CONIC + 1], dC = A[R_CONIC + 2];
-    const float inv = g.inv, inv2 = inv * inv;
-    const float da = dA * (-g.c * g.c * inv2) + dB * (g.b * g.c * inv2) + dC * (inv - g.a * g.c * inv2);
-    const float db = dA * (2.0f * g.b * g.c * inv2) + dB * (-inv - 2.0f * g.b * g.b * inv2) + dC * (2.0f * g.a * g.b * inv2);
-    const float dc = dA * (inv - g.a * g.c * inv2) + dB * (g.a * g.b * inv2) + dC * (-g.a * g.a * inv2);
-    const float hb = 0.5f * db;
-    const float* S = g.S;
-    float TS0[3], TS1[3];
-    TS0[0] = g.T0[0] * S[0] + g.T0[1] * S[1] + g.T0[2] * S[2];
-    TS0[1] = g.T0[0] * S[1] + g.T0[1] * S[3] + g.T0[2] * S[4];
-    TS0[2] = g.T0[0] * S[2] + g.T0[1] * S[4] + g.T0[2] * S[5];
-    TS1[0] = g.T1[0] * S[0] + g.T1[1] * S[1] + g.T1[2] * S[2];
-    TS1[1] = g.T1[0] * S[1] + g.T1[1] * S[3] + g.T1[2] * S[4];
-    TS1[2] = g.T1[0] * S[2] + g.T1[1] * S[4] + g.T1[2] * S[5];
-    float dT0[3], dT1[3];
-#pragma unroll
-    for (int k = 0; k < 3; ++k) {
-        dT0[k] = 2.0f * (da * TS0[k] + hb * TS1[k]);
-        dT1[k] = 2.0f * (hb * TS0[k] + dc * TS1[k]);
-    }
-    float dS[9];
-#pragma unroll
-    for (int k = 0; k < 3; ++k)
-#pragma unroll
-        for (int l = 0; l < 3; ++l)
-            dS[k * 3 + l] = g.T0[k] * g.T0[l] * da + (g.T0[k] * g.T1[l] + g.T1[k] * g.T0[l]) * hb + g.T1[k] * g.T1[l] * dc;
-    float dM[9];
-#pragma unroll
-    for (int rr = 0; rr < 3; ++rr)
-#pragma unroll
-        for (int cc = 0; cc < 3; ++cc)
-            dM[rr * 3 + cc] = 2.0f * (dS[rr * 3 + 0] * g.M[0 * 3 + cc] + dS[rr * 3 + 1] * g.M[1 * 3 + cc] + dS[rr * 3 + 2] * g.M[2 * 3 + cc]);
-    float dscale[3];
-#pragma unroll
-    for (int cc = 0; cc < 3; ++cc) {
-        dscale[cc] = (dM[0 + cc] * g.R[0 + cc] + dM[3 + cc] * g.R[3 + cc] + dM[6 + cc] * g.R[6 + cc]) * C.scale_modifier;
-#pragma unroll
-        for (int rr = 0; rr < 3; ++rr) dR[rr * 3 + cc] += dM[rr * 3 + cc] * g.s[cc];
-    }
-    const float dJ00 = dT0[0] * WR(F, 0, 0) + dT0[1] * WR(F, 0, 1) + dT0[2] * WR(F, 0, 2);
-    const float dJ02 = dT0[0] * WR(F, 2, 0) + dT0[1] * WR(F, 2, 1) + dT0[2] * WR(F, 2, 2);
-    const float dJ11 = dT1[0] * WR(F, 1, 0) + dT1[1] * WR(F, 1, 1) + dT1[2] * WR(F, 1, 2);
-    const float dJ12 = dT1[0] * WR(F, 2, 0) + dT1[1] * WR(F, 2, 1) + dT1[2] * WR(F, 2, 2);
-    const float tz2 = tz * tz, tz3 = tz2 * tz;
-    dt[2] += -dJ00 * C.fx / tz2 - dJ11 * C.fy / tz2 + 2.0f * dJ02 * C.fx * g.txc / tz3 + 2.0f * dJ12 * C.fy * g.tyc / tz3;
-    if (!g.clx) dt[0] += -dJ02 * C.fx / tz2;
-    if (!g.cly) dt[1] += -dJ12 * C.fy / tz2;
-
-    const float dndx = A[R_XY] * 0.5f * (float)C.W, dndy = A[R_XY + 1] * 0.5f * (float)C.H;
-    OUT(TEXGS_ACC_MEANS2D, d_means2D[3 * i + 0], dndx); OUT(TEXGS_ACC_MEANS2D, d_means2D[3 * i + 1], dndy); if (!(accumulate & TEXGS_ACC_MEANS2D)) d_means2D[3 * i + 2] = 0.f;
-    {
-        const float dhx = dndx * g.pw, dhy = dndy * g.pw;
-        const float dhw = -(dndx * g.hx + dndy * g.hy) * g.pw * g.pw;
-#pragma unroll
-        for (int k = 0; k < 3; ++k) dm[k] += dhx * F.P[k * 4 + 0] + dhy * F.P[k * 4 + 1] + dhw * F.P[k * 4 + 3];
-    }
-    dt[2] += A[R_DEPTH];
-    float dn[3] = {A[R_N], A[R_N + 1], A[R_N + 2]};
-
-    if (!g.degen) {
-        const float* dG = &A[R_GM];
-        float dBm[6];
-#pragma unroll
-        for (int k = 0; k < 3; ++k)
-#pragma unroll
-            for (int cc = 0; cc < 2; ++cc)
-                dBm[k * 2 + cc] = g.K[0 * 3 + k] * dG[0 * 2 + cc] + g.K[1 * 3 + k] * dG[1 * 2 + cc] + g.K[2 * 3 + k] * dG[2 * 2 + cc];
-        float dtz = dBm[0] / C.fx + dBm[3] / C.fy;
-        float dgt[2];
-#pragma unroll
-        for (int cc = 0; cc < 2; ++cc)
-            dgt[cc] = A[R_G2 + cc] - (dBm[0 * 2 + cc] * tx + dBm[1 * 2 + cc] * ty + dBm[2 * 2 + cc] * tz);
-#pragma unroll
-        for (int k = 0; k < 3; ++k) dt[k] -= dBm[k * 2 + 0] * g.gx + dBm[k * 2 + 1] * g.gy;
-        const float dax = dgt[0] / C.fx, day = dgt[1] / C.fy;
-        const float dot_a_nv = dax * g.nv[0] + day * g.nv[1];
-        dtz += dot_a_nv / g.sdot;
-        float dnv[3] = {tz * dax / g.sdot, tz * day / g.sdot, 0.f};
-        const float ds = -tz * dot_a_nv / (g.sdot * g.sdot);
-        dnv[0] += ds * tx; dnv[1] += ds * ty; dnv[2] += ds * tz;
-        dt[0] += ds * g.nv[0]; dt[1] += ds * g.nv[1]; dt[2] += ds * g.nv[2] + dtz;
-#pragma unroll
-        for (int k = 0; k < 3; ++k)
-            dn[k] += dnv[0] * WR(F, 0, k) + dnv[1] * WR(F, 1, k) + dnv[2] * WR(F, 2, k);
-    }
-#pragma unroll
-    for (int k = 0; k < 3; ++k) {
-        const float on = (g.kmin == k) ? g.sign : 0.0f;
-        dR[0 + k] += on * dn[0]; dR[3 + k] += on * dn[1]; dR[6 + k] += on * dn[2];
-    }
-
-    if (d_shs && na > 0) {
-        float b[15], bx[15], by[15], bz[15];
-#pragma unroll
-        for (int k = 0; k < 15; ++k) { b[k] = 0.f; bx[k] = 0.f; by[k] = 0.f; bz[k] = 0.f; }
-        sh_basis(C.sh_degree, g.dir[0], g.dir[1], g.dir[2], b);
-        sh_basis_grad(C.sh_degree, g.dir[0], g.dir[1], g.dir[2], bx, by, bz);
-        float* sp = s_sh + threadIdx.x * row;
-        const float v0 = A[R_VD], v1 = A[R_VD + 1], v2 = A[R_VD + 2];
-        float ddx = 0.f, ddy = 0.f, ddz = 0.f;
-#pragma unroll
-        for (int k = 0; k < 15; ++k) {
-            if (k < na) {
-                const float w = sp[3 * k + 0] * v0 + sp[3 * k + 1] * v1 + sp[3 * k + 2] * v2;
-                ddx += bx[k] * w; ddy += by[k] * w; ddz += bz[k] * w;
-                sp[3 * k + 0] = b[k] * v0; sp[3 * k + 1] = b[k] * v1; sp[3 * k + 2] = b[k] * v2;
-            }
-        }
-        for (int k = 3 * na; k < row; ++k) sp[k] = 0.f;
-        const float dd = g.dir[0] * ddx + g.dir[1] * ddy + g.dir[2] * ddz;
-        dm[0] += (ddx - g.dir[0] * dd) / g.dlen;
-        dm[1] += (ddy - g.dir[1] * dd) / g.dlen;
-        dm[2] += (ddz - g.dir[2] * dd) / g.dlen;
-    }
-
-#pragma unroll
-    for (int k = 0; k < 3; ++k) dm[k] += dt[0] * F.V[k * 4 + 0] + dt[1] * F.V[k * 4 + 1] + dt[2] * F.V[k * 4 + 2];
-    OUT(TEXGS_ACC_MEANS3D, d_means[3 * i + 0], dm[0]); OUT(TEXGS_ACC_MEANS3D, d_means[3 * i + 1], dm[1]); OUT(TEXGS_ACC_MEANS3D, d_means[3 * i + 2], dm[2]);
+    const bool sh = d_shs && na > 0;
+    float* sp = s_sh + threadIdx.x * row;
+    K8Part p;
+    k8_view<COV>(p, C, F, i, means, scales, rots, juv, cov6, opac[i], acc + (size_t)i * TEXGS_ACC_FLOATS, sp, sh ? na : 0,
+                 [sp](int k, float r, float g, float b) { sp[3 * k + 0] = r; sp[3 * k + 1] = g; sp[3 * k + 2] = b; });
+    if (sh) { for (int k = 3 * na; k < row; ++k) sp[k] = 0.f; }
+    OUT(TEXGS_ACC_OPACITIES, d_op[i], p.op);
+    if (d_uvs) { OUT(TEXGS_ACC_UVS, d_uvs[3 * i + 0], p.phi[0]); OUT(TEXGS_ACC_UVS, d_uvs[3 * i + 1], p.phi[1]); OUT(TEXGS_ACC_UVS, d_uvs[3 * i + 2], p.phi[2]); }
+    if (d_coff) { OUT(TEXGS_ACC_COLOR_OFFSET, d_coff[3 * i + 0], p.vd[0]); OUT(TEXGS_ACC_COLOR_OFFSET, d_coff[3 * i + 1], p.vd[1]); OUT(TEXGS_ACC_COLOR_OFFSET, d_coff[3 * i + 2], p.vd[2]); }
+    OUT(TEXGS_ACC_MEANS2D, d_means2D[3 * i + 0], p.m2[0]); OUT(TEXGS_ACC_MEANS2D, d_means2D[3 * i + 1], p.m2[1]); if (!(accumulate & TEXGS_ACC_MEANS2D)) d_means2D[3 * i + 2] = 0.f;
+    OUT(TEXGS_ACC_MEANS3D, d_means[3 * i + 0], p.dm[0]); OUT(TEXGS_ACC_MEANS3D, d_means[3 * i + 1], p.dm[1]); OUT(TEXGS_ACC_MEANS3D, d_means[3 * i + 2], p.dm[2]);
     if constexpr (COV) {
+        const float* dS = p.dS;
         OUT(TEXGS_ACC_COV3D, d_cov6[6 * i + 0], dS[0]); OUT(TEXGS_ACC_COV3D, d_cov6[6 * i + 1], dS[1] + dS[3]);
         OUT(TEXGS_ACC_COV3D, d_cov6[6 * i + 2], dS[2] + dS[6]); OUT(TEXGS_ACC_COV3D, d_cov6[6 * i + 3], dS[4]);
         OUT(TEXGS_ACC_COV3D, d_cov6[6 * i + 4], dS[5] + dS[7]); OUT(TEXGS_ACC_COV3D, d_cov6[6 * i + 5], dS[8]);
-    }
-    if constexpr (!COV) { OUT(TEXGS_ACC_SCALES, d_scales[3 * i + 0], dscale[0]); OUT(TEXGS_ACC_SCALES, d_scales[3 * i + 1], dscale[1]); OUT(TEXGS_ACC_SCALES, d_scales[3 * i + 2], dscale[2]); }
-
-    if constexpr (!COV) {
-    const float r = g.q[0], x = g.q[1], y = g.q[2], z = g.q[3];
-    OUT(TEXGS_ACC_ROTATIONS, d_rots[4 * i + 0], 2.0f * (-z * dR[1] + y * dR[2] + z * dR[3] - x * dR[5] - y * dR[6] + x * dR[7]));
-    OUT(TEXGS_ACC_ROTATIONS, d_rots[4 * i + 1], 2.0f * (y * dR[1] + z * dR[2] + y * dR[3] - 2.0f * x * dR[4] - r * dR[5] + z * dR[6] + r * dR[7] - 2.0f * x * dR[8]));
-    OUT(TEXGS_ACC_ROTATIONS, d_rots[4 * i + 2], 2.0f * (-2.0f * y * dR[0] + x * dR[1] + r * dR[2] + x * dR[3] + z * dR[5] - r * dR[6] + z * dR[7] - 2.0f * y * dR[8]));
-    OUT(TEXGS_ACC_ROTATIONS, d_rots[4 * i + 3], 2.0f * (-2.0f * z * dR[0] - r * dR[1] + x * dR[2] + r * dR[3] - 2.0f * z * dR[4] + y * dR[5] + x * dR[6] + y * dR[7]));
+    } else {
+        OUT(TEXGS_ACC_SCALES, d_scales[3 * i + 0], p.dscale[0]); OUT(TEXGS_ACC_SCALES, d_scales[3 * i + 1], p.dscale[1]); OUT(TEXGS_ACC_SCALES, d_scales[3 * i + 2], p.dscale[2]);
+        OUT(TEXGS_ACC_ROTATIONS, d_rots[4 * i + 0], p.dq[0]); OUT(TEXGS_ACC_ROTATIONS, d_rots[4 * i + 1], p.dq[1]);
+        OUT(TEXGS_ACC_ROTATIONS, d_rots[4 * i + 2], p.dq[2]); OUT(TEXGS_ACC_ROTATIONS, d_rots[4 * i + 3], p.dq[3]);
     }
 #undef OUT
     }
@@ -634,6 +663,106 @@
         __syncthreads();
         if (accumulate & TEXGS_ACC_SHS) sh_rows_out<K8_BLOCK, true>(d_shs + first, s_sh, count, vec);
         else sh_rows_out<K8_BLOCK, false>(d_shs + first, s_sh, count, vec);
+    }
+}
+
+struct K8GroupView {
+    CamConst C;
+    const float *vm, *pm, *cp;
+    const int32_t* radii;
+    float* acc;
+};
+struct K8Group {
+    K8GroupView v[TEXGS_K8_GROUP_MAX];
+    int V;
+};
+
+__global__ void __launch_bounds__(K8_BLOCK)
+k_preprocess_bwd_group(K8Group G, const float* __restrict__ means, const float* __restrict__ shs, const float* __restrict__ opac,
+                       const float* __restrict__ scales, const float* __restrict__ rots, const float* __restrict__ juv,
+                       float* __restrict__ d_means, float* __restrict__ d_means2D, float* __restrict__ d_shs,
+                       float* __restrict__ d_op, float* __restrict__ d_scales, float* __restrict__ d_rots,
+                       float* __restrict__ d_uvs) {
+    extern __shared__ __attribute__((aligned(16))) float s_sh[];
+    const int tid = (int)threadIdx.x;
+    const int i = blockIdx.x * K8_BLOCK + tid;
+    const int N = G.v[0].C.N, K = G.v[0].C.sh_coeffs;
+    const bool live = i < N;
+    const int row = 3 * K;
+    uint32_t vis = 0u;
+    int na_max = 0;
+#pragma unroll 1
+    for (int v = 0; v < G.V; ++v) {
+        const int deg = G.v[v].C.sh_degree;
+        const int na = (shs != nullptr && d_shs != nullptr && deg > 0) ? sh_active(deg, K) : 0;
+        na_max = max(na_max, na);
+        if (live && G.v[v].radii[i] > 0) vis |= 1u << v;
+    }
+    const size_t first = (size_t)blockIdx.x * K8_BLOCK * row;
+    const int count = (na_max > 0) ? (int)min((size_t)K8_BLOCK * row, (size_t)N * row - first) : 0;
+    float csh[45];
+#pragma unroll
+    for (int k = 0; k < 45; ++k) csh[k] = 0.f;
+    if (na_max > 0) {
+        for (int k = tid; k < count; k += K8_BLOCK) s_sh[k] = d_shs[first + k];
+        __syncthreads();
+        if (live) {
+#pragma unroll
+            for (int k = 0; k < 45; ++k) if (k < row) csh[k] = s_sh[tid * row + k];
+        }
+        __syncthreads();
+        for (int k = tid; k < count; k += K8_BLOCK) s_sh[k] = shs[first + k];
+        __syncthreads();
+    }
+    if (vis != 0u) {
+        float lm[3], ls[3], lq[4], lj[9];
+#pragma unroll
+        for (int k = 0; k < 3; ++k) { lm[k] = means[3 * i + k]; ls[k] = scales[3 * i + k]; }
+#pragma unroll
+        for (int k = 0; k < 4; ++k) lq[k] = rots[4 * i + k];
+#pragma unroll
+        for (int k = 0; k < 9; ++k) lj[k] = juv ? juv[9 * i + k] : 0.f;
+        const float op = opac[i];
+        float c_op = d_op[i], c_uv[3] = {0.f, 0.f, 0.f}, c_m2[2], c_m[3], c_s[3], c_q[4];
+        if (d_uvs) { c_uv[0] = d_uvs[3 * i + 0]; c_uv[1] = d_uvs[3 * i + 1]; c_uv[2] = d_uvs[3 * i + 2]; }
+        c_m2[0] = d_means2D[3 * i + 0]; c_m2[1] = d_means2D[3 * i + 1];
+#pragma unroll
+        for (int k = 0; k < 3; ++k) { c_m[k] = d_means[3 * i + k]; c_s[k] = d_scales[3 * i + k]; }
+#pragma unroll
+        for (int k = 0; k < 4; ++k) c_q[k] = d_rots[4 * i + k];
+#pragma unroll 1
+        for (int v = 0; v < G.V; ++v) {
+            if (!((vis >> v) & 1u)) continue;
+            const CamConst C = G.v[v].C;
+            const Frame F = load_frame(G.v[v].vm, G.v[v].pm, G.v[v].cp);
+            const int na = (na_max > 0 && C.sh_degree > 0) ? sh_active(C.sh_degree, K) : 0;
+            K8Part p;
+            k8_view<false>(p, C, F, 0, lm, ls, lq, juv ? lj : nullptr, nullptr, op, G.v[v].acc + (size_t)i * TEXGS_ACC_FLOATS,
+                           s_sh + tid * row, na,
+                           [&csh](int k, float r, float g, float b) { csh[3 * k + 0] += r; csh[3 * k + 1] += g; csh[3 * k + 2] += b; });
+            c_op += p.op;
+            c_m2[0] += p.m2[0]; c_m2[1] += p.m2[1];
+#pragma unroll
+            for (int k = 0; k < 3; ++k) { c_uv[k] += p.phi[k]; c_m[k] += p.dm[k]; c_s[k] += p.dscale[k]; }
+#pragma unroll
+            for (int k = 0; k < 4; ++k) c_q[k] += p.dq[k];
+        }
+        d_op[i] = c_op;
+        if (d_uvs) { d_uvs[3 * i + 0] = c_uv[0]; d_uvs[3 * i + 1] = c_uv[1]; d_uvs[3 * i + 2] = c_uv[2]; }
+        d_means2D[3 * i + 0] = c_m2[0]; d_means2D[3 * i + 1] = c_m2[1];
+#pragma unroll
+        for (int k = 0; k < 3; ++k) { d_means[3 * i + k] = c_m[k]; d_scales[3 * i + k] = c_s[k]; }
+#pragma unroll
+        for (int k = 0; k < 4; ++k) d_rots[4 * i + k] = c_q[k];
+    }
+    if (na_max > 0) {
+        __syncthreads();
+        if (live) {
+#pragma unroll
+            for (int k = 0; k < 45; ++k) if (k < row) s_sh[tid * row + k] = csh[k];
+        }
+        __syncthreads();
+        sh_rows_out<K8_BLOCK, false>(d_shs + first, s_sh, count, (((size_t)d_shs) & 15) == 0);
     }
 }
 
@@ -674,6 +803,28 @@
 #undef K8_LAUNCH
 }
 
+void launch_preprocess_bwd_group(const TexGSInputs* in, const TexGSGrads* gr, const TexGSGroupView* views, int num_views,
+                                 hipStream_t s) {
+    const int N = views[0].frame->num_gaussians;
+    if (N <= 0) return;
+    const int blocks = (N + K8_BLOCK - 1) / K8_BLOCK;
+    const size_t lds = gr->dL_dshs ? (size_t)K8_BLOCK * 3 * views[0].frame->sh_coeffs * sizeof(float) : 0;
+    for (int v0 = 0; v0 < num_views; v0 += TEXGS_K8_GROUP_MAX) {
+        K8Group G;
+        memset(&G, 0, sizeof(G));
+        G.V = (num_views - v0 < TEXGS_K8_GROUP_MAX) ? num_views - v0 : TEXGS_K8_GROUP_MAX;
+        for (int v = 0; v < G.V; ++v) {
+            const TexGSGroupView& w = views[v0 + v];
+            G.v[v].C = make_cam(w.frame);
+            G.v[v].vm = w.frame->viewmatrix; G.v[v].pm = w.frame->projmatrix; G.v[v].cp = w.frame->campos;
+            G.v[v].radii = w.geom->radii; G.v[v].acc = w.acc;
+        }
+        hipLaunchKernelGGL(k_preprocess_bwd_group, dim3(blocks), dim3(K8_BLOCK), lds, s, G, in->means3D, in->shs, in->opacities,
+                           in->scales, in->rotations, in->gradient_uvs, gr->dL_dmeans3D, gr->dL_dmeans2D, gr->dL_dshs,
+                           gr->dL_dopacities, gr->dL_dscales, gr->dL_drotations, gr->dL_duvs);
+    }
+}
+
 void launch_mark_visible(const TexGSFrame* f, const float* means3D, uint8_t* visible, hipStream_t s) {
     if (f->num_gaussians <= 0) return;
     const int blocks = (f->num_gaussians + TG_BLOCK - 1) / TG_BLOCK;
diff --git a/texture-gs_amd/texgs/_lib.py b/texture-gs_amd/texgs/_lib.py
--- a/texture-gs_amd/texgs/_lib.py
+++ b/texture-gs_amd/texgs/_lib.py
@@ -53,6 +53,13 @@
                 ("accumulate", C.c_int32)]
 
 
+class GroupView(C.Structure):
+    _fields_ = [("frame", C.POINTER(Frame)), ("geom", C.POINTER(Geom)), ("acc", _fp)]
+
+
+K8_GROUP_MAX = 8
+
+
 class UVNetStruct(C.Structure):
     _fields_ = [(n, _fp) for n in ("W1", "b1", "W2", "b2", "emb", "W3", "b3", "W4", "b4", "W5", "b5", "xyz_offset", "xyz_scale")] \
         + [("hidden", C.c_int32)]
@@ -99,7 +106,7 @@
 EXPORTS = ["texgs_abi_version", "texgs_build_id", "texgs_last_error", "texgs_scan_temp_bytes", "texgs_sort_temp_bytes",
            "texgs_preprocess_forward", "texgs_num_rendered_words", "texgs_num_rendered_begin", "texgs_num_rendered_reduce", "texgs_depth_sort_scan", "texgs_bin_sort_render_forward",
            "texgs_render_forward", "texgs_backward", "texgs_backward_render", "texgs_backward_preprocess",
-           "texgs_rgb_alpha_loss", "texgs_mark_visible", "texgs_profile_enable", "texgs_tex_bin_count",
+           "texgs_backward_preprocess_group", "texgs_rgb_alpha_loss", "texgs_mark_visible", "texgs_profile_enable", "texgs_tex_bin_count",
            "texgs_profile_read", "texgs_profile_select", "texgs_selftest_waveops", "texgs_geom_losses", "texgs_norm_from_depth",
            "texgs_uv_packed_bytes", "texgs_uv_pack", "texgs_uv_taylor_packed", "texgs_uv_backward", "texgs_uv_backward_temp_bytes",
            "texgs_hashgrid_levels", "texgs_hashgrid_forward", "texgs_hashgrid_backward_temp_bytes", "texgs_hashgrid_backward",
@@ -150,6 +157,8 @@
     lib.texgs_backward.argtypes = [P(Frame), P(Inputs), P(Geom), P(Binning), P(Image), P(Grads), C.c_void_p]
     lib.texgs_backward_render.argtypes = [P(Frame), P(Inputs), P(Geom), P(Binning), P(Image), P(Grads), C.c_void_p]
     lib.texgs_backward_preprocess.argtypes = [P(Frame), P(Inputs), P(Geom), P(Grads), C.c_void_p]
+    lib.texgs_backward_preprocess_group.argtypes = [P(Inputs), P(Grads), P(GroupView), C.c_int32, C.c_void_p]
+    lib.texgs_backward_preprocess_group.restype = C.c_int
     lib.texgs_mark_visible.argtypes = [P(Frame), C.c_void_p, C.c_void_p, C.c_void_p]
     lib.texgs_rgb_alpha_loss.argtypes = [C.c_void_p, C.c_void_p, C.c_void_p, C.c_void_p, C.c_int32, C.c_int32, C.c_float,
                                          C.c_float, C.c_void_p, C.c_void_p, C.c_void_p, C.c_void_p, C.c_void_p]
diff --git a/texture-gs_amd/texgs/multiview.py b/texture-gs_amd/texgs/multiview.py
--- a/texture-gs_amd/texgs/multiview.py
+++ b/texture-gs_amd/texgs/multiview.py
@@ -1,6 +1,17 @@
+import os
 from typing import List, Sequence
 
 import torch
+
+K8_GROUP_DEFAULT = 8
+
+
+def k8_group_size(num_views: int) -> int:
+    raw = os.environ.get("TEXGS_K8_GROUP", "").strip()
+    g = int(raw) if raw else K8_GROUP_DEFAULT
+    if g < 0:
+        raise ValueError("TEXGS_K8_GROUP must be >= 0")
+    return min(g, max(int(num_views), 1))
 
 
 def shard_views(num_views: int, rank: int, world: int) -> List[int]:
@@ -50,6 +61,84 @@
         self.replicas = []
         self.active = 0
         self.before_accumulate = None
+        self._group = None
+        self._acc_free = []
+        self._order_ev = None
+
+    @property
+    def group_open(self):
+        return self._group is not None
+
+    def begin_views(self, n: int) -> bool:
+        self.discard_views()
+        size = k8_group_size(n) if self.active == 0 else 0
+        if size:
+            self._group = {"size": size, "views": [], "sig": None}
+        self._order_ev = None
+        return bool(size)
+
+    def take_acc(self, N: int, device):
+        from . import _lib
+        for k, (buf, ev) in enumerate(self._acc_free):
+            if buf.shape[0] == N and buf.device == device:
+                del self._acc_free[k]
+                if ev is not None:
+                    torch.cuda.current_stream(device).wait_event(ev)
+                return buf
+        return torch.zeros(N, _lib.ACC_FLOATS, dtype=torch.float32, device=device)
+
+    def defer_view(self, sig, frame, inputs, geom, grads, acc, keep):
+        grp = self._group
+        if grp["views"] and grp["sig"] != sig:
+            self._flush()
+        grp["sig"] = sig
+        ev = torch.cuda.Event()
+        ev.record(torch.cuda.current_stream(acc.device))
+        grp["views"].append((frame, inputs, geom, grads, acc, keep, ev))
+        if len(grp["views"]) >= grp["size"]:
+            self._flush()
+
+    def order_wait(self):
+        self._flush()
+        if self._order_ev is not None:
+            torch.cuda.current_stream(self.flat.device).wait_event(self._order_ev)
+
+    def order_record(self):
+        self._order_ev = torch.cuda.Event()
+        self._order_ev.record(torch.cuda.current_stream(self.flat.device))
+
+    def _flush(self):
+        grp = self._group
+        if grp is None or not grp["views"]:
+            return
+        import ctypes as C
+        from . import _lib
+        views, grp["views"], grp["sig"] = grp["views"], [], None
+        device = views[0][4].device
+        cur = torch.cuda.current_stream(device)
+        if self._order_ev is not None:
+            cur.wait_event(self._order_ev)
+        for v in views:
+            cur.wait_event(v[6])
+            for t in v[5]:
+                if isinstance(t, torch.Tensor) and t.is_cuda:
+                    t.record_stream(cur)
+        arr = (_lib.GroupView * len(views))(*[_lib.GroupView(C.pointer(v[0]), C.pointer(v[2]), v[4].data_ptr()) for v in views])
+        with torch.cuda.device(device):
+            _lib.check(_lib.load().texgs_backward_preprocess_group(C.byref(views[0][1]), C.byref(views[0][3]), arr, len(views),
+                                                                    cur.cuda_stream), "texgs_backward_preprocess_group")
+        self.order_record()
+        for v in views:
+            self._acc_free.append((v[4], self._order_ev))
+
+    def flush_views(self):
+        try:
+            self._flush()
+        finally:
+            self.discard_views()
+
+    def discard_views(self):
+        self._group = None
 
     def select(self, k: int):
         while len(self.replicas) < k:
@@ -194,20 +283,30 @@
             prefetch_ahead=1):
         results = []
         views = list(views)
+        can_defer = (sink is not None and backward_fn is not None and order in ("backward", "accumulate")
+                     and hasattr(sink, "begin_views") and hasattr(sink, "flush_views"))
         if not self.streams:
-            for i, v in enumerate(views):
-                obj = forward_fn(v)
-                if prefetch_fn is not None and i + 1 < len(views):
-                    prefetch_fn(views[i + 1])
-                if backward_fn is not None:
-                    if texture_ready is not None and sink is not None and i == len(views) - 1:
-                        sink.before_accumulate = lambda: texture_ready([])
-                    try:
-                        backward_fn(obj)
-                    finally:
-                        if sink is not None:
-                            sink.before_accumulate = None
-                results.append(obj)
+            try:
+                if can_defer:
+                    sink.begin_views(len(views))
+                for i, v in enumerate(views):
+                    obj = forward_fn(v)
+                    if prefetch_fn is not None and i + 1 < len(views):
+                        prefetch_fn(views[i + 1])
+                    if backward_fn is not None:
+                        if texture_ready is not None and sink is not None and i == len(views) - 1:
+                            sink.before_accumulate = lambda: texture_ready([])
+                        try:
+                            backward_fn(obj)
+                        finally:
+                            if sink is not None:
+                                sink.before_accumulate = None
+                    results.append(obj)
+                if can_defer:
+                    sink.flush_views()
+            finally:
+                if can_defer and hasattr(sink, "discard_views"):
+                    sink.discard_views()
             return results
         if order not in ("backward", "accumulate", "none"):
             raise ValueError(order)
@@ -219,7 +318,9 @@
         prev_bwd = None
         render_done = {}
         depth = len(self.streams)
+        deferring = False
         try:
+            deferring = can_defer and sink.begin_views(len(views)) is not False
             ahead = depth * max(1, int(prefetch_ahead))
             if prefetch_fn is not None:
                 for i, v in enumerate(views[:ahead]):
@@ -240,7 +341,7 @@
                         if order == "accumulate":
                             last = i == len(views) - 1
 
-                            def hook(ev=prev_bwd, s=s, k=k, last=last):
+                            def hook(ev=None if deferring else prev_bwd, s=s, k=k, last=last):
                                 if texture_ready is not None:
                                     e = torch.cuda.Event()
                                     e.record(s)
@@ -254,9 +355,13 @@
                         prev_bwd = torch.cuda.Event()
                         prev_bwd.record(s)
                 results.append(obj)
+            if can_defer:
+                sink.flush_views()
         finally:
             if sink is not None:
                 sink.before_accumulate = None
+            if can_defer and hasattr(sink, "discard_views"):
+                sink.discard_views()
             for s in self.streams:
                 cur.wait_stream(s)
             if sink is not None and order == "none":
diff --git a/texture-gs_amd/texgs/rasterizer.py b/texture-gs_amd/texgs/rasterizer.py
--- a/texture-gs_amd/texgs/rasterizer.py
+++ b/texture-gs_amd/texgs/rasterizer.py
@@ -539,7 +539,7 @@
 
 
 def backward_raw(s: _State, dL_dcolor, dL_ddepth, dL_dnorm, dL_dalpha, sinks=None, before_accumulate=None,
-                 want=_lib.WANT_ALL):
+                 want=_lib.WANT_ALL, group=None):
     lib = _lib.load()
     if not s.tensors["for_backward"]:
         raise RuntimeError("this forward ran with for_backward=False (no survivor lists were kept): its backward cannot run")
@@ -570,11 +570,16 @@
                 _LAST_DIFFERENTIATED[device.index] = max(_LAST_DIFFERENTIATED.get(device.index, -1), s.serial)
         skey = (device.index, int(stream))
         sc = _SCRATCH.pop(skey, None) or SimpleNamespace(acc=None, bins=None)
-        if want_g and (sc.acc is None or sc.acc.shape[0] < max(N, 1)):
-            sc.acc = torch.zeros(max(N, 1), _lib.ACC_FLOATS, **f32)
-        acc = sc.acc if want_g else None
         sinks = sinks or {}
         outs, mask, res = _plan_outputs(N, s.K, textured, a.cov3D_precomp is not None, a.color_offset is not None, want, sinks, device)
+        defer = (group is not None and want_g and N > 0 and a.cov3D_precomp is None and a.color_offset is None
+                 and all(n in sinks for n in outs))
+        if defer:
+            acc = group.take_acc(N, device)
+        else:
+            if want_g and (sc.acc is None or sc.acc.shape[0] < max(N, 1)):
+                sc.acc = torch.zeros(max(N, 1), _lib.ACC_FLOATS, **f32)
+            acc = sc.acc if want_g else None
         tex_sink = sinks.get("texture") if want_t else None
         d_tex = (tex_sink if tex_sink is not None else torch.zeros(6, R, R, 3, **f32)) if want_t else None
         bins = None
@@ -588,7 +593,22 @@
                            _ptr(bins.rec) if bins else None, _ptr(bins.cursor) if bins else None,
                            _ptr(bins.base) if bins else None, bins.cap if bins else 0, mask)
         refs = [C.byref(x) for x in (s.frame, s.inputs, s.geom, s.bin, s.img, grads)]
-        if before_accumulate is None:
+        if defer:
+            _lib.check(lib.texgs_backward_render(*refs, stream), "texgs_backward_render")
+            if before_accumulate is not None:
+                before_accumulate()
+            sig = (N, s.K, mask) + tuple((t.data_ptr(), tuple(t.shape)) for t in a[:7] if t is not None) \
+                + tuple((n, t.data_ptr()) for n, t in sorted(outs.items()))
+            group.defer_view(sig, s.frame, s.inputs, s.geom, grads, acc,
+                             list(s.tensors["keep"]) + [s.tensors["radii"]] + list(outs.values()))
+        elif group is not None and want_g:
+            _lib.check(lib.texgs_backward_render(*refs, stream), "texgs_backward_render")
+            if before_accumulate is not None:
+                before_accumulate()
+            group.order_wait()
+            _lib.check(lib.texgs_backward_preprocess(*refs[:3], refs[5], stream), "texgs_backward_preprocess")
+            group.order_record()
+        elif before_accumulate is None:
             _lib.check(lib.texgs_backward(*refs, stream), "texgs_backward")
         else:
             _lib.check(lib.texgs_backward_render(*refs, stream), "texgs_backward_render")
@@ -662,7 +682,8 @@
             sinks = {k: g for k, g in ((k, _leaf_grad_sink(v)) for k, v in ctx.named.items()) if g is not None}
         d_means3D, d_means2D, d_shs, d_op, d_scales, d_rot, d_uvs, d_tex = backward_raw(
             s, dL_dcolor, dL_ddepth, dL_dnorm, dL_dalpha, sinks=sinks or None,
-            before_accumulate=getattr(ctx.grad_sink, "before_accumulate", None) if bucket else None, want=ctx.want)
+            before_accumulate=getattr(ctx.grad_sink, "before_accumulate", None) if bucket else None, want=ctx.want,
+            group=ctx.grad_sink if (bucket and getattr(ctx.grad_sink, "group_open", False)) else None)
         d_coff = s.tensors.get("d_color_offset")
         d_cov = s.tensors.get("d_cov3D")
         ctx.state = None
```

Result: faster. 1031 views/s (median of 5 runs) (+1.7%).
